# jasperlinthorst/reveal

Measured on AMD Instinct MI355X. Metric: Mbp/s indexed+MUM-anchored (reveal rem), higher is better.
Workload: dtype int32

## Files before the change

include/reveal_amd.h:

```cpp
#ifndef REVEAL_AMD_H
#define REVEAL_AMD_H
#include <stdint.h>

#ifdef __cplusplus
extern "C" {
#endif

typedef struct rv_index rv_index;

const char *rv_last_error(void);
int  rv_abi_version(void);
int  rv_sa_bits(void);
int  rv_device_count(void);

rv_index *rv_new(int device);
void rv_free(rv_index *h);

int rv_add_sample(rv_index *h);
int rv_add_sequence(rv_index *h, const char *seq, int64_t len, int64_t *begin, int64_t *end);
int rv_reset(rv_index *h);
int rv_reserve_text(rv_index *h, int64_t bytes);
int64_t rv_n(const rv_index *h);
int rv_nsamples(const rv_index *h);
int rv_nnodes(const rv_index *h);
// ... 39 lines not shown
int rv_align_end(rv_index *h);

typedef struct {
    int64_t steps;
    int64_t splits;
    int64_t anchored_bp;
    int32_t levels;
    int32_t maxdepth;
    int64_t scanned_ranks;
    double  t_scan, t_host, t_split, t_bubble;
} rv_align_stats;
int rv_align_builtin(rv_index *h, int minl, int minn, rv_align_stats *st);

int rv_align_builtin_until(rv_index *h, int minl, int minn, int stop_subs, rv_align_stats *st);
int rv_align_builtin_resume(rv_index *h, rv_align_stats *st);
int rv_align_builtin_continue(rv_index *h, int stop_subs, rv_align_stats *st);
int rv_frontier_counts(rv_index *h, int64_t *out);
int rv_frontier_export(rv_index *h, int64_t *meta, int64_t *node_first, int64_t *nodes);
int64_t rv_frontier_pack(rv_index *h, const int32_t *subs, int k, void *sa, void *lcp, void *bwt, int on_device);
int rv_frontier_import(rv_index *h, int minl, int minn, uint32_t maxlcp, int level, int nsubs, const int64_t *meta,
                       const int64_t *node_first, const int64_t *nodes, int64_t m,
                       const void *sa, const void *lcp, const void *bwt, int on_device);
int64_t rv_frontier_seeds_export(rv_index *h, const int32_t *subs, int k, int64_t *out, int64_t cap);
int rv_frontier_seeds_import(rv_index *h, int nsubs, const int64_t *words, int64_t nwords);
uint32_t rv_maxlcp(const rv_index *h);
int rv_cascade_info(const rv_index *h, int64_t *out);
int rv_capacity_events(const rv_index *h, int64_t *out);
const char *rv_cascade_why(const rv_index *h);
int64_t rv_anchor_count(rv_index *h, int64_t *members);
int rv_fetch_anchors(rv_index *h, uint32_t *l, int64_t *off, int64_t *pos);
int rv_set_result_buffers(rv_index *h, uint32_t *l, int64_t l_cap, int64_t *off, int64_t off_cap, int64_t *pos, int64_t pos_cap);
typedef struct {
    int64_t  key, n;
    int32_t  depth, nsamples, nnodes, picked;
    int64_t  nmums;
    uint32_t l; int32_t mn;
    int64_t  sp_min;
    uint64_t h_sa, h_lcp, h_mums;
} rv_trace;
int rv_set_trace(rv_index *h, int on);
int rv_set_preselect(rv_index *h, int64_t maxmums);
int rv_set_option(rv_index *h, const char *name, int64_t value);
int rv_get_option(rv_index *h, const char *name, int64_t *value);
int rv_set_launch_trace(int on);
int rv_option_count(void);
const char *rv_option_name(int k);
int64_t rv_trace_count(rv_index *h);
int rv_fetch_trace(rv_index *h, rv_trace *out, int64_t cap);

typedef struct rv_subindex rv_subindex;
rv_index *rv_clone(rv_index *h);
rv_subindex *rv_sx_main(rv_index *h);
rv_subindex *rv_sx_copy(rv_subindex *x);
void rv_sx_free(rv_subindex *x);
int rv_sx_info(const rv_subindex *x, rv_sub *out);
int rv_sx_nodes(const rv_subindex *x, int64_t *begin_end);
int64_t rv_sx_array(rv_subindex *x, int which, void *out, int64_t cap);
int64_t rv_sx_scan(rv_subindex *x, int minl, int minn, int64_t *members);
int rv_sx_fetch(rv_subindex *x, uint32_t *l, int32_t *n, int64_t *off, uint16_t *so, int64_t *pos);
int rv_sx_split(rv_subindex *x, const int64_t *lead, int nlead, const int64_t *trail, int ntrail,
                const int64_t *match, int nmatch, const int64_t *rest, int nrest, rv_subindex **out);
int rv_sx_extract(rv_subindex *x, int64_t *intervals, int niv);

int64_t rv_chain(int64_t m, int k, const uint32_t *len, const int32_t *nmem, const int64_t *crd, const int64_t *left,
                 const int64_t *right, int64_t wscore, int64_t wpen, int model, int64_t *out_idx, int64_t *out_score);

typedef struct { int64_t wscore, wpen, maxmums, seedsize; int gcmodel; int trim; double pcutoff; } rv_picker_args;
typedef struct {
    int picked; uint32_t pick_l; int32_t pick_n; int pick_members; uint16_t *pick_so; int64_t *pick_pos; int64_t member_cap;
    int64_t nleft, nright, nseed_members, seed_cap, seed_member_cap;
    uint32_t *seed_l; int32_t *seed_n; int64_t *seed_off; uint16_t *seed_so; int64_t *seed_pos; int64_t *seed_score; uint8_t *seed_right;
} rv_picker_out;
int rv_set_picker(rv_index *h, int kind, const rv_picker_args *args);
int rv_picker_info(const rv_index *h, int64_t *out);
int rv_pick_chain(const rv_picker_args *args, int nsub, int64_t m, const uint32_t *l, const int32_t *n, const int64_t *off, const uint16_t *so,
                  const int64_t *pos, int nsamples, const int64_t *seq_begin, const int64_t *iv_begin, const int64_t *iv_end, int minlength,
                  rv_picker_out *out);

typedef struct rv_graph rv_graph;
rv_graph *rv_graph_import(int64_t nnodes, const int64_t *node_b, const int64_t *node_e, const int8_t *node_aligned, const int8_t *node_sent,
                          const int64_t *off_ptr, const int32_t *off_sid, const int64_t *off_val,
                          int64_t nedges, const int32_t *edge_u, const int32_t *edge_v, const int64_t *edge_ptr, const int32_t *edge_paths,
                          const int64_t *pred_ptr, const int32_t *pred_edge, int npaths, const uint8_t *star, const int64_t *id2end,
                          int nstart, const int32_t *start_nodes, int literal_segments);
int rv_graph_pick(rv_graph *g, const rv_picker_args *args, int nsub, int64_t m, const uint32_t *l, const int32_t *n, const int64_t *off, const uint16_t *so, const int64_t *pos,
                  const int64_t *left, const int64_t *right, int minlength, rv_picker_out *out);
int rv_graph_align(rv_graph *g, const int64_t *nodes, int64_t nn, const int64_t *left, const int64_t *right, uint32_t l, const int64_t *pos, int npos,
                   int64_t *counts, int64_t *out6);
int rv_graph_align_fetch(rv_graph *g, int64_t *out);
int rv_set_graph_picker(rv_index *h, rv_graph *g, const rv_picker_args *args);
rv_graph *rv_graph_new(void);
int rv_graph_add_linear(rv_graph *g, int64_t b, int64_t e, int star);
int64_t rv_graph_read_gfa(rv_graph *g, rv_index *h, int64_t *text_n, const char *data, int64_t len, const char **names);
typedef struct GfaParsed rv_gfa_parsed;
rv_gfa_parsed *rv_gfa_parse(const char *data, int64_t len);
int64_t rv_graph_adopt(rv_graph *g, rv_index *h, int64_t *text_n, rv_gfa_parsed *parsed, const char **names);
void rv_gfa_parsed_free(rv_gfa_parsed *parsed);
int rv_graph_seal(rv_graph *g);
int rv_graph_paths(const rv_graph *g, int64_t *id2end);
int rv_graph_node_kinds(const rv_graph *g, int8_t *out);
int rv_graph_literal(const rv_graph *g);
int rv_graph_finish(rv_graph *g);
rv_graph *rv_graph_replay_begin(int nseq, const int64_t *begin, const int64_t *end);
int rv_set_replay_graph(rv_index *h, rv_graph *g);
rv_graph *rv_graph_replay(int nseq, const int64_t *begin, const int64_t *end, int64_t na, const uint32_t *an_l, const int64_t *an_off, const int64_t *an_pos);
const char *rv_graph_error(const rv_graph *g);
int rv_graph_sizes(const rv_graph *g, int64_t *out);
int rv_graph_export(const rv_graph *g, int64_t *node_b, int64_t *node_e, int8_t *node_aligned, int64_t *off_ptr, int32_t *off_sid, int64_t *off_val,
                    int64_t *succ_ptr, int32_t *succ_to, int32_t *succ_edge, int64_t *pred_ptr, int32_t *pred_from, int32_t *pred_edge, int64_t *edge_ptr, int32_t *edge_paths);
int rv_graph_prune(rv_graph *g, const char *T);
int64_t rv_graph_gfa(rv_graph *g, const char *T, int npaths, const char *const *names, const char *cmdline, const char **out);
void rv_graph_free(rv_graph *g);

enum { RV_K_SCAN_PAIR = 0, RV_K_SCAN_MULTI = 1, RV_K_SA_SORT = 2, RV_K_LCP = 3, RV_K_SPLIT = 4, RV_K_LABEL = 5,
       RV_K_BUBBLE = 6,
       RV_K_RADIX_SCATTER = 7, RV_K_RADIX_HIST = 8, RV_K_TEXT_ROUND = 9,
       RV_K_CASCADE = 10,
       RV_K_DIAG_TABLE = 11,
       RV_K_INIT_KEYS = 12,
       RV_K_PUBLISH = 13,
       RV_K_COUNT = 14 };
int rv_prof_enable(rv_index *h, int on);
int rv_prof_reset(rv_index *h);
int rv_prof_get(rv_index *h, int k, int64_t *launches, double *ms, double *bytes);
typedef struct rv_batch rv_batch;
rv_batch *rv_batch_new(void);
int rv_batch_add(rv_batch *b, rv_index *h);
int rv_batch_run(rv_batch *b, int minl, int minn, int construct, rv_align_stats *stats, int *status);
int rv_batch_info(const rv_batch *b, int64_t *out);
void rv_batch_free(rv_batch *b);
typedef struct rv_many rv_many;
rv_many *rv_many_new(int device);
void rv_many_free(rv_many *m);
int rv_many_option(rv_many *m, const char *name, int64_t value);
int rv_many_set_picker(rv_many *m, int kind, const rv_picker_args *args);
int64_t rv_many_add(rv_many *m, const char *const *seqs, const int64_t *lens, int k);
int rv_many_clear(rv_many *m);
int rv_many_run(rv_many *m, int minl, int minn, rv_align_stats *total);
int64_t rv_many_anchor_count(rv_many *m, int64_t *first, int64_t *members);
int rv_many_fetch(rv_many *m, uint32_t *l, int64_t *off, int64_t *pos);
int64_t rv_many_text(rv_many *m, int64_t job, char *out, int64_t cap);
int rv_many_info(const rv_many *m, int64_t *out);
int64_t rv_many_arrays(rv_many *m, int64_t job, int which, void *out, int64_t cap);
void *rv_dev_alloc(int device, int64_t bytes);
int rv_dev_free(int device, void *p);
int rv_ipc_export(int device, const void *p, uint8_t handle[64]);
void *rv_ipc_open(int device, const uint8_t handle[64]);
int rv_ipc_close(int device, void *p);
int rv_dev_copy(int device, void *dst, const void *src, int64_t bytes);
int rv_measure_bandwidth(int device, int64_t bytes, int iters, double *read_gbs, double *copy_gbs);
int rv_sa_stats(rv_index *h, int *sigma, int *bits, int *k0, int *rounds, int64_t *sorted_elems, int *radix_passes);
int rv_sa_diag_table(rv_index *h);
int rv_sa_tail(rv_index *h, int64_t *out);

int rv_test_exclusive_sum_u32(const uint32_t *in, uint32_t *out, int64_t n);
int rv_test_inclusive_max_u32(const uint32_t *in, uint32_t *out, int64_t n);
int rv_test_radix_sort(uint64_t *keys, uint32_t *vals, int64_t n, int bit_lo, int bit_hi);
int rv_test_radix_time(int64_t n, int bits, int dist, int flags, int iters, double *ms, int64_t *bad);

#ifdef __cplusplus
}
#endif
#endif
```

reveal_amd/_index.py:

```python
import ctypes
import mmap
import os
import sys
import numpy as np

from . import _lib
from ._lib import RV_T, RV_SA, RV_SAI, RV_LCP, RV_SO, RV_NSEP


def _page_array(count, dtype):
    nbytes = max(int(count), 1) * np.dtype(dtype).itemsize
    m = mmap.mmap(-1, (nbytes + mmap.PAGESIZE - 1) // mmap.PAGESIZE * mmap.PAGESIZE)
    return np.frombuffer(m, dtype=dtype, count=max(int(count), 1))


def _pairs(iv, sa64):
    a = np.ascontiguousarray(np.array([(int(b), int(e)) for b, e in iv], dtype=np.int64).reshape(-1, 2))
    return a, len(a)


_OPTION_DEFAULTS = {}


def make_index_type(sa64, error):

    class index(object):

        def __init__(self, sa="", lcp="", cache=0):
            self._lib = _lib.get(sa64)
            self._dll = self._lib.dll
            self._h = None
            self._safile, self._lcpfile, self._cache = sa or "", lcp or "", int(cache)
            self._samples, self._nodes, self.skipmums = [], set(), []
            self._leftnode = self._rightnode = None
            self._depth = 0
            self._constructed = False
            self._main = self
            self._slot = None
            self._sx = None
            self._n_sub = None
            self._nsamples_sub = None
            self._h = self._dll.rv_new(_lib.device())
            if not self._h:
                raise error(self._lib.err())
            self.options_from_env()

        def set_option(self, name, value=1):
            if self._dll.rv_set_option(self._main._h, name.encode(), int(value)) != 0:
                self._fail()

        def get_option(self, name):
            v = ctypes.c_int64(0)
            if self._dll.rv_get_option(self._main._h, name.encode(), ctypes.byref(v)) != 0:
                self._fail()
            return v.value

        def options_from_env(self):
            for k in range(self._dll.rv_option_count()):
                name = self._dll.rv_option_name(k).decode()
                v = os.environ.get(name)
                if v is None:
                    d = _OPTION_DEFAULTS.get((sa64, name))
                    if d is None:
                        d = _OPTION_DEFAULTS[(sa64, name)] = self.get_option(name)
                    elif self.get_option(name) != d:
                        self.set_option(name, d)
                    continue
                try:
                    iv = int(v) if v.strip() else 1
                except ValueError:
                    iv = 1
                _OPTION_DEFAULTS.setdefault((sa64, name), self.get_option(name))
                self.set_option(name, iv)

        @property
        def _main(self):
            m = self.__dict__.get("_main_ref")
            return self if m is None else m

        @_main.setter
        def _main(self, v):
            self.__dict__["_main_ref"] = None if v is self else v

        def __del__(self):
            try:
                if getattr(self, "_sx", None):
                    self._dll.rv_sx_free(self._sx)
                    self._sx = None
                if self._h and self._main is self:
                    self._dll.rv_free(self._h)
                    self._h = None
            except Exception:
                pass

        def _fail(self, exc=None):
            raise (exc or error)(self._lib.err())

        def addsample(self, *args):
            if len(args) < 1:
                raise error("Specify name of sample as argument.")
            if not isinstance(args[0], str):
                raise error("Sample name has to be a string.")
            self._samples.append(args[0])
            self._dll.rv_add_sample(self._h)
            self._constructed = False
            return None

        def addsequence(self, seq):
            if isinstance(seq, str):
                seq = seq.encode()
            elif not isinstance(seq, (bytes, bytearray)):
                raise TypeError("argument 1 must be str or bytes")
            b, e = ctypes.c_int64(0), ctypes.c_int64(0)
            if self._dll.rv_add_sequence(self._h, bytes(seq), len(seq), ctypes.byref(b), ctypes.byref(e)) != 0:
                self._fail()
            intv = (b.value, e.value)
            self._nodes.add(intv)
            self._constructed = False
            return intv

        def reset(self, reserve=0):
            if self._main is not self or self._slot is not None:
                raise error("reset() is for a main index outside align()")
            if self._sx:
                self._dll.rv_sx_free(self._sx)
                self._sx = None
            if self._dll.rv_reset(self._h) != 0:
                self._fail()
            if reserve and self._dll.rv_reserve_text(self._h, int(reserve)) != 0:
                self._fail()
            self._samples, self._nodes, self.skipmums = [], set(), []
            self._leftnode = self._rightnode = None
            self._depth = 0
            self._constructed = False
            self._pending = False
            self._n_sub = self._nsamples_sub = None

        def upload(self):
            if self._dll.rv_upload(self._h) != 0:
                self._fail()

        def upload_again(self):
            if self._dll.rv_upload_again(self._h) != 0:
                self._fail()

        def prof(self, enable=None, reset=False, only=None):
            ids = {"scan_pair": _lib.K_SCAN_PAIR, "scan_multi": _lib.K_SCAN_MULTI, "sa_build": _lib.K_SA_SORT, "lcp": _lib.K_LCP,
                   "split": _lib.K_SPLIT, "label": _lib.K_LABEL, "bubble": _lib.K_BUBBLE, "radix_scatter": _lib.K_RADIX_SCATTER,
                   "radix_hist": _lib.K_RADIX_HIST, "text_round": _lib.K_TEXT_ROUND, "cascade": _lib.K_CASCADE, "diag_table": _lib.K_DIAG_TABLE,
                   "init_keys": _lib.K_INIT_KEYS, "publish": _lib.K_PUBLISH}
            if enable is not None:
                on = 0
                if enable:
                    on = 1 if only is None else sum(2 << ids[k] for k in only)
                self._dll.rv_prof_enable(self._h, on)
            if reset:
                self._dll.rv_prof_reset(self._h)
            out = {}
            for name, k in ids.items():
                n, ms, by = ctypes.c_int64(0), ctypes.c_double(0), ctypes.c_double(0)
                self._dll.rv_prof_get(self._h, k, ctypes.byref(n), ctypes.byref(ms), ctypes.byref(by))
                out[name] = (n.value, ms.value, by.value)
            return out

        def sa_stats(self):
            v = [ctypes.c_int(0) for _ in range(4)]
            se, rp = ctypes.c_int64(0), ctypes.c_int(0)
            self._dll.rv_sa_stats(self._h, *[ctypes.byref(x) for x in v], ctypes.byref(se), ctypes.byref(rp))
            tail = (ctypes.c_int64 * 2)()
            self._dll.rv_sa_tail(self._h, tail)
            return dict(sigma=v[0].value, bits=v[1].value, k0=v[2].value, rounds=v[3].value, sorted_elems=se.value, radix_passes=rp.value,
                        diag_table=int(self._dll.rv_sa_diag_table(self._h)), far_pairs=int(tail[0]), lcp_list=int(tail[1]))

        def construct(self, rc=0):
            if self._sx:
                self._dll.rv_sx_free(self._sx)
                self._sx = None
            r = self._dll.rv_construct(self._h, int(rc), self._safile.encode(), self._lcpfile.encode(), self._cache)
            if r != 0:
                self._fail()
            self._constructed = True
            self._rc = 1 if int(rc) == 1 else 0
            self._depth = 0
            self._main = self
            return None

        def _sx_info(self):
            info = _lib.RvSub()
            self._dll.rv_sx_info(self._sx, ctypes.byref(info))
            return info

        @property
        def n(self):
            if self._sx:
                return self._sx_info().n
            return self._n_sub if self._n_sub is not None else self._dll.rv_n(self._h)

        @property
        def depth(self):
            return self._depth

        @property
        def nsamples(self):
            if self._sx and self._depth > 0:
                return self._sx_info().nsamples
            return self._nsamples_sub if self._nsamples_sub is not None else self._dll.rv_nsamples(self._h)

        @property
        def samples(self):
            return self._main._samples

        @property
        def nodes(self):
            if self.__dict__.get("_nodes_stale"):
                self._sync_nodes()
            return self._nodes

        @property
        def leftnode(self):
            return self._leftnode

        @property
        def rightnode(self):
            return self._rightnode

        @property
        def nsep(self):
            ns = self._dll.rv_nsamples(self._h)
            out = np.zeros(max(ns - 1, 1), dtype=np.int64)
            k = self._dll.rv_get_array(self._h, RV_NSEP, out.ctypes.data, len(out))
            return [int(x) for x in out[:max(k, 0)]]

        def _array(self, which, dtype, count, exc=TypeError):
            out = np.zeros(max(count, 1), dtype=dtype)
            if self._sx and which in (RV_SA, RV_LCP):
                k = self._dll.rv_sx_array(self._sx, which, out.ctypes.data, len(out))
            elif self._slot is not None and which in (RV_SA, RV_LCP):
                k = self._dll.rv_sub_array(self._h, self._slot, which, out.ctypes.data, len(out))
            else:
                k = self._dll.rv_get_array(self._h, which, out.ctypes.data, len(out))
            if k < 0:
                raise exc(self._lib.err())
            return out[:k]

        def _main_n(self):
            return self._dll.rv_n(self._h)

        @property
        def SA(self):
            return self._array(RV_SA, self._lib.sa_t, self.n).tolist()

        @property
        def LCP(self):
            return self._array(RV_LCP, self._lib.lcp_t, self.n).tolist()

        @property
        def SAi(self):
            return self._array(RV_SAI, self._lib.sa_t, self._main_n()).tolist()

        @property
        def SO(self):
            return self._array(RV_SO, np.uint16, self._main_n()).tolist()

        @property
        def T(self):
            return self._array(RV_T, np.uint8, self._main_n(), exc=error).tobytes().decode("latin-1")

        def array(self, name):
            which = {"SA": RV_SA, "LCP": RV_LCP, "SAi": RV_SAI, "SO": RV_SO, "T": RV_T}[name]
            dt = {RV_SA: self._lib.sa_t, RV_LCP: self._lib.lcp_t, RV_SAI: self._lib.sa_t, RV_SO: np.uint16, RV_T: np.uint8}[which]
            return self._array(which, dt, self.n if which in (RV_SA, RV_LCP) else self._main_n())

        def _sx_mums(self, minl, minn):
            mem = ctypes.c_int64(0)
            cnt = self._dll.rv_sx_scan(self._sx, int(minl), int(minn), ctypes.byref(mem))
            if cnt < 0:
                self._fail()
            l = np.zeros(max(cnt, 1), dtype=np.uint32); n = np.zeros(max(cnt, 1), dtype=np.int32)
            off = np.zeros(cnt + 1, dtype=np.int64)
            so = np.zeros(max(mem.value, 1), dtype=np.uint16); pos = np.zeros(max(mem.value, 1), dtype=np.int64)
            if self._dll.rv_sx_fetch(self._sx, l.ctypes.data, n.ctypes.data, off.ctypes.data, so.ctypes.data, pos.ctypes.data) != 0:
                self._fail()
            return _csr_to_tuples(cnt, l, n, off, so, pos)

        def getmums(self, minl=0):
            if self._sx:
                if self._dll.rv_nsamples(self._h) != 2:
                    raise error("getmums on a sub-index needs a two-sample main index")
                rc = 1 if getattr(self._main, "_rc", 0) else 0
                out = [(l, (spd[0][1], spd[1][1]), rc) for l, _, spd in self._sx_mums(minl, 0)]
                if rc:
                    nsep0, nT = self.nsep[0], self._main_n()
                    out = [(l, (a, nsep0 + (nT - b - l)), rc) for l, (a, b), _ in out]
                return out
            cnt = self._dll.rv_getmums(self._h, int(minl))
            if cnt < 0:
                self._fail(TypeError if cnt == -2 else error)
            l = np.zeros(max(cnt, 1), dtype=np.uint32)
            a = np.zeros(max(cnt, 1), dtype=np.int64)
            b = np.zeros(max(cnt, 1), dtype=np.int64)
            if self._dll.rv_fetch_mums(self._h, l.ctypes.data, a.ctypes.data, b.ctypes.data, len(l)) != 0:
                self._fail()
            rc = 1 if getattr(self, "_rc", 0) else 0
            return [(int(l[k]), (int(a[k]), int(b[k])), rc) for k in range(cnt)]

        def _multi(self, minlength, minn, mems):
            if self._sx:
                if mems or self._dll.rv_nsamples(self._h) <= 2:
                    raise error("only getmultimums of an index with more than two samples is available on a sub-index")
                return self._sx_mums(minlength, minn)
            members = ctypes.c_int64(0)
            cnt = self._dll.rv_getmultimums(self._h, int(minlength), int(minn), mems, ctypes.byref(members))
            if cnt < 0:
                self._fail(TypeError if cnt == -2 else error)
            l = np.zeros(max(cnt, 1), dtype=np.uint32); n = np.zeros(max(cnt, 1), dtype=np.int32)
            off = np.zeros(cnt + 1, dtype=np.int64)
            so = np.zeros(max(members.value, 1), dtype=np.uint16); pos = np.zeros(max(members.value, 1), dtype=np.int64)
            if self._dll.rv_fetch_multi(self._h, l.ctypes.data, n.ctypes.data, off.ctypes.data, so.ctypes.data, pos.ctypes.data) != 0:
                self._fail()
            return _csr_to_tuples(cnt, l, n, off, so, pos)

        def getmultimums(self, minlength=0, minn=2):
            return self._multi(minlength, minn, 0)

        def getmultimems(self, minlength=0, minn=2):
# ... 404 lines not shown
```

reveal_amd/_lib.py:

```python
import ctypes
import importlib.util
import os
import sys
import numpy as np

_HERE = os.path.dirname(os.path.abspath(__file__))

RV_T, RV_SA, RV_SAI, RV_LCP, RV_SO, RV_NSEP, RV_NODES = range(7)
K_SCAN_PAIR, K_SCAN_MULTI, K_SA_SORT, K_LCP, K_SPLIT, K_LABEL, K_BUBBLE, K_RADIX_SCATTER, K_RADIX_HIST, K_TEXT_ROUND, K_CASCADE, K_DIAG_TABLE, K_INIT_KEYS, K_PUBLISH = range(14)

CAPACITY_EVENTS = ("pair_ovf", "pair_out", "pair_pick_ovf", "pair_second_copy", "multi_rec", "multi_mem", "multi_cand",
                   "mems_rec", "mems_mem", "mems_long")
CAP_SITES = {"multi_cand": 1, "cas_wit": 2, "cas_tables": 4, "casm_matches": 8, "casm_wit": 16, "casm_tables": 32,
             "mems_rec": 64, "mems_mem": 128, "mems_long": 256}

c_i64p = ctypes.POINTER(ctypes.c_int64)
V = ctypes.c_void_p


class RvSub(ctypes.Structure):
    _fields_ = [("n", ctypes.c_int64), ("depth", ctypes.c_int32), ("nsamples", ctypes.c_int32),
                ("nnodes", ctypes.c_int32), ("parent", ctypes.c_int32), ("kind", ctypes.c_int32),
                ("reserved", ctypes.c_int32), ("nmums", ctypes.c_int64), ("nmembers", ctypes.c_int64)]


class RvAlignStats(ctypes.Structure):
    _fields_ = [("steps", ctypes.c_int64), ("splits", ctypes.c_int64), ("anchored_bp", ctypes.c_int64),
                ("levels", ctypes.c_int32), ("maxdepth", ctypes.c_int32), ("scanned_ranks", ctypes.c_int64),
                ("t_scan", ctypes.c_double), ("t_host", ctypes.c_double), ("t_split", ctypes.c_double),
                ("t_bubble", ctypes.c_double)]


TRACE_DTYPE = np.dtype([("key", np.int64), ("n", np.int64), ("depth", np.int32), ("nsamples", np.int32),
                        ("nnodes", np.int32), ("picked", np.int32), ("nmums", np.int64), ("l", np.uint32),
                        ("mn", np.int32), ("sp_min", np.int64), ("h_sa", np.uint64), ("h_lcp", np.uint64),
                        ("h_mums", np.uint64)], align=True)

_I, _L, _D = ctypes.c_int, ctypes.c_int64, ctypes.c_double
SYMBOLS = {
    "rv_last_error": (ctypes.c_char_p, []),
    "rv_abi_version": (_I, []),
    "rv_sa_bits": (_I, []),
    "rv_device_count": (_I, []),
    "rv_new": (V, [_I]),
    "rv_free": (None, [V]),
    "rv_add_sample": (_I, [V]),
    "rv_add_sequence": (_I, [V, ctypes.c_char_p, _L, c_i64p, c_i64p]),
    "rv_reset": (_I, [V]),
    "rv_reserve_text": (_I, [V, _L]),
    "rv_n": (_L, [V]),
    "rv_nsamples": (_I, [V]),
    "rv_nnodes": (_I, [V]),
    "rv_node_list": (_I, [V, V]),
    "rv_construct": (_I, [V, _I, ctypes.c_char_p, ctypes.c_char_p, _I]),
    "rv_upload": (_I, [V]),
    "rv_upload_again": (_I, [V]),
    "rv_get_array": (_L, [V, _I, V, _L]),
    "rv_getmums": (_L, [V, _I]),
    "rv_fetch_mums": (_I, [V, V, V, V, _L]),
    "rv_getmultimums": (_L, [V, _I, _I, _I, c_i64p]),
    "rv_fetch_multi": (_I, [V, V, V, V, V, V]),
    "rv_align_begin": (_I, [V, _I, _I]),
    "rv_frontier_size": (_I, [V]),
    "rv_frontier_scan": (_I, [V]),
    "rv_sub_skip_scan": (_I, [V, _I]),
    "rv_sub_info": (_I, [V, _I, ctypes.POINTER(RvSub)]),
    "rv_sub_nodes": (_I, [V, _I, V]),
    "rv_sub_mums": (_I, [V, _I, V, V, V, V, V]),
    "rv_sub_array": (_L, [V, _I, _I, V, _L]),
    "rv_sub_split": (_I, [V, _I, ctypes.c_uint32, _I, V, V, _I, V, _I, V, _I, V, _I]),
    "rv_frontier_commit": (_I, [V, V]),
    "rv_align_end": (_I, [V]),
    "rv_align_builtin": (_I, [V, _I, _I, ctypes.POINTER(RvAlignStats)]),
    "rv_align_builtin_until": (_I, [V, _I, _I, _I, ctypes.POINTER(RvAlignStats)]),
    "rv_align_builtin_resume": (_I, [V, ctypes.POINTER(RvAlignStats)]),
    "rv_align_builtin_continue": (_I, [V, _I, ctypes.POINTER(RvAlignStats)]),
    "rv_frontier_counts": (_I, [V, V]),
    "rv_frontier_export": (_I, [V, V, V, V]),
    "rv_frontier_pack": (_L, [V, V, _I, V, V, V, _I]),
    "rv_frontier_import": (_I, [V, _I, _I, ctypes.c_uint32, _I, _I, V, V, V, _L, V, V, V, _I]),
    "rv_frontier_seeds_export": (_L, [V, V, _I, V, _L]),
    "rv_frontier_seeds_import": (_I, [V, _I, V, _L]),
    "rv_maxlcp": (ctypes.c_uint32, [V]),
    "rv_cascade_info": (ctypes.c_int, [V, V]),
    "rv_cascade_why": (ctypes.c_char_p, [V]),
    "rv_capacity_events": (_I, [V, V]),
    "rv_anchor_count": (_L, [V, c_i64p]),
    "rv_fetch_anchors": (_I, [V, V, V, V]),
    "rv_set_result_buffers": (_I, [V, V, _L, V, _L, V, _L]),
    "rv_set_trace": (_I, [V, _I]),
    "rv_set_preselect": (_I, [V, _L]),
    "rv_set_option": (_I, [V, ctypes.c_char_p, _L]),
    "rv_set_launch_trace": (_I, [_I]),
    "rv_batch_new": (V, []),
    "rv_batch_add": (_I, [V, V]),
    "rv_batch_run": (_I, [V, _I, _I, _I, V, V]),
    "rv_batch_info": (_I, [V, V]),
    "rv_batch_free": (None, [V]),
    "rv_dev_alloc": (V, [_I, _L]),
    "rv_dev_free": (_I, [_I, V]),
    "rv_ipc_export": (_I, [_I, V, V]),
    "rv_ipc_open": (V, [_I, V]),
    "rv_ipc_close": (_I, [_I, V]),
    "rv_dev_copy": (_I, [_I, V, V, _L]),
    "rv_get_option": (_I, [V, ctypes.c_char_p, c_i64p]),
    "rv_option_count": (_I, []),
    "rv_option_name": (ctypes.c_char_p, [_I]),
    "rv_trace_count": (_L, [V]),
    "rv_fetch_trace": (_I, [V, V, _L]),
    "rv_clone": (V, [V]),
    "rv_sx_main": (V, [V]),
    "rv_sx_copy": (V, [V]),
    "rv_sx_free": (None, [V]),
    "rv_sx_info": (_I, [V, ctypes.POINTER(RvSub)]),
    "rv_sx_nodes": (_I, [V, V]),
    "rv_sx_array": (_L, [V, _I, V, _L]),
    "rv_sx_scan": (_L, [V, _I, _I, c_i64p]),
    "rv_sx_fetch": (_I, [V, V, V, V, V, V]),
    "rv_sx_split": (_I, [V, V, _I, V, _I, V, _I, V, _I, V]),
    "rv_sx_extract": (_I, [V, V, _I]),
    "rv_chain": (_L, [_L, _I, V, V, V, V, V, _L, _L, _I, V, V]),
    "rv_prof_enable": (_I, [V, _I]),
    "rv_prof_reset": (_I, [V]),
    "rv_prof_get": (_I, [V, _I, c_i64p, ctypes.POINTER(_D), ctypes.POINTER(_D)]),
    "rv_measure_bandwidth": (_I, [_I, _L, _I, ctypes.POINTER(_D), ctypes.POINTER(_D)]),
    "rv_sa_stats": (_I, [V] + [ctypes.POINTER(_I)] * 4 + [c_i64p, ctypes.POINTER(_I)]),
    "rv_sa_diag_table": (_I, [V]),
    "rv_sa_tail": (_I, [V, c_i64p]),
    "rv_set_picker": (_I, [V, _I, V]),
    "rv_picker_info": (_I, [V, c_i64p]),
    "rv_pick_chain": (_I, [V, _I, _L, V, V, V, V, V, _I, V, V, V, _I, V]),
    "rv_graph_import": (V, [_L, V, V, V, V, V, V, V, _L, V, V, V, V, V, V, _I, V, V, _I, V, _I]),
    "rv_graph_pick": (_I, [V, V, _I, _L, V, V, V, V, V, V, V, _I, V]),
    "rv_graph_align": (_I, [V, V, _L, V, V, ctypes.c_uint32, V, _I, V, V]),
    "rv_graph_align_fetch": (_I, [V, V]),
    "rv_graph_finish": (_I, [V]),
    "rv_set_graph_picker": (_I, [V, V, V]),
    "rv_graph_new": (V, []),
    "rv_graph_replay_begin": (V, [_I, V, V]),
    "rv_set_replay_graph": (_I, [V, V]),
    "rv_graph_add_linear": (_I, [V, _L, _L, _I]),
    "rv_graph_read_gfa": (_L, [V, V, V, V, _L, V]),
    "rv_graph_paths": (_I, [V, V]),
    "rv_graph_seal": (_I, [V]),
    "rv_gfa_parse": (V, [V, _L]),
    "rv_graph_adopt": (_L, [V, V, V, V, V]),
    "rv_gfa_parsed_free": (None, [V]),
    "rv_add_sequences": (_I, [V, V, _L, V, _L]),
    "rv_graph_node_kinds": (_I, [V, V]),
    "rv_graph_literal": (_I, [V]),
    "rv_graph_replay": (V, [_I, V, V, _L, V, V, V]),
    "rv_graph_error": (ctypes.c_char_p, [V]),
    "rv_graph_sizes": (_I, [V, c_i64p]),
    "rv_graph_export": (_I, [V] * 15),
    "rv_graph_prune": (_I, [V, V]),
    "rv_graph_gfa": (_L, [V, V, _I, V, V, V]),
    "rv_graph_free": (None, [V]),
    "rv_many_new": (V, [_I]),
    "rv_many_free": (None, [V]),
    "rv_many_option": (_I, [V, ctypes.c_char_p, _L]),
    "rv_many_set_picker": (_I, [V, _I, V]),
    "rv_many_add": (_L, [V, V, V, _I]),
    "rv_many_clear": (_I, [V]),
    "rv_many_run": (_I, [V, _I, _I, ctypes.POINTER(RvAlignStats)]),
    "rv_many_anchor_count": (_L, [V, V, c_i64p]),
    "rv_many_fetch": (_I, [V, V, V, V]),
    "rv_many_text": (_L, [V, _L, V, _L]),
    "rv_many_info": (_I, [V, V]),
    "rv_many_arrays": (_L, [V, _L, _I, V, _L]),
    "rv_test_exclusive_sum_u32": (_I, [V, V, _L]),
    "rv_test_inclusive_max_u32": (_I, [V, V, _L]),
    "rv_test_radix_sort": (_I, [V, V, _L, _I, _I]),
    "rv_test_radix_time": (_I, [_L, _I, _I, _I, _I, ctypes.POINTER(_D), c_i64p]),
}


def _share_torch_runtime():
    if os.environ.get("RV_SYSTEM_HIP") or "torch" in sys.modules:
        return
    try:
        spec = importlib.util.find_spec("torch")
    except (ImportError, ValueError):
        spec = None
    if spec is None or not spec.origin:
        return
    path = os.path.join(os.path.dirname(spec.origin), "lib", "libamdhip64.so")
    if os.path.exists(path):
        ctypes.CDLL(path, mode=ctypes.RTLD_GLOBAL)


class Lib:
    def __init__(self, sa64=False):
        self.sa64 = sa64
        _share_torch_runtime()
        name = "libreveal_amd64.so" if sa64 else "libreveal_amd.so"
        self.path = os.path.join(os.environ.get("RV_LIB_DIR") or _HERE, name)
        if not os.path.exists(self.path):
            raise ImportError("%s is missing: build it with `python -c 'import __graft_entry__ as g; g.build()'` "
                              "(hipcc --offload-arch=gfx950); reveal_amd has no CPU fallback" % self.path)
        self.dll = ctypes.CDLL(self.path)
        for sym, (res, args) in SYMBOLS.items():
            fn = getattr(self.dll, sym)
            fn.restype, fn.argtypes = res, args
        self.sa_t = np.int64 if sa64 else np.int32
        self.lcp_t = np.uint32 if sa64 else np.int32
        assert self.dll.rv_sa_bits() == (64 if sa64 else 32)
        v = os.environ.get("RV_LAUNCH_TRACE")
        if v is not None and v.strip() not in ("", "0"):
            self.dll.rv_set_launch_trace(1)

    def err(self):
        return (self.dll.rv_last_error() or b"").decode(errors="replace")


_libs = {}
_device = 0


def set_device(i):
    global _device
    _device = int(i)


def device():
    return _device


def measure_bandwidth(nbytes=1 << 30, iters=10):
    lib = get(False)
    r, c = _D(0), _D(0)
    if lib.dll.rv_measure_bandwidth(device(), int(nbytes), int(iters), ctypes.byref(r), ctypes.byref(c)) != 0:
        raise RuntimeError(lib.err())
    return r.value, c.value


def set_launch_trace(on=True):
    return [bool(get(w).dll.rv_set_launch_trace(1 if on else 0)) for w in (False, True)]


def get(sa64=False):
    if sa64 not in _libs:
        _libs[sa64] = Lib(sa64)
    return _libs[sa64]
```

reveal_amd/csrc/rv_api.hip:

```cpp
#include "rv_index.h"
#include "rv_cascade.h"
#include <limits>
#include <stdarg.h>
#include <stdio.h>
#include <string.h>
#include <limits.h>
#include <algorithm>
#include <thread>

static thread_local char g_err[1024] = "";

void rv_set_error(const char *fmt, ...) {
    va_list ap;
    va_start(ap, fmt);
    vsnprintf(g_err, sizeof g_err, fmt, ap);
    va_end(ap);
}

static std::vector<rv_index *> &live_handles() { static std::vector<rv_index *> v; return v; }
std::mutex &rv_trim_mutex() { static std::mutex *m = new std::mutex(); return *m; }
bool rv_oom_trim() {
    size_t got = 0;
    bool log = false;
    int caller_dev = 0;
// ... 788 lines not shown
        int id = h->prof.begin(q, RV_K_SCAN_MULTI, (double)m * (sizeof(sa_t) + sizeof(lcp_t)));
        RV_TRY(rv_scan_multi_launch(h->ws, SA, LCP, m, BWT, h->dNsep.as<sa_t>(), h->nsamples, minl, minn,
                                    brec.as<RvMultiRec>(), bso.as<uint16_t>(), bpos.as<sa_t>(), (u32)std::min<size_t>(rcap, 0xffffffffu),
                                    (u32)std::min<size_t>(mcap, 0xffffffffu), bcnt.as<u32>(), btab.as<uint4>(), d_sub_start, d_sub_want, nsubs));
        h->prof.end(q, id);
        u32 tot[2] = {0, 0};
        RV_HIP(hipMemcpyAsync(tot, bcnt.p, 8, hipMemcpyDeviceToHost, q));
        RV_HIP(hipMemcpyAsync(tab.data(), btab.p, (size_t)ntile * sizeof(uint4), hipMemcpyDeviceToHost, q));
        RV_HIP(hipStreamSynchronize(q));
        if (tot[0] <= rcap && tot[1] <= mcap) {
            std::vector<RvMultiRec> rr(tot[0]);
            std::vector<uint16_t> rso(tot[1]);
            std::vector<sa_t> rpos(tot[1]);
            if (tot[0]) RV_HIP(hipMemcpy(rr.data(), brec.p, (size_t)tot[0] * sizeof(RvMultiRec), hipMemcpyDeviceToHost));
            if (tot[1]) {
                RV_HIP(hipMemcpy(rso.data(), bso.p, (size_t)tot[1] * 2, hipMemcpyDeviceToHost));
                RV_HIP(hipMemcpy(rpos.data(), bpos.p, (size_t)tot[1] * sizeof(sa_t), hipMemcpyDeviceToHost));
            }
            l.reserve(tot[0]); n.reserve(tot[0]); off.reserve(tot[0] + 1); so.reserve(tot[1]); pos.reserve(tot[1]);
            for (int64_t t = 0; t < ntile; t++) {
                const uint4 e = tab[(size_t)t];
                for (u32 k = 0; k < e.y; k++) {
                    const RvMultiRec &r = rr[e.x + k];
                    l.push_back(r.l); n.push_back((int32_t)r.n);
                    if (ub_out) ub_out->push_back((int64_t)r.ub);
                }
                for (u32 k = 0; k < e.w; k++) { so.push_back(rso[e.z + k]); pos.push_back((int64_t)rpos[e.z + k]); }
            }
            int64_t acc = 0;
            for (size_t k = 0; k < n.size(); k++) { acc += n[k]; off.push_back(acc); }
            return 0;
        }
        if (tot[0] > rcap) { h->ws.cap_events[RV_CE_MULTI_REC]++; RV_TRY(brec.reserve((size_t)tot[0] * sizeof(RvMultiRec))); }
        if (tot[1] > mcap) { h->ws.cap_events[RV_CE_MULTI_MEM]++; RV_TRY(bso.reserve((size_t)tot[1] * 2)); RV_TRY(bpos.reserve((size_t)tot[1] * sizeof(sa_t))); }
    }
    rv_set_error("multi scan: output buffer sizing failed");
    return -1;
}

int rv_run_multi_pick(rv_index *h, const sa_t *SA, const lcp_t *LCP, const uint8_t *BWT, int64_t m, int minl, int minn,
                      const int64_t *d_sub_start, const int *d_sub_want, int nsubs, const int *d_tile_sub, std::vector<u32> &pick_l, std::vector<sa_t> &pick_pos,
                      int (*after_pick)(rv_index *), bool *redo) {
    pick_l.assign((size_t)nsubs, 0); pick_pos.clear();
    if (m <= 1 || nsubs <= 0) return 0;
    hipStream_t q = h->ws.stream;
    const int W = h->nsamples;
    DBuf &bbest = h->ws.misc[12], &bl = h->ws.misc[13], &bpos = h->ws.misc[7], &bcand = h->ws.misc[8], &bcnt = h->ws.misc[1];
    RV_TRY(bbest.reserve((size_t)nsubs * 8)); RV_TRY(bl.reserve((size_t)nsubs * 4)); RV_TRY(bpos.reserve((size_t)nsubs * W * sizeof(sa_t)));
    RV_TRY(bcnt.reserve((RV_MULTI_REGIONS * 64 + 16) * 4));
    if (bcand.cap < 65536 * RV_MULTI_CAND_BYTES) RV_TRY(bcand.reserve((size_t)std::max<int64_t>(65536, m / 64) * RV_MULTI_CAND_BYTES));
    for (int attempt = 0; attempt < 2; attempt++) {
        size_t ccap = std::min<size_t>(bcand.cap / RV_MULTI_CAND_BYTES, 0xffffffffu);
        if (attempt == 0) ccap = h->ws.cap_first<size_t>(RV_CS_MULTI_CAND, ccap, RV_MULTI_REGIONS);
        h->ws.multi_cand_cap = (u32)(ccap / RV_MULTI_REGIONS);
        hipEvent_t ev_a, ev_b;
        (void)h->prof.attach(RV_K_SCAN_MULTI, (double)m * 8.0, &ev_a, &ev_b);
        RV_TRY(rv_multi_pick_launch(h->ws, SA, LCP, m, BWT, h->dNsep.as<sa_t>(), W, minl, minn, d_sub_start, d_sub_want, nsubs, d_tile_sub,
                                    bbest.as<unsigned long long>(), bl.as<u32>(), bpos.as<sa_t>(), (RvMultiCand *)bcand.p,
                                    (u32)ccap, bcnt.as<u32>(), ev_a, ev_b));
        u32 ncand = 0;
        pick_pos.resize((size_t)nsubs * W);
        {
            const size_t b1 = (size_t)nsubs * 4, b2 = (size_t)nsubs * W * sizeof(sa_t), o1 = 64, o2 = (o1 + b1 + 63) & ~(size_t)63;
            RV_TRY(h->ws.hpin.reserve(o2 + b2 + 64));
            uint8_t *hp = h->ws.hpin.as<uint8_t>();
            if (!h->ws.ev_rb) RV_HIP(hipEventCreateWithFlags(&h->ws.ev_rb, hipEventDisableTiming));
            RV_HIP(hipMemcpyAsync(hp, bcnt.as<u32>() + RV_MULTI_REGIONS * 64, 4, hipMemcpyDeviceToHost, q));
            RV_HIP(hipMemcpyAsync(hp + o1, bl.p, b1, hipMemcpyDeviceToHost, q));
            RV_HIP(hipMemcpyAsync(hp + o2, bpos.p, b2, hipMemcpyDeviceToHost, q));
            RV_HIP(hipEventRecord(h->ws.ev_rb, q));
            if (attempt == 0 && after_pick) RV_TRY(after_pick(h));
            const hipError_t qe = rv_event_wait(h->ws.ev_rb);
            if (qe != hipSuccess) { rv_set_error("stream: %s", hipGetErrorString(qe)); return -1; }
            memcpy(&ncand, hp, 4); memcpy(pick_l.data(), hp + o1, b1); memcpy(pick_pos.data(), hp + o2, b2);
        }
        if ((size_t)ncand <= ccap / RV_MULTI_REGIONS) return 0;
        if (redo) *redo = true;
        h->ws.cap_events[RV_CE_MULTI_CAND]++;
        RV_TRY(bcand.reserve(((size_t)ncand + ncand / 2 + 64) * RV_MULTI_REGIONS * RV_MULTI_CAND_BYTES));
    }
    rv_set_error("multi picker: candidate buffer sizing failed");
    return -1;
}

extern "C" {

int64_t rv_getmultimums(rv_index *h, int minlength, int minn, int mems, int64_t *members) {
    if (!h->constructed || h->main_arrays_freed) { rv_set_error("Index not yet constructed."); return -2; }
    if (h->nsamples <= 2) {
        if (mems && h->nsamples == 2 && minn >= 2) { h->mm_l.clear(); h->mm_n.clear(); h->mm_off.assign(1, 0); h->mm_so.clear(); h->mm_pos.clear(); if (members) *members = 0; return 0; }
        rv_set_error("getmultimums needs more than two samples (SO not available)"); return -1;
    }
    (void)hipSetDevice(h->device);
    if (rv_run_multi_scan(h, h->dSA.as<sa_t>(), h->dLCP.as<lcp_t>(), h->dBWT.as<uint8_t>(), h->n, minlength, minn, mems, h->mm_l, h->mm_n, h->mm_off, h->mm_so, h->mm_pos, nullptr, nullptr, nullptr, 0)) return -1;
    if (members) *members = (int64_t)h->mm_pos.size();
    return (int64_t)h->mm_l.size();
}

int rv_fetch_multi(rv_index *h, uint32_t *l, int32_t *n, int64_t *off, uint16_t *so, int64_t *pos) {
    memcpy(l, h->mm_l.data(), h->mm_l.size() * 4);
    memcpy(n, h->mm_n.data(), h->mm_n.size() * 4);
    memcpy(off, h->mm_off.data(), h->mm_off.size() * 8);
    memcpy(so, h->mm_so.data(), h->mm_so.size() * 2);
    memcpy(pos, h->mm_pos.data(), h->mm_pos.size() * 8);
    return 0;
}

int64_t rv_getmums(rv_index *h, int minl) {
    if (!h->constructed || h->main_arrays_freed) { rv_set_error("Index not yet constructed."); return -2; }
    (void)hipSetDevice(h->device);
    std::vector<RvPairRec> recs;
    if (rv_run_pair_scan(h, h->dSA.as<sa_t>(), h->dLCP.as<lcp_t>(), h->dBWT.as<uint8_t>(), h->n, minl, recs, nullptr, nullptr, nullptr, 0, nullptr, false) != 0) return -1;
    h->m_l.resize(recs.size()); h->m_a.resize(recs.size()); h->m_b.resize(recs.size());
    for (size_t k = 0; k < recs.size(); k++) {
        int64_t b = recs[k].b;
        if (h->rc == 1) b = h->nsep[0] + (h->nT - b - (int64_t)recs[k].l);
        h->m_l[k] = recs[k].l; h->m_a[k] = recs[k].a; h->m_b[k] = b;
    }
    return (int64_t)recs.size();
}

int rv_fetch_mums(rv_index *h, uint32_t *l, int64_t *a, int64_t *b, int64_t cap) {
    if (cap < (int64_t)h->m_l.size()) { rv_set_error("buffer too small"); return -1; }
    for (size_t k = 0; k < h->m_l.size(); k++) { l[k] = h->m_l[k]; a[k] = h->m_a[k]; b[k] = h->m_b[k]; }
    return 0;
}

int rv_prof_enable(rv_index *h, int on) {
    h->prof.on = on != 0;
    h->prof.mask = (on & 1) ? 0xFFFFFFFFu : ((u32)on >> 1);
    return 0;
}
int rv_prof_reset(rv_index *h) { (void)hipStreamSynchronize(h->ws.stream); h->prof.reset(); return 0; }
int rv_prof_get(rv_index *h, int k, int64_t *launches, double *ms, double *bytes) {
    if (k < 0 || k >= RV_K_COUNT) { rv_set_error("bad kernel id"); return -1; }
    (void)hipStreamSynchronize(h->ws.stream);
    h->prof.resolve();
    if (launches) *launches = h->prof.launches[k];
    if (ms) *ms = h->prof.ms[k];
    if (bytes) *bytes = h->prof.bytes[k];
    return 0;
}
int rv_sa_stats(rv_index *h, int *sigma, int *bits, int *k0, int *rounds, int64_t *sorted_elems, int *radix_passes) {
    if (sigma) *sigma = h->sa_stats.sigma;
    if (bits) *bits = h->sa_stats.bits;
    if (k0) *k0 = h->sa_stats.k0;
    if (rounds) *rounds = h->sa_stats.rounds;
    if (sorted_elems) *sorted_elems = h->sa_stats.sorted_elems;
    if (radix_passes) *radix_passes = h->sa_stats.radix_passes;
    return 0;
}
int rv_sa_diag_table(rv_index *h) { return h->sa_stats.diag_table; }
int rv_sa_tail(rv_index *h, int64_t *out) { if (!h || !out) return -1; out[0] = h->sa_stats.far_pairs; out[1] = h->sa_stats.lcp_list; return 0; }

}
namespace {
typedef int bw_v4 __attribute__((ext_vector_type(4)));
__global__ __launch_bounds__(256) void k_bw_read(const bw_v4 *__restrict__ a, int64_t n16, unsigned *sink) {
    bw_v4 acc = {0, 0, 0, 0};
    for (int64_t i = (int64_t)blockIdx.x * 256 + threadIdx.x; i < n16; i += (int64_t)gridDim.x * 256) acc ^= __builtin_nontemporal_load(a + i);
    if ((acc.x ^ acc.y ^ acc.z ^ acc.w) == 0x12345678) sink[0] = 1;
}
__global__ __launch_bounds__(256) void k_bw_copy(const bw_v4 *__restrict__ a, bw_v4 *__restrict__ b, int64_t n16) {
    for (int64_t i = (int64_t)blockIdx.x * 256 + threadIdx.x; i < n16; i += (int64_t)gridDim.x * 256) __builtin_nontemporal_store(__builtin_nontemporal_load(a + i), b + i);
}
}
extern "C" {
struct rv_batch {
    std::vector<rv_index *> hs;
    RvBatchGroup *g = nullptr;
    std::vector<std::string> errs;
};
rv_batch *rv_batch_new(void) {
    try { return new rv_batch(); } catch (...) { rv_set_error("rv_batch_new: out of host memory"); return nullptr; }
}
int rv_batch_add(rv_batch *b, rv_index *h) {
    if (!b || !h) { rv_set_error("rv_batch_add: null argument"); return -1; }
    if (!b->hs.empty() && b->hs[0]->device != h->device) { rv_set_error("rv_batch_add: the handles of a batch live on one device"); return -1; }
    try { b->hs.push_back(h); } catch (...) { rv_set_error("rv_batch_add: out of host memory"); return -1; }
    return 0;
}
void rv_batch_free(rv_batch *b) {
    if (!b) return;
    rv_batch_group_free(b->g);
    delete b;
}
int rv_batch_info(const rv_batch *b, int64_t *out) {
    out[0] = out[1] = 0;
    if (b && b->g) rv_batch_group_info(b->g, out);
    return 0;
}
int rv_batch_run(rv_batch *b, int minl, int minn, int construct, rv_align_stats *stats, int *status) {
    if (!b || b->hs.empty()) { rv_set_error("rv_batch_run: empty batch"); return -1; }
    const int n = (int)b->hs.size();
    try {
        b->errs.assign((size_t)n, std::string());
        if (!b->g) b->g = rv_batch_group_new(b->hs[0]->device);
        int members = 0;
        for (rv_index *h : b->hs) {
            const bool in = h->nsamples > 2 && !h->ws.opt.no_cascade;
            h->batch = in ? b->g : nullptr; h->batch_settled = false;
            members += in ? 1 : 0;
        }
        rv_batch_group_begin(b->g, members);
        std::vector<int> rc((size_t)n, 0);
        auto work = [&](int i) {
            rv_index *h = b->hs[(size_t)i];
            int r = 0;
            if (hipSetDevice(h->device) != hipSuccess) { rv_set_error("hipSetDevice failed"); r = -1; }
            if (r == 0 && construct) r = rv_construct(h, 0, "", "", 0);
            if (r == 0) r = rv_align_builtin(h, minl, minn, stats ? &stats[i] : nullptr);
            if (h->batch && !h->batch_settled) { h->batch_settled = true; rv_batch_group_leave(h->batch); }
            if (r != 0) b->errs[(size_t)i] = rv_last_error();
            rc[(size_t)i] = r;
        };
        std::vector<std::thread> th;
        int started = n;
        for (int i = 1; i < n; i++) {
            try { th.emplace_back(work, i); }
            catch (...) { started = i; break; }
        }
        if (started < n) for (int i = started; i < n; i++) { rv_index *h = b->hs[(size_t)i]; if (h->batch) { h->batch_settled = true; rv_batch_group_leave(h->batch); h->batch = nullptr; } }
        work(0);
        for (auto &t : th) t.join();
        for (int i = started; i < n; i++) work(i);
        int bad = -1;
        for (int i = 0; i < n; i++) { b->hs[(size_t)i]->batch = nullptr; if (status) status[i] = rc[(size_t)i]; if (rc[(size_t)i] != 0 && bad < 0) bad = i; }
        if (bad >= 0) { rv_set_error("rv_batch_run: job %d: %s", bad, b->errs[(size_t)bad].c_str()); return -1; }
        return 0;
    } catch (const std::exception &e) {
        for (rv_index *h : b->hs) h->batch = nullptr;
        rv_set_error("rv_batch_run: %s", e.what());
        return -1;
    }
}

void *rv_dev_alloc(int device, int64_t bytes) {
    void *p = nullptr;
    if (bytes < 0 || hipSetDevice(device) != hipSuccess) { rv_set_error("rv_dev_alloc: bad device or size"); return nullptr; }
    const hipError_t e = hipMalloc(&p, (size_t)std::max<int64_t>(bytes, 256));
    if (e != hipSuccess) { (void)hipGetLastError(); rv_set_error("rv_dev_alloc(%lld bytes): %s", (long long)bytes, hipGetErrorString(e)); return nullptr; }
    return p;
}
int rv_dev_free(int device, void *p) {
    if (!p) return 0;
    RV_HIP(hipSetDevice(device));
    RV_HIP(hipFree(p));
    return 0;
}
int rv_ipc_export(int device, const void *p, uint8_t handle[64]) {
    static_assert(sizeof(hipIpcMemHandle_t) == 64, "hipIpcMemHandle_t is 64 bytes");
    RV_HIP(hipSetDevice(device));
    hipIpcMemHandle_t hd;
    RV_HIP(hipIpcGetMemHandle(&hd, const_cast<void *>(p)));
    memcpy(handle, &hd, 64);
    return 0;
}
void *rv_ipc_open(int device, const uint8_t handle[64]) {
    if (hipSetDevice(device) != hipSuccess) { rv_set_error("rv_ipc_open: bad device"); return nullptr; }
    hipIpcMemHandle_t hd;
    memcpy(&hd, handle, 64);
    void *p = nullptr;
    const hipError_t e = hipIpcOpenMemHandle(&p, hd, hipIpcMemLazyEnablePeerAccess);
    if (e != hipSuccess) { (void)hipGetLastError(); rv_set_error("rv_ipc_open: %s", hipGetErrorString(e)); return nullptr; }
    return p;
}
int rv_ipc_close(int device, void *p) {
    if (!p) return 0;
    RV_HIP(hipSetDevice(device));
    RV_HIP(hipIpcCloseMemHandle(p));
    return 0;
}
int rv_dev_copy(int device, void *dst, const void *src, int64_t bytes) {
    if (bytes <= 0) return 0;
    RV_HIP(hipSetDevice(device));
    RV_HIP(hipMemcpy(dst, src, (size_t)bytes, hipMemcpyDefault));
    RV_HIP(hipStreamSynchronize(nullptr));
    return 0;
}

int rv_measure_bandwidth(int device, int64_t bytes, int iters, double *read_gbs, double *copy_gbs) {
    if (bytes < (1 << 20) || iters < 1) { rv_set_error("rv_measure_bandwidth: bytes >= 1 MiB and iters >= 1 needed"); return -1; }
    RV_HIP(hipSetDevice(device));
    const int64_t n16 = bytes / 16;
    void *a = nullptr, *b = nullptr; unsigned *sink = nullptr;
    hipStream_t q = nullptr; hipEvent_t e0 = nullptr, e1 = nullptr;
    RV_HIP(hipMalloc(&a, (size_t)n16 * 16)); RV_HIP(hipMalloc(&b, (size_t)n16 * 16)); RV_HIP(hipMalloc((void **)&sink, 64));
    RV_HIP(hipStreamCreateWithFlags(&q, hipStreamNonBlocking));
    RV_HIP(hipEventCreate(&e0)); RV_HIP(hipEventCreate(&e1));
    RV_HIP(hipMemsetAsync(a, 1, (size_t)n16 * 16, q)); RV_HIP(hipMemsetAsync(b, 2, (size_t)n16 * 16, q));
    const unsigned grid = 256 * 16;
    double out[2] = {0, 0};
    for (int pass = 0; pass < 2; pass++) {
        for (int r = -1; r < iters; r++) {
            if (r == 0) RV_HIP(hipEventRecord(e0, q));
            if (pass == 0) hipLaunchKernelGGL(k_bw_read, dim3(grid), dim3(256), 0, q, (const bw_v4 *)a, n16, sink);
            else hipLaunchKernelGGL(k_bw_copy, dim3(grid), dim3(256), 0, q, (const bw_v4 *)a, (bw_v4 *)b, n16);
        }
        RV_HIP(hipEventRecord(e1, q));
        RV_HIP(hipEventSynchronize(e1));
        float ms = 0.f;
        RV_HIP(hipEventElapsedTime(&ms, e0, e1));
        out[pass] = (double)n16 * 16 * (pass ? 2 : 1) * iters / ((double)ms * 1e6);
    }
    if (read_gbs) *read_gbs = out[0];
    if (copy_gbs) *copy_gbs = out[1];
    (void)hipEventDestroy(e0); (void)hipEventDestroy(e1); (void)hipStreamDestroy(q);
    (void)hipFree(a); (void)hipFree(b); (void)hipFree(sink);
    return 0;
}

static int test_ws(Workspace &ws) {
    if (rv_device_count() <= 0) { rv_set_error("no HIP device"); return -1; }
    RV_HIP(hipSetDevice(0));
    RV_HIP(hipStreamCreateWithFlags(&ws.stream, hipStreamNonBlocking));
    return 0;
}
static void test_ws_done(Workspace &ws) { ws.release(); (void)hipStreamDestroy(ws.stream); }

static int test_scan(const uint32_t *in, uint32_t *out, int64_t n, bool maxscan) {
    Workspace ws;
    RV_TRY(test_ws(ws));
    DBuf a, b;
    int r = 0;
    if (a.reserve((size_t)n * 4 + 64) || b.reserve((size_t)n * 4 + 64)) r = -1;
    if (!r && hipMemcpy(a.p, in, (size_t)n * 4, hipMemcpyHostToDevice) != hipSuccess) r = -1;
    if (!r) r = maxscan ? rv_inclusive_max_u32(ws, a.as<u32>(), b.as<u32>(), n) : rv_exclusive_sum_u32(ws, a.as<u32>(), b.as<u32>(), n);
    if (!r && hipStreamSynchronize(ws.stream) != hipSuccess) { rv_set_error("sync failed: %s", hipGetErrorString(hipGetLastError())); r = -1; }
    if (!r && hipMemcpy(out, b.p, (size_t)n * 4, hipMemcpyDeviceToHost) != hipSuccess) r = -1;
    a.release(); b.release();
    test_ws_done(ws);
    return r;
}
int rv_test_exclusive_sum_u32(const uint32_t *in, uint32_t *out, int64_t n) { return test_scan(in, out, n, false); }
int rv_test_inclusive_max_u32(const uint32_t *in, uint32_t *out, int64_t n) { return test_scan(in, out, n, true); }

int rv_test_radix_sort(uint64_t *keys, uint32_t *vals, int64_t n, int bit_lo, int bit_hi) {
    Workspace ws;
    RV_TRY(test_ws(ws));
    DBuf k0, k1, v0, v1;
    int r = 0, in1 = 0;
    if (k0.reserve((size_t)n * 8 + 64) || k1.reserve((size_t)n * 8 + 64) || v0.reserve((size_t)n * 4 + 64) || v1.reserve((size_t)n * 4 + 64)) r = -1;
    if (!r && hipMemcpy(k0.p, keys, (size_t)n * 8, hipMemcpyHostToDevice) != hipSuccess) r = -1;
    if (!r && hipMemcpy(v0.p, vals, (size_t)n * 4, hipMemcpyHostToDevice) != hipSuccess) r = -1;
    if (!r) r = rv_radix_sort_pairs<u32>(ws, k0.as<u64>(), v0.as<u32>(), k1.as<u64>(), v1.as<u32>(), n, bit_lo, bit_hi, &in1);
    if (!r && hipStreamSynchronize(ws.stream) != hipSuccess) { rv_set_error("sync failed: %s", hipGetErrorString(hipGetLastError())); r = -1; }
    if (!r && hipMemcpy(keys, in1 ? k1.p : k0.p, (size_t)n * 8, hipMemcpyDeviceToHost) != hipSuccess) r = -1;
    if (!r && hipMemcpy(vals, in1 ? v1.p : v0.p, (size_t)n * 4, hipMemcpyDeviceToHost) != hipSuccess) r = -1;
    k0.release(); k1.release(); v0.release(); v1.release();
    test_ws_done(ws);
    return r;
}

}
namespace {
__device__ inline u64 rt_mix(u64 x) { x ^= x >> 33; x *= 0xff51afd7ed558ccdull; x ^= x >> 33; x *= 0xc4ceb9fe1a85ec53ull; x ^= x >> 33; return x; }
__global__ __launch_bounds__(256) void k_rt_fill(u64 *keys, u32 *vals, int64_t n, int bits, int dist) {
    const int64_t i = (int64_t)blockIdx.x * 256 + threadIdx.x;
    if (i >= n) return;
    u64 r = rt_mix((u64)i * 0x9E3779B97F4A7C15ull + 12345);
    u64 k = 0;
    if (dist == 0) k = r;
    else if (dist == 1) { u64 r2 = rt_mix(r); for (int j = 0; j < 17; j++) { k = k * 5 + 1 + (r2 & 3); r2 >>= 2; } }
    const u64 mask = bits >= 64 ? ~0ull : (1ull << bits) - 1;
    keys[i] = (k & mask) | (r & ~mask & 0x00ffffffffffffffull);
    vals[i] = (u32)i;
}
__global__ __launch_bounds__(256) void k_rt_check(const u64 *keys, const u32 *vals, int64_t n, int bits, unsigned long long *bad) {
    const int64_t i = (int64_t)blockIdx.x * 256 + threadIdx.x;
    if (i + 1 >= n) return;
    const u64 mask = bits >= 64 ? ~0ull : (1ull << bits) - 1;
    const u64 a = keys[i] & mask, b = keys[i + 1] & mask;
    if (a > b || (a == b && vals[i] > vals[i + 1])) atomicAdd(bad, 1ull);
}
}
extern "C" {
int rv_test_radix_time(int64_t n, int bits, int dist, int flags, int iters, double *ms, int64_t *bad) {
    Workspace ws;
    RV_TRY(test_ws(ws));
    ws.opt.rs_bits = (flags & 1) ? 10 : 8; ws.opt.rs_xcd = (flags & 2) ? 1 : 0; ws.opt.rs_cnt16 = (flags & 4) ? 1 : 0; ws.opt.rs_no_digit_bytes = (flags & 8) ? 1 : 0;
    DBuf k0, k1, v0, v1, db;
    int r = 0, in1 = 0;
    hipEvent_t e0 = nullptr, e1 = nullptr;
    if (k0.reserve((size_t)n * 8 + 64) || k1.reserve((size_t)n * 8 + 64) || v0.reserve((size_t)n * 4 + 64) || v1.reserve((size_t)n * 4 + 64) || db.reserve(64)) r = -1;
    if (!r && (hipEventCreate(&e0) != hipSuccess || hipEventCreate(&e1) != hipSuccess)) r = -1;
    for (int it = 0; !r && it < iters; it++) {
        hipLaunchKernelGGL(k_rt_fill, dim3((unsigned)ceil_div(n, 256)), dim3(256), 0, ws.stream, k0.as<u64>(), v0.as<u32>(), n, bits, dist);
        (void)hipEventRecord(e0, ws.stream);
        r = rv_radix_sort_pairs<u32>(ws, k0.as<u64>(), v0.as<u32>(), k1.as<u64>(), v1.as<u32>(), n, 0, bits, &in1);
        (void)hipEventRecord(e1, ws.stream);
        if (!r && hipEventSynchronize(e1) != hipSuccess) { rv_set_error("sync failed: %s", hipGetErrorString(hipGetLastError())); r = -1; }
        float t = 0;
        if (!r) { (void)hipEventElapsedTime(&t, e0, e1); ms[it] = t; }
    }
    if (!r) {
        (void)hipMemsetAsync(db.p, 0, 8, ws.stream);
        hipLaunchKernelGGL(k_rt_check, dim3((unsigned)ceil_div(n, 256)), dim3(256), 0, ws.stream, (const u64 *)(in1 ? k1.p : k0.p), (const u32 *)(in1 ? v1.p : v0.p), n, bits,
                           db.as<unsigned long long>());
        unsigned long long b = 0;
        if (hipMemcpyAsync(&b, db.p, 8, hipMemcpyDeviceToHost, ws.stream) != hipSuccess || hipStreamSynchronize(ws.stream) != hipSuccess) r = -1;
        *bad = (int64_t)b;
    }
    if (e0) (void)hipEventDestroy(e0);
    if (e1) (void)hipEventDestroy(e1);
    k0.release(); k1.release(); v0.release(); v1.release(); db.release();
    test_ws_done(ws);
    return r;
}

}
```

reveal_amd/csrc/rv_common.h:

```cpp
#pragma once
#include <algorithm>
#include <mutex>
#include <thread>
#include <vector>
#include <utility>
#include <hip/hip_runtime.h>
#include <stdint.h>
#include <string.h>
#include <stddef.h>
#include <vector>
#include <string>

#ifdef RV_SA64
typedef int64_t  sa_t;
typedef uint32_t lcp_t;
#else
typedef int32_t  sa_t;
typedef int32_t  lcp_t;
#endif

typedef unsigned long long u64;
typedef unsigned int       u32;

void rv_set_error(const char *fmt, ...);

#define RV_HIP(x)                                                                              \
    do {                                                                                       \
        hipError_t e_ = (x);                                                                   \
        if (e_ != hipSuccess) {                                                                \
            rv_set_error("%s:%d %s: %s", __FILE__, __LINE__, #x, hipGetErrorString(e_));       \
            return -1;                                                                         \
        }                                                                                      \
    } while (0)
#define RV_TRY(x)                                                                              \
    do {                                                                                       \
        int r_ = (x);                                                                          \
        if (r_ != 0) return r_;                                                                \
    } while (0)
#define RV_OPTION_LIST(X) \
    X(bubble_par_min, "RV_BUBBLE_PAR_MIN", -1) \
    X(presel_log, "RV_PRESEL_LOG", 0) \
    X(presel_host, "RV_PRESEL_HOST", 0) \
    X(leaf_acap, "RV_LEAF_ACAP", 256) \
    X(bubble_lds_always, "RV_BUBBLE_LDS_ALWAYS", 0) \
    X(no_early_bubble, "RV_NO_EARLY_BUBBLE", 0) \
    X(early_bubble_many, "RV_EARLY_BUBBLE_MANY", 0) \
    X(no_early_split, "RV_NO_EARLY_SPLIT", 0) \
    X(keep_dead, "RV_KEEP_DEAD", 0) \
    X(bubble_no_lds, "RV_BUBBLE_NO_LDS", 0) \
    X(bubble_no_join, "RV_BUBBLE_NO_JOIN", 0) \
    X(bubble_no_merge, "RV_BUBBLE_NO_MERGE", 0) \
    X(tables_memcpy, "RV_TABLES_MEMCPY", 0) \
    X(bubble_parent_scratch, "RV_BUBBLE_PARENT_SCRATCH", 0) \
    X(level_log, "RV_LEVEL_LOG", 0) \
    X(pb_two_pass, "RV_PB_TWO_PASS", 0) \
    X(no_leaf, "RV_NO_LEAF", 0) \
    X(leaf_prof, "RV_LEAF_PROF", 0) \
    X(no_cascade, "RV_NO_CASCADE", 0) \
    X(cascade_second, "RV_CASCADE_SECOND", 0) \
    X(cascade_danger, "RV_CASCADE_DANGER", 1) \
    X(cascade_second_off, "RV_CASCADE_SECOND_OFF", 0) \
    X(sync_block, "RV_SYNC_BLOCK", 0) \
    X(pb_refresh_tmin, "RV_PB_REFRESH_TMIN", 0) \
    X(cascade_log, "RV_CASCADE_LOG", 0) \
    X(cascade_danger_min, "RV_CASCADE_DANGER_MIN", 0) \
    X(cascade_batch, "RV_CASCADE_BATCH", 8) \
    X(lcp_by_rank, "RV_LCP_BY_RANK", 0) \
    X(no_tiny_sa, "RV_NO_TINY_SA", 0) \
    X(no_short_alphabet, "RV_NO_SHORT_ALPHABET", 0) \
    X(no_fused_lcp, "RV_NO_FUSED_LCP", 0) \
    X(no_diag, "RV_NO_DIAG", 0) \
    X(no_packed_text, "RV_NO_PACKED_TEXT", 0) \
    X(no_heads_fusion, "RV_NO_HEADS_FUSION", 0) \
    X(no_twin_collapse, "RV_NO_TWIN_COLLAPSE", 0) \
    X(no_far_twins, "RV_NO_FAR_TWINS", 0) \
    X(no_lcp_list, "RV_NO_LCP_LIST", 0) \
    X(no_text_jump, "RV_NO_TEXT_JUMP", 0) \
    X(far_table, "RV_FAR_TABLE", 0) \
    X(no_slow_class, "RV_NO_SLOW_CLASS", 0) \
    X(no_dwalk_blocks, "RV_NO_DWALK_BLOCKS", 0) \
    X(no_pub_twins, "RV_NO_PUB_TWINS", 0) \
    X(sa_no_text, "RV_SA_NO_TEXT", 0) \
    X(text_mode, "RV_TEXT_MODE", -1) \
    X(carry_ch, "RV_CARRY_CH", -1) \
    X(rs_bits, "RV_RS_BITS", 8) \
    X(rs_xcd, "RV_RS_XCD", 1) \
    X(rs_cnt16, "RV_RS_CNT16", 1) \
    X(rs_no_digit_bytes, "RV_RS_NO_DIGIT_BYTES", 0) \
    X(diag_table, "RV_DIAG_TABLE", -1) \
    X(no_cascade_chain, "RV_NO_CASCADE_CHAIN", 0) \
    X(casm_rank_count, "RV_CASM_RANK_COUNT", 0) \
    X(casm_big_min, "RV_CASM_BIG_MIN", -1) \
    X(casm_no_big, "RV_CASM_NO_BIG", 0) \
    X(casm_big_root, "RV_CASM_BIG_ROOT", 1 << 22) \
    X(casm_big_total, "RV_CASM_BIG_TOTAL", 1 << 26) \
    X(lock_any, "RV_LOCK_ANY", 0) \
    X(presel_dev_min, "RV_PRESEL_DEV_MIN", 65536) \
    X(scan_v1, "RV_SCAN_V1", 0) \
    X(pick_threads, "RV_PICK_THREADS", 0) \
    X(cascade_prio, "RV_CASCADE_PRIO", 0) \
    X(cas_witness_pass, "RV_CAS_WITNESS_PASS", 0) \
    X(cap_limit, "RV_CAP_LIMIT", 0) \
    X(cap_sites, "RV_CAP_SITES", -1) \
    X(many_chain_multi, "RV_MANY_CHAIN_MULTI", 0)
struct RvOptions {
#define RV_X_(f, name, def) int64_t f = def;
    RV_OPTION_LIST(RV_X_)
#undef RV_X_
    int64_t *find(const char *name) {
#define RV_X_(f, nm, def) if (strcmp(name, nm) == 0) return &f;
        RV_OPTION_LIST(RV_X_)
#undef RV_X_
        return nullptr;
    }
};
extern int g_rv_launch_trace;
static inline bool rv_launch_trace_on() { return g_rv_launch_trace != 0; }
#define RV_LAUNCH_CHECK()                                                                      \
    do {                                                                                       \
        RV_HIP(hipGetLastError());                                                             \
        if (rv_launch_trace_on()) {                                                            \
            fprintf(stderr, "launch %s:%d\n", __FILE__, __LINE__);                             \
            fflush(stderr);                                                                    \
            RV_HIP(hipDeviceSynchronize());                                                    \
        }                                                                                      \
    } while (0)

static inline int64_t ceil_div(int64_t a, int64_t b) { return (a + b - 1) / b; }

#define RV_BWT_SIDE 0x80u
#define RV_BWT_CHAR 0x7fu

#ifdef __HIPCC__
__device__ inline u32 rv_wave_min_u32(u32 v) {
    const int inf = -1;
    int x = (int)v, y;
#define RV_DPP_MIN(ctrl, rmask)                                                        \
    y = __builtin_amdgcn_update_dpp(inf, x, ctrl, rmask, 0xf, false);                  \
    x = (int)(((u32)y < (u32)x) ? (u32)y : (u32)x);
    RV_DPP_MIN(0xB1, 0xf)
    RV_DPP_MIN(0x4E, 0xf)
    RV_DPP_MIN(0x141, 0xf)
    RV_DPP_MIN(0x140, 0xf)
    RV_DPP_MIN(0x142, 0xa)
    RV_DPP_MIN(0x143, 0xc)
#undef RV_DPP_MIN
    return (u32)__builtin_amdgcn_readlane(x, 63);
}
#endif

#ifdef __HIPCC__
template <int CTRL, int ROWMASK> __device__ inline u32 rv_dpp_u32(u32 x) { return (u32)__builtin_amdgcn_update_dpp(0, (int)x, CTRL, ROWMASK, 0xf, false); }
#define RV_WAVE_SCAN_STEPS(STEP)                                                     \
    STEP(0x111, 0xf, (lane & 15) >= 1)                                               \
    STEP(0x112, 0xf, (lane & 15) >= 2)                                               \
    STEP(0x114, 0xf, (lane & 15) >= 4)                                               \
    STEP(0x118, 0xf, (lane & 15) >= 8)                                               \
    STEP(0x142, 0xa, (lane & 31) >= 16)                                              \
    STEP(0x143, 0xc, lane >= 32)
__device__ inline u64 rv_wave_max_u64(u64 v) {
#define RV_STEP_(CTRL, RM, TAKE) { const u64 t = ((u64)rv_dpp_u32<CTRL, RM>((u32)(v >> 32)) << 32) | rv_dpp_u32<CTRL, RM>((u32)v); v = t > v ? t : v; }
    RV_WAVE_SCAN_STEPS(RV_STEP_)
#undef RV_STEP_
    return ((u64)(u32)__builtin_amdgcn_readlane((int)(u32)(v >> 32), 63) << 32) | (u32)__builtin_amdgcn_readlane((int)(u32)v, 63);
}
__device__ inline u64 rv_wave_seg_max_u64(u32 seg, u64 v) {
    const int lane = threadIdx.x & 63;
    u32 lo = (u32)v, hi = (u32)(v >> 32);
#define RV_STEP_(CTRL, RM, TAKE) { const u32 os = rv_dpp_u32<CTRL, RM>(seg), ol = rv_dpp_u32<CTRL, RM>(lo), oh = rv_dpp_u32<CTRL, RM>(hi); \
                                   const bool up = (TAKE) && os == seg && (oh > hi || (oh == hi && ol > lo)); lo = up ? ol : lo; hi = up ? oh : hi; }
    RV_WAVE_SCAN_STEPS(RV_STEP_)
#undef RV_STEP_
    return ((u64)hi << 32) | lo;
}
__device__ inline u32 rv_wave_seg_max_u32(u32 seg, u32 v) {
    const int lane = threadIdx.x & 63;
#define RV_STEP_(CTRL, RM, TAKE) { const u32 os = rv_dpp_u32<CTRL, RM>(seg), ov = rv_dpp_u32<CTRL, RM>(v); v = ((TAKE) && os == seg && ov > v) ? ov : v; }
    RV_WAVE_SCAN_STEPS(RV_STEP_)
#undef RV_STEP_
    return v;
}
__device__ inline u32 rv_wave_incl_sum_u32(u32 v) {
    const int lane = threadIdx.x & 63;
#define RV_STEP_(CTRL, RM, TAKE) { const u32 t = rv_dpp_u32<CTRL, RM>(v); v += (TAKE) ? t : 0u; }
    RV_WAVE_SCAN_STEPS(RV_STEP_)
#undef RV_STEP_
    return v;
}
#endif

bool rv_oom_trim();

inline hipError_t rv_event_wait(hipEvent_t ev) {
    hipError_t e;
    for (int spins = 0; (e = hipEventQuery(ev)) == hipErrorNotReady; spins++) {
        if (spins < 64) { __builtin_ia32_pause(); continue; }
        if (spins < 640) { std::this_thread::yield(); continue; }
        return hipEventSynchronize(ev);
    }
    return e;
}

struct DBuf {
    void  *p = nullptr;
    size_t cap = 0;
    int reserve(size_t bytes) {
        if (bytes <= cap) return 0;
        if (p) { (void)hipFree(p); p = nullptr; cap = 0; }
        size_t want = bytes + (bytes >= ((size_t)256 << 20) ? bytes / 64 : bytes / 8) + 256;
        hipError_t e = hipMalloc(&p, want);
        if (e == hipErrorOutOfMemory) {
            (void)hipGetLastError();
            if (rv_oom_trim()) e = hipMalloc(&p, want);
            if (e == hipErrorOutOfMemory) { (void)hipGetLastError(); want = bytes + 256; e = hipMalloc(&p, want); }
        }
        if (e != hipSuccess) { p = nullptr; rv_set_error("%s:%d hipMalloc(%zu bytes): %s", __FILE__, __LINE__, want, hipGetErrorString(e)); return -1; }
        cap = want;
        return 0;
    }
    void release() { if (p) (void)hipFree(p); p = nullptr; cap = 0; }
    template <class T> T *as() const { return (T *)p; }
};

struct RvPools {
    std::mutex mu;
    std::vector<std::pair<int, hipStream_t>> streams;
    struct Pin { int dev; void *p; size_t cap; };
    std::vector<Pin> pinned;
    size_t pinned_bytes = 0;
};
inline RvPools &rv_pools() { static RvPools *p = new RvPools(); return *p; }
inline hipError_t rv_stream_get(hipStream_t *s) {
    int dev = 0; (void)hipGetDevice(&dev);
    {
        RvPools &P = rv_pools();
        std::lock_guard<std::mutex> g(P.mu);
        for (size_t k = P.streams.size(); k-- > 0;)
            if (P.streams[k].first == dev) { *s = P.streams[k].second; P.streams.erase(P.streams.begin() + (ptrdiff_t)k); return hipSuccess; }
    }
    return hipStreamCreateWithFlags(s, hipStreamNonBlocking);
}
inline void rv_stream_put(hipStream_t s) {
    if (!s) return;
    (void)hipStreamSynchronize(s);
    int dev = 0; (void)hipGetDevice(&dev);
    RvPools &P = rv_pools();
    {
        std::lock_guard<std::mutex> g(P.mu);
        if (P.streams.size() < 64) { P.streams.push_back({dev, s}); return; }
    }
    (void)hipStreamDestroy(s);
}
inline hipError_t rv_pinned_get(size_t bytes, void **p, size_t *cap) {
    int dev = 0; (void)hipGetDevice(&dev);
    {
        RvPools &P = rv_pools();
        std::lock_guard<std::mutex> g(P.mu);
        size_t best = (size_t)-1;
        for (size_t k = 0; k < P.pinned.size(); k++)
            if (P.pinned[k].dev == dev && P.pinned[k].cap >= bytes && P.pinned[k].cap <= 4 * bytes + (1u << 20) && (best == (size_t)-1 || P.pinned[k].cap < P.pinned[best].cap)) best = k;
        if (best != (size_t)-1) { *p = P.pinned[best].p; *cap = P.pinned[best].cap; P.pinned_bytes -= *cap; P.pinned.erase(P.pinned.begin() + (ptrdiff_t)best); return hipSuccess; }
    }
    const hipError_t e = hipHostMalloc(p, bytes, hipHostMallocDefault);
    if (e == hipSuccess) *cap = bytes;
    return e;
}
inline void rv_pinned_put(void *p, size_t cap) {
    if (!p) return;
    int dev = 0; (void)hipGetDevice(&dev);
    RvPools &P = rv_pools();
    {
        std::lock_guard<std::mutex> g(P.mu);
        if (cap <= ((size_t)64 << 20) && P.pinned_bytes + cap <= ((size_t)512 << 20) && P.pinned.size() < 256) { P.pinned.push_back({dev, p, cap}); P.pinned_bytes += cap; return; }
    }
    (void)hipHostFree(p);
}

struct HBuf {
    void  *p = nullptr;
    size_t cap = 0;
    int reserve(size_t bytes) {
        if (bytes <= cap) return 0;
        if (p) { (void)hipDeviceSynchronize(); rv_pinned_put(p, cap); p = nullptr; cap = 0; }
        size_t want = bytes + bytes / 2 + 4096;
        RV_HIP(rv_pinned_get(want, &p, &cap));
        return 0;
    }
    void release() { if (p) rv_pinned_put(p, cap); p = nullptr; cap = 0; }
    template <class T> T *as() const { return (T *)p; }
};

enum RvCapEvent { RV_CE_PAIR_OVF = 0, RV_CE_PAIR_OUT, RV_CE_PAIR_PICK_OVF, RV_CE_PAIR_SECOND_COPY, RV_CE_MULTI_REC, RV_CE_MULTI_MEM, RV_CE_MULTI_CAND,
                  RV_CE_MEMS_REC, RV_CE_MEMS_MEM, RV_CE_MEMS_LONG, RV_CE_COUNT };
enum RvCapSite { RV_CS_MULTI_CAND = 1, RV_CS_CAS_WIT = 2, RV_CS_CAS_TABLES = 4, RV_CS_CASM_MATCHES = 8, RV_CS_CASM_WIT = 16, RV_CS_CASM_TABLES = 32,
                 RV_CS_MEMS_REC = 64, RV_CS_MEMS_MEM = 128, RV_CS_MEMS_LONG = 256 };
struct Workspace {
    hipStream_t stream = nullptr;
    RvOptions opt;
    int64_t cap_events[RV_CE_COUNT] = {0};
    u32 pair_ovf_cap = 0, multi_cand_cap = 0;
    template <class T> T cap_first(int site, T cap, T least = 1) const {
        if (opt.cap_limit <= 0 || !(opt.cap_sites & (int64_t)site)) return cap;
        const T lim = (T)std::max<int64_t>(opt.cap_limit, (int64_t)least);
        return cap < lim ? cap : lim;
    }
    DBuf scan_tmp[4];
    DBuf rs_hist;
    DBuf rs_digits;
    DBuf misc[20];
    DBuf sa[32];
    HBuf hpin;
    hipEvent_t ev_rb = nullptr;
    void *prof_ctx = nullptr;
    int (*prof_begin_fn)(void *, hipStream_t, int, double) = nullptr;
    void (*prof_end_fn)(void *, hipStream_t, int) = nullptr;
    int prof_begin(int k, double bytes) { return prof_begin_fn ? prof_begin_fn(prof_ctx, stream, k, bytes) : -1; }
    void prof_end(int id) { if (prof_end_fn && id >= 0) prof_end_fn(prof_ctx, stream, id); }
    bool sa_in_use = false;
    size_t trim_sa() {
        size_t got = 0;
        for (auto &b : sa) { got += b.cap; b.release(); }
        return got;
    }
    void release() {
        hpin.release();
        if (ev_rb) { (void)hipEventDestroy(ev_rb); ev_rb = nullptr; }
        for (auto &b : scan_tmp) b.release();
        rs_hist.release(); rs_digits.release();
        for (auto &b : misc) b.release();
        for (auto &b : sa) b.release();
    }
};

std::mutex &rv_trim_mutex();
struct SaScratchInUse {
    Workspace &w; bool was;
    SaScratchInUse(Workspace &x) : w(x) { std::lock_guard<std::mutex> g(rv_trim_mutex()); was = w.sa_in_use; w.sa_in_use = true; }
    ~SaScratchInUse() { std::lock_guard<std::mutex> g(rv_trim_mutex()); w.sa_in_use = was; }
};

int rv_exclusive_sum_u32(Workspace &ws, const u32 *in, u32 *out, int64_t n);
int rv_exclusive_sum_u64(Workspace &ws, const u64 *in, u64 *out, int64_t n);
int rv_inclusive_max_u32(Workspace &ws, const u32 *in, u32 *out, int64_t n);
int rv_inclusive_max_u64(Workspace &ws, const u64 *in, u64 *out, int64_t n);

int rv_radix_passes(const Workspace &ws, int nbits);
template <class V>
int rv_radix_sort_pairs(Workspace &ws, u64 *k0, V *v0, u64 *k1, V *v1, int64_t n,
                        int bit_lo, int bit_hi, int *result_in_1, bool first_digits = false);
uint8_t *rv_radix_first_digits(Workspace &ws, int64_t n, int bit_lo, int bit_hi);

int rv_read_back(Workspace &ws, void *dst, const void *dsrc, size_t bytes);
int rv_read_back2(Workspace &ws, void *dst_a, const void *dsrc_a, size_t bytes_a, void *dst_b, const void *dsrc_b, size_t bytes_b);

int rv_h2d_copy(Workspace &ws, const void *pinned_src, void *dst, size_t bytes);

struct RvSaStats {
    int    sigma, bits, k0;
    int    rounds;
    int64_t sorted_elems;
    int    radix_passes;
    int    diag_table;
    int64_t far_pairs;
    int64_t lcp_list;
};
int rv_build_sa(Workspace &ws, const uint8_t *T, int64_t n, sa_t *SA, RvSaStats *st,
                lcp_t *LCP = nullptr, uint8_t *BWT = nullptr, sa_t side_sep = 0, u32 *d_maxlcp = nullptr, bool *fused_done = nullptr,
                const int64_t *seps = nullptr, int nseps = 0);
int rv_build_inverse(Workspace &ws, const sa_t *SA, sa_t *SAi, int64_t n);
int rv_build_inverse_checked(Workspace &ws, const sa_t *SA, sa_t *SAi, int64_t n);
int rv_build_lcp(Workspace &ws, const uint8_t *T, const sa_t *SA, bool by_rank, lcp_t *LCP, int64_t n, u32 *d_maxlcp, uint8_t *BWT, sa_t side_sep);
int rv_build_bwt(Workspace &ws, const uint8_t *T, const sa_t *SA, int64_t n, uint8_t *BWT, sa_t side_sep);
```

reveal_amd/csrc/rv_construct.hip:

```cpp
#include "rv_common.h"
#include <string.h>
#include <stdlib.h>
#include <algorithm>
#include <limits>

#ifdef RV_SA64
typedef u64 sav_t;
#else
typedef u32 sav_t;
#endif

namespace {

constexpr int TB = 256;

__device__ inline u64 swar_eq(u64 v, uint8_t c) {
    const u64 t = v ^ (0x0101010101010101ull * c);
    return ~(((t & 0x7f7f7f7f7f7f7f7full) + 0x7f7f7f7f7f7f7f7full) | t) & 0x8080808080808080ull;
}
__device__ inline u64 swar_acgt(u64 v) { return swar_eq(v, 'A') | swar_eq(v, 'C') | swar_eq(v, 'G') | swar_eq(v, 'T'); }
__device__ inline u32 swar_code2(u64 v) {
    u64 y = ((v >> 1) ^ (v >> 2)) & 0x0303030303030303ull;
    y = (y | (y >> 6)) & 0x000f000f000f000full;
    y = (y | (y >> 12)) & 0x000000ff000000ffull;
    y = (y | (y >> 24)) & 0xffffull;
    return (u32)y;
}

__global__ __launch_bounds__(TB) void k_hist256(const uint8_t *__restrict__ T, int64_t n, u32 *__restrict__ hist) {
    __shared__ u32 hh[256];
    hh[threadIdx.x] = 0;
    __syncthreads();
    u32 cA = 0, cC = 0, cG = 0, cT = 0, cS = 0;
    const int64_t stride = (int64_t)gridDim.x * TB * 16;
    for (int64_t base = ((int64_t)blockIdx.x * TB + threadIdx.x) * 16; base < n; base += stride) {
        if (base + 16 <= n) {
            const uint4 v = *reinterpret_cast<const uint4 *>(T + base);
            const u64 w[2] = {(u64)v.x | ((u64)v.y << 32), (u64)v.z | ((u64)v.w << 32)};
            u64 sep[2];
#pragma unroll
            for (int k = 0; k < 2; k++) {
                const u64 eA = swar_eq(w[k], 'A'), eC = swar_eq(w[k], 'C'), eG = swar_eq(w[k], 'G'), eT = swar_eq(w[k], 'T'), eS = swar_eq(w[k], '$');
                cA += (u32)__popcll(eA); cC += (u32)__popcll(eC); cG += (u32)__popcll(eG); cT += (u32)__popcll(eT); cS += (u32)__popcll(eS);
                sep[k] = eS;
                u64 other = ~(eA | eC | eG | eT | eS) & 0x8080808080808080ull;
                while (other) {
                    const int b = __builtin_ctzll(other) >> 3;
                    atomicAdd(&hh[(w[k] >> (8 * b)) & 255u], 1u);
                    other &= other - 1;
                }
            }
            if (sep[0] | sep[1]) for (int64_t i = base; i < base + 16; i++) if (T[i] == '$' && i + 1 < n && T[i + 1] == '$') atomicAdd(&hist[256], 1u);
        } else {
            for (int64_t i = base; i < n; i++) { atomicAdd(&hh[T[i]], 1u); if (T[i] == '$' && i + 1 < n && T[i + 1] == '$') atomicAdd(&hist[256], 1u); }
        }
    }
    if (cA) atomicAdd(&hh[(uint8_t)'A'], cA);
    if (cC) atomicAdd(&hh[(uint8_t)'C'], cC);
    if (cG) atomicAdd(&hh[(uint8_t)'G'], cG);
    if (cT) atomicAdd(&hh[(uint8_t)'T'], cT);
    if (cS) atomicAdd(&hh[(uint8_t)'$'], cS);
    __syncthreads();
    const u32 tot = hh[threadIdx.x];
    if (tot) atomicAdd(&hist[threadIdx.x], tot);
    if (blockIdx.x == 0 && threadIdx.x == 0) hist[257] = T[n - 1];
}

constexpr int KEY_TILE = 1024;

struct DiagBits { const u64 *stop, *exc, *lt; int64_t D; int tab; };
struct DiagSamples { int ns; int64_t sep[15], Ds[16]; };
__device__ inline int64_t diag_partner(const DiagSamples &ds, int64_t y) {
    int s = 0;
    for (int q = 0; q < ds.ns - 1; q++) s += ds.sep[q] < y ? 1 : 0;
    return s == 0 ? y + ds.Ds[1] : (s < 16 ? y - ds.Ds[s] : -1);
}
__global__ __launch_bounds__(TB) void k_diag_bits(const uint8_t *__restrict__ T, int64_t n, DiagSamples ds, u64 *__restrict__ stop, u64 *__restrict__ exc,
                                                  u64 *__restrict__ lt, int64_t nwords) {
    const int64_t w = (int64_t)blockIdx.x * TB + threadIdx.x;
    if (w >= nwords) return;
    const int64_t y0 = w * 64;
    u64 ws = 0, we = 0, wl = 0;
    const int64_t p0 = diag_partner(ds, y0), p63 = y0 + 63 < n ? diag_partner(ds, y0 + 63) : -1;
    if (y0 + 64 <= n && p0 >= 0 && p63 == p0 + 63 && p0 + 64 <= n) {
        u64 a[8], b[8];
        __builtin_memcpy(a, T + y0, 64);
        __builtin_memcpy(b, T + p0, 64);
#pragma unroll
        for (int k = 0; k < 8; k++)
#pragma unroll
            for (int j = 0; j < 8; j++) {
                const u32 ca = (u32)(a[k] >> (8 * j)) & 0xffu, cb = (u32)(b[k] >> (8 * j)) & 0xffu;
                const bool ea = !((ca == 'A') | (ca == 'C') | (ca == 'G') | (ca == 'T')), eb = !((cb == 'A') | (cb == 'C') | (cb == 'G') | (cb == 'T'));
                const int bit = 8 * k + j;
                we |= (u64)(ea | eb) << bit; ws |= (u64)((ca != cb) | ea | eb) << bit; wl |= (u64)(ca < cb) << bit;
            }
    } else {
        for (int bit = 0; bit < 64; bit++) {
            const int64_t y = y0 + bit;
            const int64_t p = y < n ? diag_partner(ds, y) : -1;
            if (p < 0 || p >= n) { we |= 1ull << bit; ws |= 1ull << bit; continue; }
            const u32 ca = T[y], cb = T[p];
            const bool ea = !((ca == 'A') | (ca == 'C') | (ca == 'G') | (ca == 'T')), eb = !((cb == 'A') | (cb == 'C') | (cb == 'G') | (cb == 'T'));
            we |= (u64)(ea | eb) << bit; ws |= (u64)((ca != cb) | ea | eb) << bit; wl |= (u64)(ca < cb) << bit;
        }
    }
    stop[w] = ws; exc[w] = we; lt[w] = wl;
}
constexpr int32_t DT_NONE = 0x7fffffff;
constexpr int DT_SHIFT = 4, DT_TILE = 1 << DT_SHIFT;
constexpr int SEED_K = 32, SEED_SLOTS = 4;
constexpr u64 SEED_EMPTY = (1ull << 40) - 1;
struct DiagTab { const int32_t *dtab; int64_t S2, D; };
__device__ inline u64 seed_mix(u64 x) { x ^= x >> 31; x *= 0x9E3779B97F4A7C15ull; x ^= x >> 29; x *= 0xBF58476D1CE4E5B9ull; x ^= x >> 32; return x; }
__global__ __launch_bounds__(TB) void k_seed_sample(const uint8_t *__restrict__ T, int64_t n, u64 *__restrict__ keys, sav_t *__restrict__ vals, int64_t nwords) {
    const int64_t w = (int64_t)blockIdx.x * TB + threadIdx.x;
    if (w >= nwords) return;
    const int64_t y0 = w * 64;
    u64 code = 0; int run = 0, cnt = 0;
    u64 ok[SEED_SLOTS]; sav_t ov[SEED_SLOTS];
#pragma unroll
    for (int k = 0; k < SEED_SLOTS; k++) { ok[k] = SEED_EMPTY; ov[k] = 0; }
    for (int64_t i = y0 - (SEED_K - 1); i < y0 + 64 && i < n; i++) {
        const u32 c = i >= 0 ? T[i] : 0u;
        const u32 c2 = c == 'A' ? 0u : c == 'C' ? 1u : c == 'G' ? 2u : c == 'T' ? 3u : 4u;
        run = c2 < 4u ? run + 1 : 0;
        code = (code << 2) | (c2 & 3u);
        if (i >= y0 && run >= SEED_K) {
            const u64 h = seed_mix(code);
            if ((h & 15u) == 0u && cnt < SEED_SLOTS) {
                const u64 k40 = h >> 24;
                if (k40 != SEED_EMPTY) {
#pragma unroll
                    for (int k = 0; k < SEED_SLOTS; k++) if (k == cnt) { ok[k] = k40; ov[k] = (sav_t)(i - (SEED_K - 1)); }
                    cnt++;
                }
            }
        }
    }
#pragma unroll
    for (int k = 0; k < SEED_SLOTS; k++) { keys[w * SEED_SLOTS + k] = ok[k]; vals[w * SEED_SLOTS + k] = ov[k]; }
}
__global__ __launch_bounds__(TB) void k_seed_pairs(const u64 *__restrict__ keys, const sav_t *__restrict__ vals, int64_t m, int64_t S2, int64_t D, int32_t *__restrict__ raw) {
    const int64_t j = (int64_t)blockIdx.x * TB + threadIdx.x;
    if (j + 1 >= m) return;
    const u64 mk = (1ull << 40) - 1;
    const u64 k0 = keys[j] & mk, k1 = keys[j + 1] & mk;
    if (k0 == SEED_EMPTY || k0 != k1) return;
    if (j > 0 && (keys[j - 1] & mk) == k0) return;
    if (j + 2 < m && (keys[j + 2] & mk) == k0) return;
    int64_t a = (int64_t)vals[j], b = (int64_t)vals[j + 1];
    if (a > b) { const int64_t t = a; a = b; b = t; }
    if (!(a + SEED_K < S2 && b >= S2)) return;
    const int64_t dd = b - a - D;
    if (dd <= -(int64_t)0x3fffffff || dd >= (int64_t)0x3fffffff) return;
    for (int64_t t = a >> DT_SHIFT; t <= (a + SEED_K - 1) >> DT_SHIFT; t++) atomicMin(&raw[t], (int32_t)dd);
    for (int64_t t = b >> DT_SHIFT; t <= (b + SEED_K - 1) >> DT_SHIFT; t++) atomicMin(&raw[t], (int32_t)dd);
}
__device__ inline int dtab_agree(const uint8_t *__restrict__ T, int64_t n, int64_t S2, int64_t D, int64_t t, int32_t dd) {
    int c = 0;
    for (int k = 0; k < DT_TILE; k++) {
        const int64_t y = (t << DT_SHIFT) + k;
        if (y >= n) break;
        const int64_t z = y < S2 ? y + D + (int64_t)dd : y - D - (int64_t)dd;
        c += (z >= 0 && z < n && T[y] == T[z]) ? 1 : 0;
    }
    return c;
}
__global__ __launch_bounds__(TB) void k_dtab_fill(const uint8_t *__restrict__ T, int64_t n, int64_t S2, int64_t D, const int32_t *__restrict__ raw, int32_t *__restrict__ dtab, int64_t ntiles) {
    const int64_t t = (int64_t)blockIdx.x * TB + threadIdx.x;
    if (t >= ntiles) return;
    int32_t v = raw[t];
    if (v >= 0x7f000000) {
        int32_t L = DT_NONE, R = DT_NONE;
        for (int d = 1; d <= 64 && L == DT_NONE; d++) if (t - d >= 0) { const int32_t x = raw[t - d]; if (x < 0x7f000000) L = x; }
        for (int d = 1; d <= 64 && R == DT_NONE; d++) if (t + d < ntiles) { const int32_t x = raw[t + d]; if (x < 0x7f000000) R = x; }
        if (L == DT_NONE) v = R;
        else if (R == DT_NONE || R == L) v = L;
        else v = dtab_agree(T, n, S2, D, t, R) > dtab_agree(T, n, S2, D, t, L) ? R : L;
    }
    dtab[t] = v;
}
__device__ inline int32_t dtab_link(const DiagTab &dt, int64_t y, int64_t n, int64_t *partner) {
    if (y < 0 || y >= n || y == dt.S2 - 1) return DT_NONE;
    const int32_t dd = dt.dtab[y >> DT_SHIFT];
    if (dd == DT_NONE) return DT_NONE;
    const bool s1 = y < dt.S2;
    const int64_t z = s1 ? y + dt.D + (int64_t)dd : y - dt.D - (int64_t)dd;
    if (z < 0 || z >= n || (s1 ? z < dt.S2 : z >= dt.S2 - 1)) return DT_NONE;
    if (dt.dtab[z >> DT_SHIFT] != dd) return DT_NONE;
    *partner = z;
    return dd;
}
__global__ __launch_bounds__(TB) void k_diag_bits_tab(const uint8_t *__restrict__ T, int64_t n, DiagTab dt, u64 *__restrict__ stop, u64 *__restrict__ exc,
                                                      u64 *__restrict__ lt, int64_t nwords) {
    const int64_t w = (int64_t)blockIdx.x * TB + threadIdx.x;
    if (w >= nwords) return;
    const int64_t y0 = w * 64;
    u64 ws = 0, we = 0, wl = 0;
    int64_t zp = 0;
    int32_t prev = dtab_link(dt, y0 - 1, n, &zp);
    for (int sub = 0; sub < 64 / DT_TILE; sub++) {
        const int64_t ys = y0 + sub * DT_TILE;
        u32 ms = 0, me = 0, ml = 0;
        const int32_t dd = ys < n ? dt.dtab[ys >> DT_SHIFT] : DT_NONE;
        const bool one_side = ys >= dt.S2 || ys + DT_TILE - 1 < dt.S2 - 1;
        const int64_t z0 = ys < dt.S2 ? ys + dt.D + (int64_t)dd : ys - dt.D - (int64_t)dd;
        const bool other_side = ys < dt.S2 ? z0 >= dt.S2 : z0 + DT_TILE - 1 < dt.S2 - 1;
        if (dd == DT_NONE) { ms = me = 0xffffu; prev = DT_NONE; }
        else if (one_side && ys + DT_TILE <= n && z0 >= 0 && z0 + DT_TILE <= n && other_side) {
            const int off = (int)(z0 & (DT_TILE - 1));
            const bool v0 = dt.dtab[z0 >> DT_SHIFT] == dd, v1 = off ? dt.dtab[(z0 >> DT_SHIFT) + 1] == dd : v0;
            const u32 lowm = off ? ((1u << (DT_TILE - off)) - 1u) : 0xffffu;
            const u32 valid = (v0 ? lowm : 0u) | (v1 ? (~lowm & 0xffffu) : 0u);
            u64 a[2], b[2];
            __builtin_memcpy(a, T + ys, 16);
            __builtin_memcpy(b, T + z0, 16);
#pragma unroll
            for (int k = 0; k < 2; k++)
#pragma unroll
                for (int j = 0; j < 8; j++) {
                    const u32 ca = (u32)(a[k] >> (8 * j)) & 0xffu, cb = (u32)(b[k] >> (8 * j)) & 0xffu;
                    const bool ea = !((ca == 'A') | (ca == 'C') | (ca == 'G') | (ca == 'T')), eb = !((cb == 'A') | (cb == 'C') | (cb == 'G') | (cb == 'T'));
                    const int bit = 8 * k + j;
                    me |= (u32)(ea | eb) << bit; ms |= (u32)((ca != cb) | ea | eb) << bit; ml |= (u32)(ca < cb) << bit;
                }
            u32 forced = 0;
            if ((valid & 1u) && prev != dd) forced |= 1u;
            if (off && !v0 && v1) forced |= 1u << (DT_TILE - off);
            ms |= (~valid & 0xffffu) | forced; me |= (~valid & 0xffffu) | forced; ml &= valid & ~forced;
            prev = (valid >> (DT_TILE - 1)) & 1u ? dd : DT_NONE;
        } else {
            for (int bit = 0; bit < DT_TILE; bit++) {
                const int64_t y = ys + bit;
                int64_t z = 0;
                const int32_t l = dtab_link(dt, y, n, &z);
                if (l == DT_NONE || l != prev) { me |= 1u << bit; ms |= 1u << bit; prev = l; continue; }
                const u32 ca = T[y], cb = T[z];
                const bool ea = !((ca == 'A') | (ca == 'C') | (ca == 'G') | (ca == 'T')), eb = !((cb == 'A') | (cb == 'C') | (cb == 'G') | (cb == 'T'));
                me |= (u32)(ea | eb) << bit; ms |= (u32)((ca != cb) | ea | eb) << bit; ml |= (u32)((ca < cb) & !(ea | eb)) << bit;
            }
        }
        ws |= (u64)ms << (sub * DT_TILE); we |= (u64)me << (sub * DT_TILE); wl |= (u64)ml << (sub * DT_TILE);
    }
    stop[w] = ws; exc[w] = we; lt[w] = wl;
}
constexpr sav_t TW_FLAG = (sav_t)1 << (sizeof(sav_t) * 8 - 1);
__device__ inline u64 tw_window_clear(u64 prev, u64 lo, u64 hi, int K) {
    u64 a = lo, b = hi;
    int m = 1;
    while (2 * m <= K) { a |= (a >> m) | (b << (64 - m)); b |= b >> m; m *= 2; }
    if (m < K) { const int d = K - m; a |= (a >> d) | (b << (64 - d)); }
    return ~(a | (lo << 1) | (prev >> 63));
}
__device__ inline u64 tw_range(int64_t w, int64_t a, int64_t b) {
    const int64_t lo = a - 64 * w, hi = b - 64 * w;
    if (hi <= 0 || lo >= 64) return 0ull;
    const u64 from = lo <= 0 ? ~0ull : (~0ull << lo), to = hi >= 64 ? ~0ull : ((1ull << hi) - 1ull);
    return from & to;
}
// ... 737 lines not shown
            const u32 q = run + before + (u32)__popcll(bal & lt);
            P[q] = pos_in ? pos_in[j] : (u32)j;
            S[q] = suf_in[j];
            G[q] = grp_in[j];
            if (cls_out) cls_out[q] = cls_in ? (cls_is ? (cls_in[j] == (uint8_t)cls_is) : cls_in[j]) : (uint8_t)0;
        }
        run += tot;
        __syncthreads();
    }
}

__global__ __launch_bounds__(TB) void k_cp_count_g(const uint8_t *__restrict__ head, int64_t n, u32 *__restrict__ tilecnt, u32 *__restrict__ tilelast) {
    __shared__ u32 wsum[TB / 64], wlast[TB / 64];
    static_assert(CP_ITEMS == 8, "eight head bytes per load");
    const int64_t j0 = (int64_t)blockIdx.x * CP_TILE + (int64_t)threadIdx.x * CP_ITEMS;
    u32 c = 0, last = 0;
    if (j0 + CP_ITEMS < n) {
        const u64 hb = *reinterpret_cast<const u64 *>(head + j0);
        const u64 nx = (hb >> 8) | ((u64)head[j0 + CP_ITEMS] << 56);
#pragma unroll
        for (int k = 0; k < CP_ITEMS; k++) c += !(((hb >> (8 * k)) & 0xFFu) && ((nx >> (8 * k)) & 0xFFu));
        if (hb) last = (u32)(j0 + ((63 - __builtin_clzll(hb)) >> 3) + 1);
    } else {
        for (int64_t j = j0; j < j0 + CP_ITEMS && j < n; j++) { c += unsorted_at(head, j, n); last = head[j] ? (u32)(j + 1) : last; }
    }
    for (int d = 32; d >= 1; d >>= 1) { c += __shfl_down(c, d, 64); const u32 o = __shfl_down(last, d, 64); last = o > last ? o : last; }
    if ((threadIdx.x & 63) == 0) { wsum[threadIdx.x >> 6] = c; wlast[threadIdx.x >> 6] = last; }
    __syncthreads();
    if (threadIdx.x == 0) {
        tilecnt[blockIdx.x] = wsum[0] + wsum[1] + wsum[2] + wsum[3];
        if (blockIdx.x + 1 == gridDim.x) tilecnt[gridDim.x] = 0;
        u32 l = wlast[0];
        for (int k = 1; k < TB / 64; k++) l = wlast[k] > l ? wlast[k] : l;
        tilelast[blockIdx.x] = l;
    }
}
__global__ __launch_bounds__(TB) void k_cp_emit_g(const uint8_t *__restrict__ head, int64_t n, const u32 *__restrict__ tileoff, const u32 *__restrict__ tilelast,
                                                  const sav_t *__restrict__ suf_in, u32 *__restrict__ P, sav_t *__restrict__ S, u32 *__restrict__ G) {
    __shared__ u32 wcnt[TB / 64], wlast[TB / 64];
    static_assert(CP_ITEMS == 8, "eight head bytes per load");
    const int lane = threadIdx.x & 63, w = threadIdx.x >> 6;
    const int64_t j0 = (int64_t)blockIdx.x * CP_TILE + (int64_t)threadIdx.x * CP_ITEMS;
    u32 hm = 0, um = 0;
    if (j0 + CP_ITEMS < n) {
        const u64 hb = *reinterpret_cast<const u64 *>(head + j0);
        const u64 nx = (hb >> 8) | ((u64)head[j0 + CP_ITEMS] << 56);
#pragma unroll
        for (int k = 0; k < CP_ITEMS; k++) {
            const bool h = (hb >> (8 * k)) & 0xFFu, hn = (nx >> (8 * k)) & 0xFFu;
            hm |= (u32)h << k; um |= (u32)!(h && hn) << k;
        }
    } else {
        for (int k = 0; k < CP_ITEMS; k++) { const int64_t j = j0 + k; if (j < n) { hm |= (u32)(head[j] != 0) << k; um |= (u32)unsorted_at(head, j, n) << k; } }
    }
    const u32 c = (u32)__popc(um);
    const u32 mylast = hm ? (u32)(j0 + (31 - __clz(hm)) + 1) : 0u;
    u32 inc = c, lastinc = mylast;
#pragma unroll
    for (int d = 1; d < 64; d <<= 1) {
        const u32 t = __shfl_up(inc, d, 64), l = __shfl_up(lastinc, d, 64);
        if (lane >= d) { inc += t; lastinc = l > lastinc ? l : lastinc; }
    }
    if (lane == 63) { wcnt[w] = inc; wlast[w] = lastinc; }
    __syncthreads();
    u32 before = inc - c;
    u32 prevlast = __shfl_up(lastinc, 1, 64);
    if (lane == 0) prevlast = 0;
    u32 seen = blockIdx.x ? tilelast[blockIdx.x - 1] : 0u;
    for (int k = 0; k < w; k++) { before += wcnt[k]; seen = wlast[k] > seen ? wlast[k] : seen; }
    prevlast = prevlast > seen ? prevlast : seen;
    u32 q = tileoff[blockIdx.x] + before;
    u32 cur = prevlast;
#pragma unroll
    for (int k = 0; k < CP_ITEMS; k++) {
        const int64_t j = j0 + k;
        if ((hm >> k) & 1u) cur = (u32)(j + 1);
        if ((um >> k) & 1u) {
            P[q] = (u32)j;
            S[q] = suf_in[j];
            G[q] = cur - 1u;
            q++;
        }
    }
}

__global__ __launch_bounds__(TB) void k_round_isa(const sav_t *__restrict__ S, const u32 *__restrict__ newG, int64_t m, u32 *__restrict__ ISA, const u32 *__restrict__ oldG = nullptr) {
    const int64_t q = (int64_t)blockIdx.x * TB + threadIdx.x;
    if (q >= m) return;
    const u32 g = newG[q];
    if (oldG && oldG[q] == g) return;
    ISA[S[q]] = g;
}

constexpr int SMALL_GROUP = 8;

__device__ inline u32 key2_of(sav_t s, int64_t h, int64_t n, const u32 *__restrict__ ISA) {
    const int64_t s2 = (int64_t)s + h;
    return (s2 < n) ? ISA[s2] + 1u : 0u;
}

__global__ __launch_bounds__(TB) void k_round_small(sav_t *__restrict__ S, const u32 *__restrict__ G, const u32 *__restrict__ P, int64_t m, int64_t n, int64_t h,
                                                    const u32 *__restrict__ ISA, uint8_t *__restrict__ headq, uint8_t *__restrict__ bigflag,
                                                    sa_t *__restrict__ SA, const uint8_t *__restrict__ slow = nullptr) {
    const int64_t q = (int64_t)blockIdx.x * TB + threadIdx.x;
    if (q >= m) return;
    const u32 g = G[q];
    const u32 off = P[q] - g;
    if (slow && !slow[q]) { bigflag[q] = 0; headq[q] = off == 0; return; }
    const int64_t look = q + (SMALL_GROUP - (int64_t)off);
    const bool big = off >= (u32)SMALL_GROUP || (look < m && G[look] == g);
    bigflag[q] = big;
    if (big || off != 0) return;
    sav_t s[SMALL_GROUP]; u32 k[SMALL_GROUP];
    int size = 1;
    s[0] = S[q]; k[0] = key2_of(s[0], h, n, ISA);
#pragma unroll
    for (int j = 1; j < SMALL_GROUP; j++) {
        if (size == j && q + j < m && G[q + j] == g) { s[j] = S[q + j]; k[j] = key2_of(s[j], h, n, ISA); size = j + 1; }
    }
#pragma unroll
    for (int a = 1; a < SMALL_GROUP; a++) {
        if (a < size) {
            const sav_t cs = s[a]; const u32 ck = k[a];
            int b = a;
#pragma unroll
            for (int t = SMALL_GROUP - 1; t >= 1; t--) {
                if (t <= a && t == b && k[t - 1] > ck) { s[t] = s[t - 1]; k[t] = k[t - 1]; b = t - 1; }
            }
#pragma unroll
            for (int t = 0; t < SMALL_GROUP; t++) if (t == b) { s[t] = cs; k[t] = ck; }
        }
    }
#pragma unroll
    for (int j = 0; j < SMALL_GROUP; j++) {
        if (j < size) {
            S[q + j] = s[j];
            SA[(size_t)g + j] = (sa_t)s[j];
            headq[q + j] = (j == 0) || (k[j] != k[j - (j > 0)]);
        }
    }
}

__device__ inline u64 zero_bytes(u64 y) {
    return (y - 0x0101010101010101ull) & ~y & 0x8080808080808080ull;
}
__device__ inline u64 load8(const uint8_t *p) {
    u64 v;
    __builtin_memcpy(&v, p, 8);
    return v;
}

constexpr int TEXT_LIM = 4096;
constexpr int PK_BLOCK = 128;
__global__ __launch_bounds__(TB) void k_pack2(const uint8_t *__restrict__ T, int64_t n, u64 *__restrict__ Tp, uint8_t *__restrict__ blk, int64_t nwords) {
    const int64_t w = (int64_t)blockIdx.x * TB + threadIdx.x;
    if (w >= nwords) return;
    const int64_t p0 = w * 32;
    u64 word = 0; bool exc = false;
    if (p0 + 32 <= n) {
        const uint4 *q4 = reinterpret_cast<const uint4 *>(T + p0);
        const uint4 lo = q4[0], hi = q4[1];
        const u64 v[4] = {(u64)lo.x | ((u64)lo.y << 32), (u64)lo.z | ((u64)lo.w << 32), (u64)hi.x | ((u64)hi.y << 32), (u64)hi.z | ((u64)hi.w << 32)};
        u64 ok = 0x8080808080808080ull;
#pragma unroll
        for (int k = 0; k < 4; k++) {
            const u64 m = swar_acgt(v[k]);
            ok &= m;
            word |= (u64)swar_code2(v[k] & (m | (m >> 1) | (m >> 2) | (m >> 3) | (m >> 4) | (m >> 5) | (m >> 6) | (m >> 7))) << (16 * k);
        }
        exc = ok != 0x8080808080808080ull;
    } else {
        exc = true;
        for (int j = 0; j < 32 && p0 + j < n; j++) {
            const u32 c = T[p0 + j];
            const u32 code = c == 'A' ? 0u : c == 'C' ? 1u : c == 'G' ? 2u : c == 'T' ? 3u : 0u;
            word |= (u64)code << (2 * j);
        }
    }
    Tp[w] = word;
    if (exc) blk[p0 / PK_BLOCK] = 1;
}
struct Packed { const u64 *Tp; const uint8_t *blk; };

template <int W>
__device__ inline int cmp_text(const uint8_t *__restrict__ T, sav_t a, sav_t b, u32 *lcp, int h0 = 0, u32 stop0 = 0xFFFFFFFFu) {
    const uint8_t *pa = T + (int64_t)a, *pb = T + (int64_t)b;
    u32 stop_at = stop0;
    for (int off = h0; off < TEXT_LIM; off += 8 * W) {
        u64 wa[W], wb[W];
        __builtin_memcpy(wa, pa + off, 8 * W);
        __builtin_memcpy(wb, pb + off, 8 * W);
        if (stop_at == 0xFFFFFFFFu) {
            u64 any = 0;
#pragma unroll
            for (int k = 0; k < W; k++) any |= zero_bytes(wb[k] ^ 0x2424242424242424ull) | zero_bytes(wb[k] ^ 0x4E4E4E4E4E4E4E4Eull) | zero_bytes(wb[k]);
            if (any) {
#pragma unroll
                for (int k = W - 1; k >= 0; k--) {
                    const u64 st = zero_bytes(wb[k] ^ 0x2424242424242424ull) | zero_bytes(wb[k] ^ 0x4E4E4E4E4E4E4E4Eull) | zero_bytes(wb[k]);
                    stop_at = st ? (u32)off + 8u * (u32)k + (u32)(__builtin_ctzll(st) >> 3) : stop_at;
                }
            }
        }
        u64 x = 0, y = 0; u32 at = 0; bool diff = false;
#pragma unroll
        for (int k = W - 1; k >= 0; k--) {
            const bool d = wa[k] != wb[k];
            x = d ? wa[k] : x; y = d ? wb[k] : y; at = d ? 8u * (u32)k : at; diff |= d;
        }
        if (diff) {
            const u32 dpos = (u32)off + at + (u32)(__builtin_ctzll(x ^ y) >> 3);
            *lcp = dpos < stop_at ? dpos : stop_at;
            return __builtin_bswap64(x) < __builtin_bswap64(y) ? -1 : 1;
        }
    }
    *lcp = 0;
    return 0;
}

template <int W>
__device__ inline int cmp_suffix(const uint8_t *__restrict__ T, const Packed &pk, sav_t a, sav_t b, u32 *lcp, int h0, u32 stop0) {
#ifdef RV_RT_NOCMP
    *lcp = 20; return a < b ? -1 : 1;
#endif
    if (pk.Tp == nullptr) return cmp_text<W>(T, a, b, lcp, h0, stop0);
    for (int off = h0; off < TEXT_LIM; off += PK_BLOCK) {
        const int64_t pa = (int64_t)a + off, pb = (int64_t)b + off;
        const int64_t ba = pa / PK_BLOCK, bb = pb / PK_BLOCK;
        if (pk.blk[ba] | pk.blk[ba + 1] | pk.blk[bb] | pk.blk[bb + 1]) return cmp_text<W>(T, a, b, lcp, off, stop0);
        u64 ra[5], rb[5];
        __builtin_memcpy(ra, pk.Tp + (pa >> 5), 40);
        __builtin_memcpy(rb, pk.Tp + (pb >> 5), 40);
        const int sa = (int)(pa & 31) * 2, sb = (int)(pb & 31) * 2;
        u64 x = 0, y = 0; u32 at = 0; bool diff = false;
#pragma unroll
        for (int k = 3; k >= 0; k--) {
            const u64 xa = sa ? (ra[k] >> sa) | (ra[k + 1] << (64 - sa)) : ra[k];
            const u64 xb = sb ? (rb[k] >> sb) | (rb[k + 1] << (64 - sb)) : rb[k];
            const bool d = xa != xb;
            x = d ? xa : x; y = d ? xb : y; at = d ? 32u * (u32)k : at; diff |= d;
        }
        if (diff) {
            const int bit = __builtin_ctzll(x ^ y) & ~1;
            const u32 dpos = (u32)off + at + (u32)(bit >> 1);
            *lcp = dpos < stop0 ? dpos : stop0;
            return ((x >> bit) & 3u) < ((y >> bit) & 3u) ? -1 : 1;
        }
    }
    *lcp = 0;
    return 0;
}

struct FusedOut { lcp_t *LCP; uint8_t *BWT; const u64 *keys; u32 *maxlcp; sa_t side_sep; KeyDigits kd; int h; Packed pk; int far_defer; };
__device__ inline bool twins_linked(const KeyDigits &kd, int64_t n, int64_t a, int64_t b) {
    if (a < 0 || a >= kd.D - 1 || b >= n || b < kd.D) return false;
    if (!kd.dtab) return b - a == kd.D;
    const int32_t dd = kd.dtab[a >> DT_SHIFT];
    return dd != DT_NONE && kd.D + (int64_t)dd == b - a && kd.dtab[b >> DT_SHIFT] == dd;
}
__device__ inline void fused_put(const FusedOut &f, size_t rank, sav_t suf, u32 pay, bool first, u32 lcp, u32 &lmax) {
    f.BWT[rank] = (uint8_t)(pay | ((sa_t)suf > f.side_sep ? RV_BWT_SIDE : 0u));
    if (!first) {
        f.LCP[rank] = (lcp_t)lcp;
        lmax = lcp > lmax ? lcp : lmax;
    }
}
__device__ inline void fused_max_flush(const FusedOut &f, u32 lmax) {
    const u32 wm = (u32)rv_wave_max_u64((u64)lmax);
    if ((threadIdx.x & 63) == 0 && f.maxlcp && wm > __atomic_load_n(f.maxlcp, __ATOMIC_RELAXED)) atomicMax(f.maxlcp, wm);
}

constexpr int MEDIUM_GROUP = 64;
__global__ __launch_bounds__(TB) void k_medium_back(const uint8_t *__restrict__ flag, const sav_t *__restrict__ Sout, sav_t *__restrict__ S, int64_t m) {
    const int64_t q0 = ((int64_t)blockIdx.x * TB + threadIdx.x) * 8;
    if (q0 >= m) return;
    if (q0 + 8 <= m) {
        const u64 f = *reinterpret_cast<const u64 *>(flag + q0);
        if (((f ^ 0x0202020202020202ull) - 0x0101010101010101ull) & ~(f ^ 0x0202020202020202ull) & 0x8080808080808080ull) {
#pragma unroll
            for (int k = 0; k < 8; k++) if (((f >> (8 * k)) & 0xFFu) == 2u) S[q0 + k] = Sout[q0 + k];
        }
    } else {
        for (int64_t q = q0; q < m; q++) if (flag[q] == 2) S[q] = Sout[q];
    }
}
template <int W, int MODE>
__device__ __forceinline__ void round_text_body(const uint8_t *__restrict__ T, sav_t *__restrict__ S, const u32 *__restrict__ G, const u32 *__restrict__ P,
                                                int64_t m, uint8_t *__restrict__ headq, uint8_t *__restrict__ bigflag, sa_t *__restrict__ SA,
                                                sav_t *__restrict__ Sout, const FusedOut &fo, int64_t q, u32 &lmax) {
    const u32 g = G[q];
    const u32 off = P[q] - g;
    const int64_t look = q + (MEDIUM_GROUP - (int64_t)off);
    const bool big = off >= (u32)MEDIUM_GROUP || (look < m && G[look] == g);
    const int64_t qs = q - (int64_t)off;
    const bool fused = fo.LCP != nullptr;
    const int h0 = fo.h;
    const u32 stop0 = (fused && !big) ? key_first_stop(fo.keys[g], fo.kd) : 0xFFFFFFFFu;
    constexpr int DIRECT = MODE == 0 ? SMALL_GROUP : MODE == 1 ? 2 : 1;
    const bool self = !big && qs + DIRECT < m && G[qs + DIRECT] == g;
    bigflag[q] = big ? 1 : self ? 2 : 0;
    if (big) return;
    if (self) {
        int size = (int)off + 1;
        while (qs + size < m && G[qs + size] == g) size++;
        const sav_t mine = S[q];
        int rank = 0; bool tie_before = false; u32 best = 0;
        for (int j = 0; j < size; j++) {
            if (j == (int)off) continue;
            u32 l;
            const int c = cmp_suffix<W>(T, fo.pk, S[qs + j], mine, &l, h0, stop0);
            rank += (c < 0) | ((c == 0) & (j < (int)off));
            tie_before |= (c == 0) & (j < (int)off);
            best = (c < 0 && l > best) ? l : best;
        }
        Sout[qs + rank] = mine;
        SA[(size_t)g + rank] = (sa_t)mine;
        headq[qs + rank] = !tie_before;
        if (fused) fused_put(fo, (size_t)g + rank, mine, (u32)(fo.keys[(size_t)g + off] >> 56), rank == 0, best, lmax);
        return;
    }
    if (off != 0) return;
    if (MODE >= 1) {
        const sav_t s0 = S[q], s1 = S[q + 1];
        u32 l;
        const int c = cmp_suffix<W>(T, fo.pk, s0, s1, &l, h0, stop0);
        const sav_t lo = c <= 0 ? s0 : s1, hi = c <= 0 ? s1 : s0;
        S[q] = lo; S[q + 1] = hi;
        SA[(size_t)g] = (sa_t)lo; SA[(size_t)g + 1] = (sa_t)hi;
        headq[q] = 1; headq[q + 1] = c != 0;
        if (fused) {
            const u32 p0 = (u32)(fo.keys[(size_t)g] >> 56), p1 = (u32)(fo.keys[(size_t)g + 1] >> 56);
            fused_put(fo, (size_t)g, lo, c <= 0 ? p0 : p1, true, 0, lmax);
            fused_put(fo, (size_t)g + 1, hi, c <= 0 ? p1 : p0, false, l, lmax);
// ... 693 lines not shown
    const int64_t k = (int64_t)blockIdx.x * TB + threadIdx.x;
    if (k < n) { const sa_t p = SA[k]; BWT[k] = (uint8_t)((p > 0 ? T[p - 1] : (uint8_t)'$') | (p > side_sep ? RV_BWT_SIDE : 0)); }
}

constexpr int TINY_N = 2048;
__global__ __launch_bounds__(TB) void k_sa_tiny_rank(const uint8_t *__restrict__ T, int n, uint16_t *__restrict__ ord) {
    __shared__ __attribute__((aligned(8))) uint8_t txt[TINY_N + 32];
    for (int k = threadIdx.x; k < n + 32; k += TB) txt[k] = k < n ? T[k] : (uint8_t)0;
    __syncthreads();
    const int i = (int)blockIdx.x * TB + threadIdx.x;
    if (i >= n) return;
    u64 ki = 0, wj = 0;
#pragma unroll
    for (int b = 0; b < 8; b++) { ki |= (u64)txt[i + b] << (8 * b); wj |= (u64)txt[b] << (8 * b); }
    int cnt = 0;
    for (int j0 = 0; j0 < n; j0 += 8) {
        u64 nxt = *reinterpret_cast<const u64 *>(txt + j0 + 8);
#pragma unroll
        for (int e = 0; e < 8; e++) {
            const int j = j0 + e;
            if (j < n && j != i) {
                const int lim = n - (i > j ? i : j);
                const u64 d = ki ^ wj;
                int x = d ? (__builtin_ctzll(d) >> 3) : 8;
                bool j_less;
                if (x < 8 && x < lim) j_less = (u32)((wj >> (8 * x)) & 0xffu) < (u32)((ki >> (8 * x)) & 0xffu);
                else {
                    if (x >= 8 && lim > 8) {
                        x = 8;
                        while (x + 8 <= lim) {
                            u64 a, b;
                            __builtin_memcpy(&a, txt + i + x, 8);
                            __builtin_memcpy(&b, txt + j + x, 8);
                            if (a != b) { x += __builtin_ctzll(a ^ b) >> 3; break; }
                            x += 8;
                        }
                        while (x < lim && txt[i + x] == txt[j + x]) x++;
                    }
                    j_less = (x < lim) ? (txt[j + x] < txt[i + x]) : (j > i);
                }
                cnt += j_less ? 1 : 0;
            }
            wj = (wj >> 8) | (nxt << 56);
            nxt >>= 8;
        }
    }
    ord[cnt] = (uint16_t)i;
}
__global__ __launch_bounds__(TB) void k_sa_tiny_emit(const uint8_t *__restrict__ T, int n, const uint16_t *__restrict__ ord, sa_t *__restrict__ SA, lcp_t *__restrict__ LCP,
                                                     uint8_t *__restrict__ BWT, sa_t side_sep, u32 *__restrict__ d_maxlcp) {
    __shared__ uint8_t txt[TINY_N + 16];
    for (int k = threadIdx.x; k < n + 16; k += TB) txt[k] = k < n ? T[k] : (uint8_t)0;
    __syncthreads();
    const int r = (int)blockIdx.x * TB + threadIdx.x;
    u32 l = 0;
    if (r < n) {
        const int i = ord[r];
        if (r > 0) {
            const int j = ord[r - 1];
            const int lim = n - (i > j ? i : j);
            int x = 0;
            while (x < lim) { const uint8_t c = txt[i + x]; if (c != txt[j + x] || c == '$' || c == 'N') break; x++; }
            l = (u32)x;
        }
        SA[r] = (sa_t)i; LCP[r] = (lcp_t)l;
        BWT[r] = (uint8_t)((i > 0 ? txt[i - 1] : (uint8_t)'$') | ((sa_t)i > side_sep ? RV_BWT_SIDE : 0u));
    }
    const u32 wm = (u32)rv_wave_max_u64((u64)l);
    if ((threadIdx.x & 63) == 0 && wm) atomicMax(d_maxlcp, wm);
}

inline int bitlen(u64 v) { int b = 0; while (v) { b++; v >>= 1; } return b; }

}

int rv_build_inverse(Workspace &ws, const sa_t *SA, sa_t *SAi, int64_t n) {
    if (n <= 0) return 0;
    hipLaunchKernelGGL(k_inverse, dim3((unsigned)ceil_div(n, TB)), dim3(TB), 0, ws.stream, SA, SAi, n);
    RV_LAUNCH_CHECK();
    return 0;
}

int rv_build_inverse_checked(Workspace &ws, const sa_t *SA, sa_t *SAi, int64_t n) {
    if (n <= 0) return 0;
    RV_TRY(ws.misc[1].reserve(64));
    u32 *d_err = ws.misc[1].as<u32>();
    RV_HIP(hipMemsetAsync(d_err, 0, 4, ws.stream));
    RV_HIP(hipMemsetAsync(SAi, 0xFF, (size_t)n * sizeof(sa_t), ws.stream));
    hipLaunchKernelGGL(k_inverse_checked, dim3((unsigned)ceil_div(n, TB)), dim3(TB), 0, ws.stream, SA, SAi, n, d_err);
    RV_LAUNCH_CHECK();
    hipLaunchKernelGGL(k_inverse_verify, dim3((unsigned)ceil_div(n, TB)), dim3(TB), 0, ws.stream, SA, (const sa_t *)SAi, n, d_err);
    RV_LAUNCH_CHECK();
    u32 err = 0;
    RV_TRY(rv_read_back(ws, &err, d_err, 4));
    if (err) { rv_set_error("the suffix array file does not hold a permutation of 0..n-1 (%s): stale or foreign cache file?", (err & 1u) ? "entry out of range" : "duplicate entries"); return -1; }
    return 0;
}

int rv_build_bwt(Workspace &ws, const uint8_t *T, const sa_t *SA, int64_t n, uint8_t *BWT, sa_t side_sep) {
    if (n <= 0) return 0;
    hipLaunchKernelGGL(k_bwt, dim3((unsigned)ceil_div(n, TB)), dim3(TB), 0, ws.stream, T, SA, n, BWT, side_sep);
    RV_LAUNCH_CHECK();
    return 0;
}

int rv_build_lcp(Workspace &ws, const uint8_t *T, const sa_t *SA, bool by_rank, lcp_t *LCP, int64_t n, u32 *d_maxlcp, uint8_t *BWT, sa_t side_sep) {
    SaScratchInUse in_use(ws);
    if (n <= 0) return 0;
    RV_HIP(hipMemsetAsync(d_maxlcp, 0, sizeof(u32), ws.stream));
    if (by_rank || ws.opt.lcp_by_rank) {
        hipLaunchKernelGGL(k_lcp, dim3((unsigned)ceil_div(n, TB)), dim3(TB), 0, ws.stream, T, SA, LCP, n, d_maxlcp, BWT, side_sep);
        RV_LAUNCH_CHECK();
        return 0;
    }
    DBuf &bphi = ws.sa[1], &bpl = ws.sa[0];
    RV_TRY(bphi.reserve((size_t)n * sizeof(sa_t)));
    RV_TRY(bpl.reserve((size_t)n * 8));
    hipLaunchKernelGGL(k_phi, dim3((unsigned)ceil_div(n, TB)), dim3(TB), 0, ws.stream, SA, n, bphi.as<sa_t>());
    RV_LAUNCH_CHECK();
    hipLaunchKernelGGL(k_plcp, dim3((unsigned)ceil_div(ceil_div(n, PHI_K), TB)), dim3(TB), 0, ws.stream, T, (const sa_t *)bphi.as<sa_t>(), bpl.as<u64>(), n, side_sep);
    RV_LAUNCH_CHECK();
    hipLaunchKernelGGL(k_lcp_gather, dim3((unsigned)ceil_div(n, TB)), dim3(TB), 0, ws.stream, SA, (const u64 *)bpl.as<u64>(), LCP, n, d_maxlcp, BWT);
    RV_LAUNCH_CHECK();
    return 0;
}

int rv_build_sa(Workspace &ws, const uint8_t *T, int64_t n, sa_t *SA, RvSaStats *st,
                lcp_t *LCP, uint8_t *BWT, sa_t side_sep, u32 *d_maxlcp, bool *fused_done, const int64_t *seps, int nseps) {
    SaScratchInUse in_use(ws);
    RvSaStats s;
    memset(&s, 0, sizeof s);
    if (fused_done) *fused_done = false;
    if (n <= 0) { if (st) *st = s; return 0; }
    if (n >= ((int64_t)1 << 32) - 2) { rv_set_error("SA build: n >= 2^32-2 not supported yet"); return -1; }
    hipStream_t q = ws.stream;
    if (n <= TINY_N / 2 && LCP && BWT && d_maxlcp && !ws.opt.no_tiny_sa) {
        RV_TRY(ws.sa[0].reserve((size_t)TINY_N * 2 + 64));
        RV_HIP(hipMemsetAsync(d_maxlcp, 0, sizeof(u32), q));
        const unsigned nb = (unsigned)ceil_div(n, TB);
        hipLaunchKernelGGL(k_sa_tiny_rank, dim3(nb), dim3(TB), 0, q, T, (int)n, ws.sa[0].as<uint16_t>());
        RV_LAUNCH_CHECK();
        hipLaunchKernelGGL(k_sa_tiny_emit, dim3(nb), dim3(TB), 0, q, T, (int)n, (const uint16_t *)ws.sa[0].as<uint16_t>(), SA, LCP, BWT, side_sep, d_maxlcp);
        RV_LAUNCH_CHECK();
        s.rounds = 0; s.sorted_elems = 0;
        if (st) *st = s;
        if (fused_done) *fused_done = true;
        return 0;
    }

    DBuf &d_hist = ws.sa[16], &d_lut = ws.sa[17];
    RV_TRY(d_hist.reserve(264 * sizeof(u32)));
    RV_TRY(d_lut.reserve(256));
    RV_HIP(hipMemsetAsync(d_hist.p, 0, 264 * sizeof(u32), q));
    {
        int64_t blocks = ceil_div(n, (int64_t)TB * 16);
        if (blocks > 2048) blocks = 2048;
        hipLaunchKernelGGL(k_hist256, dim3((unsigned)blocks), dim3(TB), 0, q, T, n, d_hist.as<u32>());
        RV_LAUNCH_CHECK();
    }
    u32 hist[258];
    RV_TRY(rv_read_back(ws, hist, d_hist.p, sizeof hist));
    uint8_t lut[256];
    int sigma = 0;
    for (int c = 0; c < 256; c++) lut[c] = hist[c] ? (uint8_t)(++sigma) : (uint8_t)0;
    u32 radix = (u32)sigma + 1;
    if (sigma >= 255) radix = 256;
    if (sigma >= 255) for (int c = 0; c < 256; c++) lut[c] = (uint8_t)c;
    const bool short_alphabet = sigma >= 2 && sigma < 255 && T != nullptr && hist[(uint8_t)'$'] > 0 && lut[(uint8_t)'$'] == 1 && hist[256] == 0 && !ws.opt.no_short_alphabet;
    bool ends_with_sep = false;
    if (short_alphabet) ends_with_sep = hist[257] == (u32)(uint8_t)'$';
    if (short_alphabet && ends_with_sep) {
        for (int c = 0; c < 256; c++) lut[c] = hist[c] ? (uint8_t)(lut[c] - 1) : (uint8_t)0;
        radix = (u32)sigma;
    }
    int K = 1;
    int bits = 0;
    KeyPack kp;
    {
        const double base = sigma > 2 ? (double)(sigma - 1) : 2.0;
        const double want = (double)n * ((seps && nseps > 1) ? 16.0 : 1.0);
        int best_g = 0, best_K = 0, best_bits = 0;
        u64 rg = 1;
        for (int g = 1; g <= KP_MAXG; g++) {
            rg *= radix;
            if (rg > KP_MAXFIELD && g > 1) break;
            const int fb = bitlen(rg - 1);
            auto bits_of = [&](int k) { u64 rl = 1; for (int e = 0; e < k % g; e++) rl *= radix; return (k / g) * fb + (k % g ? bitlen(rl - 1) : 0); };
            bool exact = true;
            for (int i = 1; i < g && exact; i++) {
                u64 d = 1; for (int e = 0; e < g - i; e++) d *= radix;
                const u32 m = (u32)(((1ull << 20) + d - 1) / d);
                for (u64 f = 0; f < rg && exact; f++) exact = ((f * m) >> 20) == f / d && f * m < (1ull << 32);
            }
            if (!exact) continue;
            int k = 1; double cap = base;
            while (cap < want && bits_of(k + 1) <= 62) { cap *= base; k++; }
            const int passes = rv_radix_passes(ws, bits_of(k));
            while (bits_of(k + 1) <= 62 && rv_radix_passes(ws, bits_of(k + 1)) == passes) k++;
            const int b = bits_of(k);
            if (k > best_K || (k == best_K && b < best_bits)) { best_g = g; best_K = k; best_bits = b; }
        }
        K = best_K; bits = best_bits;
        u64 rgb = 1; for (int e = 0; e < best_g; e++) rgb *= radix;
        kp.g = best_g; kp.fb = bitlen(rgb - 1); kp.nf = (K + best_g - 1) / best_g; kp.gl = K - (kp.nf - 1) * best_g;
        u64 rl = 1; for (int e = 0; e < kp.gl; e++) rl *= radix;
        kp.fbl = bitlen(rl - 1); kp.bits = bits; kp.rad = radix; kp.fmask = (1u << kp.fb) - 1u; kp.lmask = (1u << kp.fbl) - 1u;
        kp.lscale = (u32)(rgb / rl); kp.fdiv = (1u << 16) / (u32)kp.fb + 1u;
        kp.lastmul = kp.gl == best_g ? (1u << 20) : (u32)(((1ull << 20) + kp.lscale - 1) / kp.lscale);
        for (int i = 1; i < KP_MAXG; i++) {
            u64 d = 1; for (int e = 0; e < best_g - i; e++) d *= radix;
            kp.dmul[i - 1] = i < best_g ? (u32)(((1ull << 20) + d - 1) / d) : 0u;
        }
    }
    s.sigma = sigma; s.bits = bits; s.k0 = K;
    RV_HIP(hipMemcpyAsync(d_lut.p, lut, 256, hipMemcpyHostToDevice, q));
    bool fused = LCP && BWT && d_maxlcp && bits <= 48 && !ws.opt.no_fused_lcp;
    KeyDigits kd;
    kd.ly.sortmask = bits >= 64 ? ~0ull : (1ull << bits) - 1;
    kd.ly.at_bits = K <= 30 ? 5 : 8; kd.ly.at_shift = 56 - kd.ly.at_bits;
    kd.ly.nd_shift = (bits + 7) / 8 * 8; kd.ly.nd_bits = 0;
    kd.D = (side_sep > 0 && (int64_t)side_sep < n - 1) ? (int64_t)side_sep + 1 : 0;
    kd.ns = 0;
    for (int q2 = 0; q2 < HINT_K - 1; q2++) kd.sep[q2] = std::numeric_limits<int64_t>::max();
    for (int q2 = 0; q2 < HINT_K; q2++) kd.Ds[q2] = 0;
    if (seps && nseps > 0 && kd.D > 0) {
        kd.ns = (nseps + 1 < HINT_K + 1) ? nseps + 1 : HINT_K + 1;
        if (kd.ns > HINT_K) kd.ns = HINT_K;
        for (int q2 = 0; q2 < kd.ns - 1; q2++) kd.sep[q2] = seps[q2];
        for (int q2 = 1; q2 < kd.ns; q2++) kd.Ds[q2] = seps[q2 - 1] + 1;
        if (nseps + 1 > HINT_K) kd.ns = 0;
    }
    const bool want_hint = fused && kd.D > 0 && kd.ns >= 2 && kd.ly.at_shift - kd.ly.nd_shift >= 8 && !ws.opt.no_diag && !ws.opt.no_packed_text;
    if (want_hint) kd.ly.nd_bits = std::min(kd.ly.at_shift - kd.ly.nd_shift - 1, 11);
    kd.K = K; kd.kp = kp; kd.stop0 = lut[(uint8_t)'$']; kd.stop1 = lut[(uint8_t)'N'];
    if (fused) RV_HIP(hipMemsetAsync(d_maxlcp, 0, sizeof(u32), q));

    DBuf &bk0 = ws.sa[0], &bk1 = ws.sa[1], &bv0 = ws.sa[2], &bv1 = ws.sa[3], &bhead = ws.sa[4], &bseed = ws.sa[5], &bgrp = ws.sa[6], &bisa = ws.sa[7],
         &bP0 = ws.sa[8], &bP1 = ws.sa[9], &bG0 = ws.sa[10], &bG1 = ws.sa[11], &btile = ws.sa[12], &bbig = ws.sa[13], &bQb = ws.sa[14], &bPb = ws.sa[15];
    auto freeall = [&]() {};
#define SA_TRY(x) do { int r__ = (x); if (r__) { freeall(); return r__; } } while (0)
#define SA_HIP(x) do { hipError_t e__ = (x); if (e__ != hipSuccess) { rv_set_error("%s:%d %s", __FILE__, __LINE__, hipGetErrorString(e__)); freeall(); return -1; } } while (0)
    SA_TRY(bk0.reserve((size_t)n * 8)); SA_TRY(bk1.reserve((size_t)n * 8));
    SA_TRY(bv0.reserve((size_t)n * sizeof(sav_t))); SA_TRY(bv1.reserve((size_t)n * sizeof(sav_t)));
    SA_TRY(bhead.reserve((size_t)n + 16));
    auto need_seed_grp = [&](int64_t cnt) -> int {
        RV_TRY(bseed.reserve((size_t)std::max<int64_t>(cnt, 1) * (sizeof(sav_t) > 4 ? sizeof(sav_t) : 4)));
        return bgrp.reserve((size_t)std::max<int64_t>(cnt, 1) * 4);
    };
    SA_TRY(bisa.reserve((size_t)n * 4));
    const unsigned nblk = (unsigned)ceil_div(n, TB);

    DiagBits dg; dg.stop = dg.exc = dg.lt = nullptr; dg.D = kd.D; dg.tab = 0;
    kd.dtab = nullptr;
    const int64_t nw = (n + 63) / 64;
    DiagSamples dsm; dsm.ns = kd.ns;
    for (int q2 = 0; q2 < HINT_K - 1; q2++) dsm.sep[q2] = kd.sep[q2];
    for (int q2 = 0; q2 < HINT_K; q2++) dsm.Ds[q2] = kd.Ds[q2];
    if (kd.ly.nd_bits > 0) {
        DBuf &bds = ws.sa[20], &bde = ws.sa[21], &bdl = ws.sa[22];
        SA_TRY(bds.reserve((size_t)nw * 8)); SA_TRY(bde.reserve((size_t)nw * 8)); SA_TRY(bdl.reserve((size_t)nw * 8));
        hipLaunchKernelGGL(k_diag_bits, dim3((unsigned)ceil_div(nw, TB)), dim3(TB), 0, q, T, n, dsm, bds.as<u64>(), bde.as<u64>(), bdl.as<u64>(), nw);
        SA_HIP(hipGetLastError());
        dg.stop = bds.as<u64>(); dg.exc = bde.as<u64>(); dg.lt = bdl.as<u64>();
    }
    const bool collapse = fused && kd.ly.nd_bits > 0 && kd.ns == 2 && K < 64 && kd.D > 1 && n > kd.D + 1 && !ws.opt.no_heads_fusion && !ws.opt.no_twin_collapse
                          && (sizeof(sav_t) > 4 || n < ((int64_t)1 << 31));
    int64_t nsort = n;
    const u32 *tw_off = nullptr;
    if (collapse) {
        const int64_t ntiles = ceil_div(n, KEY_TILE);
        DBuf &btw = ws.sa[23];
        SA_TRY(btw.reserve((size_t)(std::max<int64_t>(ntiles, ceil_div(n, TB)) + 1) * 4 + 64));
        u32 *tc = btw.as<u32>();
        auto count_kept = [&](int tab, u32 *kept_out) -> int {
            hipLaunchKernelGGL(k_tw_count, dim3((unsigned)ceil_div(nw, TB)), dim3(TB), 0, q, (const u64 *)dg.stop, nw, K, kd.D, n, tc, ntiles, tab);
            RV_LAUNCH_CHECK();
            RV_TRY(rv_exclusive_sum_u32(ws, tc, tc, ntiles + 1));
            return rv_read_back(ws, kept_out, tc + ntiles, 4);
        };
        u32 kept = 0;
        SA_TRY(count_kept(0, &kept));
        const int dt_mode = (int)ws.opt.diag_table;
        const int64_t n2 = n - kd.D;
        if (dt_mode != 0 && n >= 4096 && (dt_mode == 1 || (int64_t)kept * 10 > n2 * 3)) {
            const int64_t mseeds = nw * SEED_SLOTS;
            DBuf &bdt = ws.sa[25];
            const int64_t ndt = (n >> DT_SHIFT) + 1;
            SA_TRY(bdt.reserve((size_t)ndt * 8 + 64));
            int32_t *raw = bdt.as<int32_t>(), *tab = raw + ndt;
            const int did = ws.prof_begin(11 , (double)n + (double)mseeds * 12.0);
            hipLaunchKernelGGL(k_seed_sample, dim3((unsigned)ceil_div(nw, TB)), dim3(TB), 0, q, T, n, bk0.as<u64>(), bv0.as<sav_t>(), nw);
            SA_HIP(hipGetLastError());
            int sin1 = 0;
            SA_TRY(rv_radix_sort_pairs<sav_t>(ws, bk0.as<u64>(), bv0.as<sav_t>(), bk1.as<u64>(), bv1.as<sav_t>(), mseeds, 0, 40, &sin1));
            SA_HIP(hipMemsetAsync(raw, 0x7f, (size_t)ndt * 4, q));
            hipLaunchKernelGGL(k_seed_pairs, dim3((unsigned)ceil_div(mseeds, TB)), dim3(TB), 0, q, (const u64 *)(sin1 ? bk1.as<u64>() : bk0.as<u64>()),
                               (const sav_t *)(sin1 ? bv1.as<sav_t>() : bv0.as<sav_t>()), mseeds, kd.D, kd.D, raw);
            SA_HIP(hipGetLastError());
            hipLaunchKernelGGL(k_dtab_fill, dim3((unsigned)ceil_div(ndt, TB)), dim3(TB), 0, q, T, n, kd.D, kd.D, (const int32_t *)raw, tab, ndt);
            SA_HIP(hipGetLastError());
            DiagTab dt; dt.dtab = tab; dt.S2 = kd.D; dt.D = kd.D;
            hipLaunchKernelGGL(k_diag_bits_tab, dim3((unsigned)ceil_div(nw, TB)), dim3(TB), 0, q, T, n, dt, ws.sa[20].as<u64>(), ws.sa[21].as<u64>(), ws.sa[22].as<u64>(), nw);
            SA_HIP(hipGetLastError());
            ws.prof_end(did);
            u32 kept_tab = 0;
            SA_TRY(count_kept(1, &kept_tab));
            if (dt_mode == 1 || (int64_t)kept_tab * 5 < (int64_t)kept * 4) { kept = kept_tab; kd.dtab = tab; dg.tab = 1; }
            else {
                hipLaunchKernelGGL(k_diag_bits, dim3((unsigned)ceil_div(nw, TB)), dim3(TB), 0, q, T, n, dsm, ws.sa[20].as<u64>(), ws.sa[21].as<u64>(), ws.sa[22].as<u64>(), nw);
                SA_HIP(hipGetLastError());
                SA_TRY(count_kept(0, &kept));
            }
        }
        nsort = kd.D + (int64_t)kept;
        tw_off = tc;
        s.diag_table = dg.tab;
    }
    uint8_t *dig0 = nullptr;
    {
        const int64_t iktiles = ceil_div(n, KEY_TILE);
        const dim3 ig((unsigned)std::min<int64_t>(iktiles, 256 * 8));
        dig0 = rv_radix_first_digits(ws, nsort, 0, bits);
#define RV_IK_(G) hipLaunchKernelGGL(k_init_keys<G>, ig, dim3(TB), 0, q, T, n, d_lut.as<uint8_t>(), K, kp, bk0.as<u64>(), bv0.as<sav_t>(), fused ? 1 : 0, \
                                     kd.stop0, kd.stop1, kd.ly, dg, tw_off, iktiles, dig0)
        const int ikid = ws.prof_begin(12 , (double)n + (double)nsort * (8.0 + sizeof(sav_t) + 1.0));
        switch (kp.g) { case 1: RV_IK_(1); break; case 2: RV_IK_(2); break; case 3: RV_IK_(3); break; case 4: RV_IK_(4); break; default: RV_IK_(5); break; }
        ws.prof_end(ikid);
#undef RV_IK_
    }
    SA_HIP(hipGetLastError());
    int in1 = 0;
    SA_TRY(rv_radix_sort_pairs<sav_t>(ws, bk0.as<u64>(), bv0.as<sav_t>(), bk1.as<u64>(), bv1.as<sav_t>(), nsort, 0, bits, &in1, dig0 != nullptr));
    s.radix_passes += rv_radix_passes(ws, bits); s.sorted_elems += nsort;
    u64 *ks = in1 ? bk1.as<u64>() : bk0.as<u64>();
    sav_t *vs = in1 ? bv1.as<sav_t>() : bv0.as<sav_t>();
    u64 *kt = in1 ? bk0.as<u64>() : bk1.as<u64>();
    sav_t *vt = in1 ? bv0.as<sav_t>() : bv1.as<sav_t>();

    uint8_t *head = bhead.as<uint8_t>();
    if (!collapse) SA_TRY(need_seed_grp(n));
    u32 *seed = bseed.as<u32>(), *grp = bgrp.as<u32>(), *ISA = bisa.as<u32>();
    const u64 *keys_by_rank = ks;
    const sav_t *vals_by_rank = vs;
    if (collapse) {
        const int64_t nb = ceil_div(nsort, TC_TILE);
        u32 *bc = ws.sa[23].as<u32>();
        hipLaunchKernelGGL(k_tw_flags, dim3((unsigned)nb), dim3(TB), 0, q, (const sav_t *)vs, nsort, bc);
        SA_HIP(hipGetLastError());
        SA_TRY(rv_exclusive_sum_u32(ws, bc, bc, nb));
        sav_t *vexp = reinterpret_cast<sav_t *>(bisa.p);
        if (sizeof(sav_t) > 4) { SA_TRY(ws.sa[24].reserve((size_t)n * sizeof(sav_t))); vexp = ws.sa[24].as<sav_t>(); }
        const int pbid = ws.prof_begin(13 , (double)nsort * 2.0 * (8.0 + sizeof(sav_t)) + (double)n * (1.0 + sizeof(sa_t) + sizeof(lcp_t) + 1.0));
        hipLaunchKernelGGL(k_heads_publish_tc, dim3((unsigned)nb), dim3(TB), 0, q, (const u64 *)ks, (const sav_t *)vs, nsort, (const u32 *)bc, head, LCP, SA, BWT,
                           side_sep, kd, d_maxlcp, ws.opt.no_pub_twins ? 0 : 1, kt, vexp);
        ws.prof_end(pbid);
        SA_HIP(hipGetLastError());
        keys_by_rank = kt; vals_by_rank = vexp;
    } else if (fused && kd.ly.nd_bits > 0 && !ws.opt.no_heads_fusion) {
        hipLaunchKernelGGL(k_heads_publish, dim3((unsigned)ceil_div(n, (int64_t)HP_ITEMS * TB)), dim3(TB), 0, q, (const u64 *)ks, (const sav_t *)vs, n, head, seed, LCP, SA, BWT, side_sep, kd, d_maxlcp,
                           ws.opt.no_pub_twins ? 0 : 1);
        SA_HIP(hipGetLastError());
        SA_TRY(rv_inclusive_max_u32(ws, seed, grp, n));
    } else {
        hipLaunchKernelGGL(k_heads, dim3(nblk), dim3(TB), 0, q, (const u64 *)ks, n, head, seed, fused ? LCP : (lcp_t *)nullptr, kd, fused ? d_maxlcp : (u32 *)nullptr);
        SA_HIP(hipGetLastError());
        SA_TRY(rv_inclusive_max_u32(ws, seed, grp, n));
        {
            KeyDigits kp = kd;
            if (ws.opt.no_pub_twins) kp.ly.nd_bits = 0;
            hipLaunchKernelGGL(k_publish0, dim3(nblk), dim3(TB), 0, q, (const sav_t *)vs, n, SA, (const u64 *)ks, fused ? BWT : (uint8_t *)nullptr, side_sep,
                               kp, fused ? LCP : (lcp_t *)nullptr, head, d_maxlcp, grp);
        }
        SA_HIP(hipGetLastError());
    }
    bool isa_built = false;
    const sav_t *cur_S = nullptr; const u32 *cur_G = nullptr; int64_t cur_m = 0;
    auto need_isa = [&]() -> int {
        if (isa_built) return 0;
        hipLaunchKernelGGL(k_isa_identity, dim3(nblk), dim3(TB), 0, q, (const sa_t *)SA, n, ISA);
        RV_LAUNCH_CHECK();
        if (cur_m > 0) {
            hipLaunchKernelGGL(k_round_isa, dim3((unsigned)ceil_div(cur_m, TB)), dim3(TB), 0, q, cur_S, cur_G, cur_m, ISA);
            RV_LAUNCH_CHECK();
        }
        isa_built = true;
        return 0;
    };

    int64_t ntile = ceil_div(n, CP_TILE);
    SA_TRY(btile.reserve(std::max((size_t)(ntile + 1) * 8 + 64, (size_t)RT_REGIONS * 4)));
    u32 *tile = btile.as<u32>();
    auto count_unsorted = [&](const uint8_t *hd, int64_t len, int64_t *m_out) -> int {
        const int64_t nt = ceil_div(len, CP_TILE);
        hipLaunchKernelGGL(k_cp_count, dim3((unsigned)nt), dim3(TB), 0, q, hd, len, tile);
        RV_LAUNCH_CHECK();
        RV_TRY(rv_exclusive_sum_u32(ws, tile, tile, nt + 1));
        u32 tot = 0;
        RV_TRY(rv_read_back(ws, &tot, tile + nt, 4));
        *m_out = tot;
        return 0;
    };
    auto emit_unsorted = [&](const uint8_t *hd, int64_t len, const u32 *pos_in, const sav_t *suf_in, const u32 *grp_in, u32 *P, sav_t *S, u32 *G,
                             const uint8_t *cls_in = nullptr, uint8_t *cls_out = nullptr, int cls_is = 0) -> int {
        const int64_t nt = ceil_div(len, CP_TILE);
        hipLaunchKernelGGL(k_cp_emit, dim3((unsigned)nt), dim3(TB), 0, q, hd, len, (const u32 *)tile, pos_in, suf_in, grp_in, P, S, G, cls_in, cls_out, cls_is);
        RV_LAUNCH_CHECK();
        return 0;
    };
    int64_t m = 0;
    if (collapse) {
        u32 *tlast = tile + (ntile + 1);
        hipLaunchKernelGGL(k_cp_count_g, dim3((unsigned)ntile), dim3(TB), 0, q, (const uint8_t *)head, n, tile, tlast);
        SA_HIP(hipGetLastError());
        SA_TRY(rv_exclusive_sum_u32(ws, tile, tile, ntile + 1));
        SA_TRY(rv_inclusive_max_u32(ws, tlast, tlast, ntile));
        u32 tot = 0;
        SA_TRY(rv_read_back(ws, &tot, tile + ntile, 4));
        m = tot;
        SA_TRY(bP0.reserve((size_t)std::max<int64_t>(m, 1) * 4)); SA_TRY(bG0.reserve((size_t)std::max<int64_t>(m, 1) * 4));
        SA_TRY(need_seed_grp(m));
        seed = bseed.as<u32>(); grp = bgrp.as<u32>();
        if (m > 0) {
            hipLaunchKernelGGL(k_cp_emit_g, dim3((unsigned)ntile), dim3(TB), 0, q, (const uint8_t *)head, n, (const u32 *)tile, (const u32 *)tlast, vals_by_rank,
                               bP0.as<u32>(), vt, bG0.as<u32>());
            SA_HIP(hipGetLastError());
        }
    } else {
        SA_TRY(count_unsorted(head, n, &m));
        SA_TRY(bP0.reserve((size_t)std::max<int64_t>(m, 1) * 4)); SA_TRY(bG0.reserve((size_t)std::max<int64_t>(m, 1) * 4));
        if (m > 0) SA_TRY(emit_unsorted(head, n, nullptr, vals_by_rank, grp, bP0.as<u32>(), vt, bG0.as<u32>()));
    }
    const int64_t m_list0 = m;
    u32 *P = bP0.as<u32>(), *G = bG0.as<u32>(), *Pn = nullptr, *Gn = nullptr;
    sav_t *S = vt;
    sav_t *Sfree = vs;
    u64 *kA = ks, *kB = kt;
    if (m > 0) { SA_TRY(bbig.reserve((size_t)m + 16)); SA_TRY(bQb.reserve((size_t)m * 4)); SA_TRY(bPb.reserve((size_t)m * 4)); }

    const int lowbits = bitlen((u64)n), highbits = bitlen((u64)(n > 1 ? n - 1 : 1));
    int64_t h = K;
    const bool can_far = fused && kd.ly.nd_bits > 0 && kd.ns == 2 && dg.stop != nullptr && !ws.opt.no_far_twins;
    const bool can_list = fused && !ws.opt.no_lcp_list;
    bool text_round_ran = false, far_ran = false, partial = false;
    DBuf &btodo = ws.sa[26];
    int64_t ntodo = 0;
    auto todo_add = [&](const u32 *ranks, int64_t cnt) -> int {
        if (cnt <= 0) return 0;
        if ((size_t)(ntodo + cnt) * 4 > btodo.cap) {
            DBuf nb;
            RV_TRY(nb.reserve((size_t)(ntodo + cnt) * 4 * 2 + 1024));
            if (ntodo) RV_HIP(hipMemcpyAsync(nb.p, btodo.p, (size_t)ntodo * 4, hipMemcpyDeviceToDevice, q));
            RV_HIP(hipStreamSynchronize(q));
            btodo.release();
            btodo = nb;
        }
        RV_HIP(hipMemcpyAsync(btodo.as<u32>() + ntodo, ranks, (size_t)cnt * 4, hipMemcpyDeviceToDevice, q));
        ntodo += cnt;
        return 0;
    };
    auto leave_fused = [&](const u32 *ranks, int64_t cnt) -> int {
        if (!fused) return 0;
        if (!can_list) { fused = false; return 0; }
        partial = true;
        return todo_add(ranks, cnt);
    };
    bool list_in_todo = false;
    DBuf &bcls0 = ws.sa[30], &bcls1 = ws.sa[31];
    uint8_t *cls = nullptr, *cls_next = nullptr;
    while (m > 0) {
        if (h >= 2 * n + 2 + 2 * TEXT_LIM) { rv_set_error("SA build: did not converge"); freeall(); return -1; }
        s.rounds++;
        const unsigned mb = (unsigned)ceil_div(m, TB);
        uint8_t *bigflag = bbig.as<uint8_t>();
        cur_S = S; cur_G = G; cur_m = m;
        const bool far_round = text_round_ran && !far_ran && can_far;
        const bool text_round = !far_round && s.rounds == 1 && h <= 64 && !ws.opt.sa_no_text;
        bool text_big = false;
        if (far_round) {
            far_ran = true;
            DBuf &bR = ws.sa[27], &bM = ws.sa[28];
            const int64_t nw1 = ceil_div(kd.D - 1, (int64_t)64);
            SA_TRY(bR.reserve(std::max((size_t)nw * 4 + 64, (size_t)(nw1 * 64 + 64) * 4))); SA_TRY(bM.reserve((size_t)nw * 4 + 64));
            hipLaunchKernelGGL(k_far_rev, dim3((unsigned)ceil_div(nw, TB)), dim3(TB), 0, q, (const u64 *)dg.stop, nw, bR.as<u32>());
            SA_HIP(hipGetLastError());
            SA_TRY(rv_inclusive_max_u32(ws, bR.as<u32>(), bM.as<u32>(), nw));
            FarTwins ft; ft.stop = dg.stop; ft.exc = dg.exc; ft.lt = dg.lt; ft.M = bM.as<u32>(); ft.nw = nw; ft.n = n; ft.S2 = kd.D; ft.D = kd.D; ft.dtab = kd.dtab;
            const bool nd_table = m >= ((int64_t)1 << 21) || ws.opt.far_table == 1;
            if (nd_table) {
                hipLaunchKernelGGL(k_far_nd, dim3((unsigned)ceil_div(nw1, TB)), dim3(TB), 0, q, ft, bR.as<u32>(), nw1);
                SA_HIP(hipGetLastError());
            }
            hipLaunchKernelGGL(k_far_twins, dim3(mb), dim3(TB), 0, q, T, S, (const u32 *)G, (const u32 *)P, m, ft, nd_table ? (const u32 *)bR.as<u32>() : (const u32 *)nullptr, head, bigflag, SA, LCP, BWT, side_sep, d_maxlcp);
            SA_HIP(hipGetLastError());
        }
        else if (text_round)
        {
            text_round_ran = true;
            FusedOut fo;
            fo.pk.Tp = nullptr; fo.pk.blk = nullptr;
            if (!ws.opt.no_packed_text) {
                DBuf &bTp = ws.sa[18], &bBlk = ws.sa[19];
                const int64_t nwords = n / 32 + 4, nblk = n / PK_BLOCK + 8;
                SA_TRY(bTp.reserve((size_t)(nwords + 8) * 8)); SA_TRY(bBlk.reserve((size_t)nblk + 16));
                SA_HIP(hipMemsetAsync(bBlk.p, 0, (size_t)nblk + 16, q));
                SA_HIP(hipMemsetAsync(bTp.as<u64>() + nwords, 0, 64, q));
                hipLaunchKernelGGL(k_pack2, dim3((unsigned)ceil_div(nwords, TB)), dim3(TB), 0, q, T, n, bTp.as<u64>(), bBlk.as<uint8_t>(), nwords);
                SA_HIP(hipGetLastError());
                fo.pk.Tp = bTp.as<u64>(); fo.pk.blk = bBlk.as<uint8_t>();
            }
            fo.LCP = fused ? LCP : (lcp_t *)nullptr; fo.BWT = BWT; fo.keys = keys_by_rank; fo.maxlcp = d_maxlcp; fo.side_sep = side_sep; fo.kd = kd;
            fo.h = (int)h;
            fo.far_defer = (can_far && kd.dtab == nullptr) ? 1 : 0;
            const int tmode = ws.opt.text_mode >= 0 ? (int)ws.opt.text_mode : (kd.ly.nd_bits > 0 ? 3 : 1);
#define RT_LAUNCH(M_) hipLaunchKernelGGL((k_round_text<4, M_>), dim3(mb), dim3(TB), 0, q, T, S, (const u32 *)G, (const u32 *)P, m, head, bigflag, SA, Sfree, fo)
            const int tid = ws.prof_begin(9 , (double)m * (4 + 4 + sizeof(sav_t) + 8) + (double)m * (sizeof(sav_t) + sizeof(sa_t) + sizeof(lcp_t) + 2));
            if (tmode == 3 && fused) {
                u32 *work = bQb.as<u32>(), *work_count = tile;
                const u32 reg_cap = (u32)(ceil_div((int64_t)mb, RT_REGIONS) * (TB / 2));
                SA_HIP(hipMemsetAsync(work_count, 0, RT_REGIONS * 4, q));
                hipLaunchKernelGGL((k_round_text3<4>), dim3(mb), dim3(TB), 0, q, T, S, (const u32 *)G, (const u32 *)P, m, n, head, bigflag, SA, Sfree, fo, work, work_count, reg_cap);
                SA_HIP(hipGetLastError());
                u32 cnt[RT_REGIONS];
                SA_TRY(rv_read_back(ws, cnt, work_count, sizeof cnt));
                u32 mx = 0;
                for (int r = 0; r < RT_REGIONS; r++) mx = std::max(mx, cnt[r]);
                if (mx) {
                    const u32 bpr = (u32)ceil_div((int64_t)mx, TB);
                    hipLaunchKernelGGL((k_round_text3b<4>), dim3(bpr * RT_REGIONS), dim3(TB), 0, q, T, S, (const u32 *)G, m, n, head, SA, fo, (const u32 *)work,
                                       (const u32 *)work_count, reg_cap, bpr);
                }
            }
            else if (tmode == 0) RT_LAUNCH(0); else if (tmode == 2) RT_LAUNCH(2); else RT_LAUNCH(1);
#undef RT_LAUNCH
            SA_HIP(hipGetLastError());
            ws.prof_end(tid);
            hipLaunchKernelGGL(k_medium_back, dim3((unsigned)ceil_div(m, (int64_t)TB * 8)), dim3(TB), 0, q, (const uint8_t *)bigflag, (const sav_t *)Sfree, S, m);
        }
        else {
            if (!list_in_todo) { SA_TRY(leave_fused(P, m)); list_in_todo = true; }
            SA_TRY(need_isa());
            const uint8_t *slow = (cls && 2 * h <= TEXT_LIM) ? cls : nullptr;
            hipLaunchKernelGGL(k_round_small, dim3(mb), dim3(TB), 0, q, S, (const u32 *)G, (const u32 *)P, m, n, h, (const u32 *)ISA, head, bigflag, SA, slow);
        }
        SA_HIP(hipGetLastError());
        if (!far_round) {
            const int64_t nt = ceil_div(m, CP_TILE);
            hipLaunchKernelGGL(k_flag_count, dim3((unsigned)nt), dim3(TB), 0, q, (const uint8_t *)bigflag, m, tile);
            SA_HIP(hipGetLastError());
            SA_TRY(rv_exclusive_sum_u32(ws, tile, tile, nt + 1));
            u32 mbig = 0;
            SA_TRY(rv_read_back(ws, &mbig, tile + nt, 4));
            if (mbig > 0) {
                text_big = text_round;
                SA_TRY(need_isa());
                u32 *Pb = bPb.as<u32>(), *Qb = bQb.as<u32>();
                hipLaunchKernelGGL(k_flag_emit, dim3((unsigned)nt), dim3(TB), 0, q, (const uint8_t *)bigflag, m, (const u32 *)tile, (const u32 *)P, (const sav_t *)S,
                                   (const u32 *)G, n, h, (const u32 *)ISA, Pb, Sfree, Qb, kA);
                SA_HIP(hipGetLastError());
                if (!list_in_todo) SA_TRY(leave_fused(Pb, (int64_t)mbig));
                sav_t *sb0 = Sfree, *sb1 = reinterpret_cast<sav_t *>(bseed.p);
                int f1 = 0, f2 = 0;
                SA_TRY(rv_radix_sort_pairs<sav_t>(ws, kA, sb0, kB, sb1, mbig, 0, lowbits, &f1));
                u64 *k_in = f1 ? kB : kA, *k_out = f1 ? kA : kB;
                sav_t *s_in = f1 ? sb1 : sb0, *s_out = f1 ? sb0 : sb1;
                SA_TRY(rv_radix_sort_pairs<sav_t>(ws, k_in, s_in, k_out, s_out, mbig, 32, 32 + highbits, &f2));
                const u64 *kS = f2 ? k_out : k_in;
                const sav_t *sS = f2 ? s_out : s_in;
                s.radix_passes += rv_radix_passes(ws, lowbits) + rv_radix_passes(ws, highbits); s.sorted_elems += mbig;
                hipLaunchKernelGGL(k_big_writeback, dim3((unsigned)ceil_div(mbig, TB)), dim3(TB), 0, q, kS, (const u32 *)Pb, (const u32 *)Qb, sS, (int64_t)mbig, S, head, SA);
                SA_HIP(hipGetLastError());
            }
        }
        int64_t m2 = 0;
        SA_TRY(count_unsorted(head, m, &m2));
        if (far_round) s.far_pairs = (m - m2) / 2;
        if (m2 == 0) break;
        if (!can_far && !can_list) fused = false;
        hipLaunchKernelGGL(k_seed, dim3(mb), dim3(TB), 0, q, (const uint8_t *)head, (const u32 *)P, m, seed);
        SA_HIP(hipGetLastError());
        SA_TRY(rv_inclusive_max_u32(ws, seed, grp, m));
        if (isa_built) {
            hipLaunchKernelGGL(k_round_isa, dim3(mb), dim3(TB), 0, q, (const sav_t *)S, (const u32 *)grp, m, ISA, (const u32 *)G);
            SA_HIP(hipGetLastError());
        }
        if (!Pn) {
            SA_TRY(bP1.reserve((size_t)std::max<int64_t>(m_list0, 1) * 4)); SA_TRY(bG1.reserve((size_t)std::max<int64_t>(m_list0, 1) * 4));
            Pn = bP1.as<u32>(); Gn = bG1.as<u32>();
        }
        const bool want_cls = (text_round && text_big && !ws.opt.no_slow_class && n > 2 * TEXT_LIM) || cls != nullptr;
        if (want_cls) {
            SA_TRY(bcls0.reserve((size_t)m2 + 64)); SA_TRY(bcls1.reserve((size_t)m2 + 64));
            cls_next = (cls == bcls0.as<uint8_t>()) ? bcls1.as<uint8_t>() : bcls0.as<uint8_t>();
            SA_TRY(emit_unsorted(head, m, P, S, grp, Pn, Sfree, Gn, text_round ? (const uint8_t *)bigflag : (const uint8_t *)cls, cls_next, text_round ? 1 : 0));
            cls = cls_next;
        } else
        SA_TRY(emit_unsorted(head, m, P, S, grp, Pn, Sfree, Gn));
        { u32 *t = P; P = Pn; Pn = t; t = G; G = Gn; Gn = t; }
        { sav_t *t = S; S = Sfree; Sfree = t; }
        m = m2;
        if (text_round && !text_big && !ws.opt.no_text_jump && h < TEXT_LIM && n > 2 * TEXT_LIM) h = TEXT_LIM;
        else if (!far_round) h *= 2;
    }
    if (fused && partial) {
        DBuf &bov = ws.sa[29];
        SA_TRY(bov.reserve(64));
        SA_HIP(hipMemsetAsync(bov.p, 0, 4, q));
        hipLaunchKernelGGL(k_lcp_list, dim3((unsigned)ceil_div(ntodo * 64, TB)), dim3(TB), 0, q, T, n, (const sa_t *)SA, (const u32 *)btodo.as<u32>(), ntodo, LCP, BWT, side_sep,
                           d_maxlcp, bov.as<u32>());
        SA_HIP(hipGetLastError());
        u32 ov = 0;
        SA_TRY(rv_read_back(ws, &ov, bov.p, 4));
        if (ov) fused = false;
        s.lcp_list = ntodo;
    }
#undef SA_TRY
#undef SA_HIP
    freeall();
    if (st) *st = s;
    if (fused_done) *fused_done = fused;
    return 0;
}
```

Measured before the change: 24940.

## Fuse histogram, 2-bit packing and diagonal bit computation into one front pass

Adds a k_front kernel that reads the text once and computes the byte histogram, the 2-bit packed text with exception-block flags, and the stop/exc/lt/gt diagonal bitmaps using SWAR compares and an 8x8 bit transpose. The mirrored half of the diagonal bitmaps is derived from the gt bits by a shift-copy kernel instead of being recomputed from text. This replaces separate k_hist256, k_pack2 and k_diag_bits launches for the two-sequence case, so the text is streamed fewer times. It adds complexity, atomic-based histogramming for non-ACGT bytes, serial tail handling in one thread, and a test entry point with a toggle to disable it.

```diff
diff --git a/include/reveal_amd.h b/include/reveal_amd.h
--- a/include/reveal_amd.h
+++ b/include/reveal_amd.h
@@ -215,10 +215,13 @@
 int rv_sa_stats(rv_index *h, int *sigma, int *bits, int *k0, int *rounds, int64_t *sorted_elems, int *radix_passes);
 int rv_sa_diag_table(rv_index *h);
 int rv_sa_tail(rv_index *h, int64_t *out);
+int rv_sa_passes(rv_index *h, int64_t *out);
 
 int rv_test_exclusive_sum_u32(const uint32_t *in, uint32_t *out, int64_t n);
 int rv_test_inclusive_max_u32(const uint32_t *in, uint32_t *out, int64_t n);
 int rv_test_radix_sort(uint64_t *keys, uint32_t *vals, int64_t n, int bit_lo, int bit_hi);
+int rv_test_front_pass(const uint8_t *T, int64_t n, const int64_t *seps, int nseps, int which, uint32_t *hist, uint64_t *stop, uint64_t *exc, uint64_t *lt,
+                       uint64_t *Tp, uint8_t *blk);
 int rv_test_radix_time(int64_t n, int bits, int dist, int flags, int iters, double *ms, int64_t *bad);
 
 #ifdef __cplusplus
diff --git a/reveal_amd/_index.py b/reveal_amd/_index.py
--- a/reveal_amd/_index.py
+++ b/reveal_amd/_index.py
@@ -171,6 +171,11 @@
             self._dll.rv_sa_tail(self._h, tail)
             return dict(sigma=v[0].value, bits=v[1].value, k0=v[2].value, rounds=v[3].value, sorted_elems=se.value, radix_passes=rp.value,
                         diag_table=int(self._dll.rv_sa_diag_table(self._h)), far_pairs=int(tail[0]), lcp_list=int(tail[1]))
+
+        def sa_passes(self):
+            out = (ctypes.c_int64 * 3)()
+            self._dll.rv_sa_passes(self._h, out)
+            return tuple(int(x) for x in out)
 
         def construct(self, rc=0):
             if self._sx:
diff --git a/reveal_amd/_lib.py b/reveal_amd/_lib.py
--- a/reveal_amd/_lib.py
+++ b/reveal_amd/_lib.py
@@ -127,6 +127,7 @@
     "rv_sa_stats": (_I, [V] + [ctypes.POINTER(_I)] * 4 + [c_i64p, ctypes.POINTER(_I)]),
     "rv_sa_diag_table": (_I, [V]),
     "rv_sa_tail": (_I, [V, c_i64p]),
+    "rv_sa_passes": (_I, [V, c_i64p]),
     "rv_set_picker": (_I, [V, _I, V]),
     "rv_picker_info": (_I, [V, c_i64p]),
     "rv_pick_chain": (_I, [V, _I, _L, V, V, V, V, V, _I, V, V, V, _I, V]),
@@ -171,6 +172,7 @@
     "rv_test_exclusive_sum_u32": (_I, [V, V, _L]),
     "rv_test_inclusive_max_u32": (_I, [V, V, _L]),
     "rv_test_radix_sort": (_I, [V, V, _L, _I, _I]),
+    "rv_test_front_pass": (_I, [V, _L, V, _I, _I, V, V, V, V, V, V]),
     "rv_test_radix_time": (_I, [_L, _I, _I, _I, _I, ctypes.POINTER(_D), c_i64p]),
 }
 
diff --git a/reveal_amd/csrc/rv_api.hip b/reveal_amd/csrc/rv_api.hip
--- a/reveal_amd/csrc/rv_api.hip
+++ b/reveal_amd/csrc/rv_api.hip
@@ -964,6 +964,7 @@
 }
 int rv_sa_diag_table(rv_index *h) { return h->sa_stats.diag_table; }
 int rv_sa_tail(rv_index *h, int64_t *out) { if (!h || !out) return -1; out[0] = h->sa_stats.far_pairs; out[1] = h->sa_stats.lcp_list; return 0; }
+int rv_sa_passes(rv_index *h, int64_t *out) { if (!h || !out) return -1; out[0] = h->sa_stats.front_pass; out[1] = h->sa_stats.front_diag; out[2] = 0; return 0; }
 
 }
 namespace {
@@ -1160,6 +1161,28 @@
     if (!r && hipMemcpy(keys, in1 ? k1.p : k0.p, (size_t)n * 8, hipMemcpyDeviceToHost) != hipSuccess) r = -1;
     if (!r && hipMemcpy(vals, in1 ? v1.p : v0.p, (size_t)n * 4, hipMemcpyDeviceToHost) != hipSuccess) r = -1;
     k0.release(); k1.release(); v0.release(); v1.release();
+    test_ws_done(ws);
+    return r;
+}
+
+int rv_test_front_pass(const uint8_t *T, int64_t n, const int64_t *seps, int nseps, int which, uint32_t *hist, uint64_t *stop, uint64_t *exc, uint64_t *lt,
+                       uint64_t *Tp, uint8_t *blk) {
+    if (n <= 0 || nseps < 0 || (nseps > 0 && !seps)) { rv_set_error("rv_test_front_pass: bad arguments"); return -1; }
+    Workspace ws;
+    RV_TRY(test_ws(ws));
+    const int64_t nw = (n + 63) / 64, pkw = n / 32 + 4, pkb = n / 128 + 8;
+    DBuf dT, dh, ds, de, dl, dTp, db;
+    int r = 0;
+    if (dT.reserve((size_t)n + 64) || dh.reserve(264 * 4) || ds.reserve((size_t)nw * 8) || de.reserve((size_t)nw * 8) || dl.reserve((size_t)nw * 8) ||
+        dTp.reserve((size_t)(pkw + 8) * 8) || db.reserve((size_t)pkb + 16)) r = -1;
+    if (!r && hipMemset(dT.p, 0, (size_t)n + 64) != hipSuccess) r = -1;
+    if (!r && hipMemcpy(dT.p, T, (size_t)n, hipMemcpyHostToDevice) != hipSuccess) r = -1;
+    if (!r) r = rv_front_pass_run(ws, dT.as<uint8_t>(), n, seps, nseps, which, dh.as<u32>(), ds.as<u64>(), de.as<u64>(), dl.as<u64>(), dTp.as<u64>(), db.as<uint8_t>());
+    if (!r && hipStreamSynchronize(ws.stream) != hipSuccess) { rv_set_error("sync failed: %s", hipGetErrorString(hipGetLastError())); r = -1; }
+    if (!r && (hipMemcpy(hist, dh.p, 258 * 4, hipMemcpyDeviceToHost) != hipSuccess || hipMemcpy(stop, ds.p, (size_t)nw * 8, hipMemcpyDeviceToHost) != hipSuccess ||
+               hipMemcpy(exc, de.p, (size_t)nw * 8, hipMemcpyDeviceToHost) != hipSuccess || hipMemcpy(lt, dl.p, (size_t)nw * 8, hipMemcpyDeviceToHost) != hipSuccess ||
+               hipMemcpy(Tp, dTp.p, (size_t)pkw * 8, hipMemcpyDeviceToHost) != hipSuccess || hipMemcpy(blk, db.p, (size_t)pkb, hipMemcpyDeviceToHost) != hipSuccess)) r = -1;
+    dT.release(); dh.release(); ds.release(); de.release(); dl.release(); dTp.release(); db.release();
     test_ws_done(ws);
     return r;
 }
diff --git a/reveal_amd/csrc/rv_common.h b/reveal_amd/csrc/rv_common.h
--- a/reveal_amd/csrc/rv_common.h
+++ b/reveal_amd/csrc/rv_common.h
@@ -71,6 +71,7 @@
     X(no_fused_lcp, "RV_NO_FUSED_LCP", 0) \
     X(no_diag, "RV_NO_DIAG", 0) \
     X(no_packed_text, "RV_NO_PACKED_TEXT", 0) \
+    X(no_front_pass, "RV_NO_FRONT_PASS", 0) \
     X(no_heads_fusion, "RV_NO_HEADS_FUSION", 0) \
     X(no_twin_collapse, "RV_NO_TWIN_COLLAPSE", 0) \
     X(no_far_twins, "RV_NO_FAR_TWINS", 0) \
@@ -308,7 +309,7 @@
     DBuf rs_hist;
     DBuf rs_digits;
     DBuf misc[20];
-    DBuf sa[32];
+    DBuf sa[33];
     HBuf hpin;
     hipEvent_t ev_rb = nullptr;
     void *prof_ctx = nullptr;
@@ -363,10 +364,12 @@
     int    diag_table;
     int64_t far_pairs;
     int64_t lcp_list;
+    int    front_pass, front_diag;
 };
 int rv_build_sa(Workspace &ws, const uint8_t *T, int64_t n, sa_t *SA, RvSaStats *st,
                 lcp_t *LCP = nullptr, uint8_t *BWT = nullptr, sa_t side_sep = 0, u32 *d_maxlcp = nullptr, bool *fused_done = nullptr,
                 const int64_t *seps = nullptr, int nseps = 0);
+int rv_front_pass_run(Workspace &ws, const uint8_t *T, int64_t n, const int64_t *seps, int nseps, int which, u32 *hist, u64 *stop, u64 *exc, u64 *lt, u64 *Tp, uint8_t *blk);
 int rv_build_inverse(Workspace &ws, const sa_t *SA, sa_t *SAi, int64_t n);
 int rv_build_inverse_checked(Workspace &ws, const sa_t *SA, sa_t *SAi, int64_t n);
 int rv_build_lcp(Workspace &ws, const uint8_t *T, const sa_t *SA, bool by_rank, lcp_t *LCP, int64_t n, u32 *d_maxlcp, uint8_t *BWT, sa_t side_sep);
diff --git a/reveal_amd/csrc/rv_construct.hip b/reveal_amd/csrc/rv_construct.hip
--- a/reveal_amd/csrc/rv_construct.hip
+++ b/reveal_amd/csrc/rv_construct.hip
@@ -25,6 +25,21 @@
     y = (y | (y >> 12)) & 0x000000ff000000ffull;
     y = (y | (y >> 24)) & 0xffffull;
     return (u32)y;
+}
+__device__ inline u64 swar_ne(u64 a, u64 b) {
+    const u64 t = a ^ b;
+    return (((t & 0x7f7f7f7f7f7f7f7full) + 0x7f7f7f7f7f7f7f7full) | t) & 0x8080808080808080ull;
+}
+__device__ inline u64 swar_ltu(u64 a, u64 b) {
+    const u64 H = 0x8080808080808080ull;
+    const u64 t = (a | H) - (b & ~H);
+    return ((~a & b) | (~(a ^ b) & ~t)) & H;
+}
+__device__ inline u64 swar_transpose8(u64 x) {
+    u64 t = (x ^ (x >> 7)) & 0x00AA00AA00AA00AAull; x ^= t ^ (t << 7);
+    t = (x ^ (x >> 14)) & 0x0000CCCC0000CCCCull; x ^= t ^ (t << 14);
+    t = (x ^ (x >> 28)) & 0x00000000F0F0F0F0ull; x ^= t ^ (t << 28);
+    return x;
 }
 
 __global__ __launch_bounds__(TB) void k_hist256(const uint8_t *__restrict__ T, int64_t n, u32 *__restrict__ hist) {
@@ -76,11 +91,12 @@
     return s == 0 ? y + ds.Ds[1] : (s < 16 ? y - ds.Ds[s] : -1);
 }
 __global__ __launch_bounds__(TB) void k_diag_bits(const uint8_t *__restrict__ T, int64_t n, DiagSamples ds, u64 *__restrict__ stop, u64 *__restrict__ exc,
-                                                  u64 *__restrict__ lt, int64_t nwords) {
-    const int64_t w = (int64_t)blockIdx.x * TB + threadIdx.x;
-    if (w >= nwords) return;
+                                                  u64 *__restrict__ lt, int64_t nwords, int64_t w0 = 0, u64 *__restrict__ gt = nullptr, int64_t gt_words = 0,
+                                                  int64_t v0 = 0, int64_t v1 = 0) {
+    int64_t w = w0 + (int64_t)blockIdx.x * TB + threadIdx.x;
+    if (w >= nwords) { w = v0 + (w - std::max(nwords, w0)); if (w >= v1) return; }
     const int64_t y0 = w * 64;
-    u64 ws = 0, we = 0, wl = 0;
+    u64 ws = 0, we = 0, wl = 0, wg = 0;
     const int64_t p0 = diag_partner(ds, y0), p63 = y0 + 63 < n ? diag_partner(ds, y0 + 63) : -1;
     if (y0 + 64 <= n && p0 >= 0 && p63 == p0 + 63 && p0 + 64 <= n) {
         u64 a[8], b[8];
@@ -93,7 +109,7 @@
                 const u32 ca = (u32)(a[k] >> (8 * j)) & 0xffu, cb = (u32)(b[k] >> (8 * j)) & 0xffu;
                 const bool ea = !((ca == 'A') | (ca == 'C') | (ca == 'G') | (ca == 'T')), eb = !((cb == 'A') | (cb == 'C') | (cb == 'G') | (cb == 'T'));
                 const int bit = 8 * k + j;
-                we |= (u64)(ea | eb) << bit; ws |= (u64)((ca != cb) | ea | eb) << bit; wl |= (u64)(ca < cb) << bit;
+                we |= (u64)(ea | eb) << bit; ws |= (u64)((ca != cb) | ea | eb) << bit; wl |= (u64)(ca < cb) << bit; wg |= (u64)(ca > cb) << bit;
             }
     } else {
         for (int bit = 0; bit < 64; bit++) {
@@ -102,10 +118,11 @@
             if (p < 0 || p >= n) { we |= 1ull << bit; ws |= 1ull << bit; continue; }
             const u32 ca = T[y], cb = T[p];
             const bool ea = !((ca == 'A') | (ca == 'C') | (ca == 'G') | (ca == 'T')), eb = !((cb == 'A') | (cb == 'C') | (cb == 'G') | (cb == 'T'));
-            we |= (u64)(ea | eb) << bit; ws |= (u64)((ca != cb) | ea | eb) << bit; wl |= (u64)(ca < cb) << bit;
+            we |= (u64)(ea | eb) << bit; ws |= (u64)((ca != cb) | ea | eb) << bit; wl |= (u64)(ca < cb) << bit; wg |= (u64)(ca > cb) << bit;
         }
     }
     stop[w] = ws; exc[w] = we; lt[w] = wl;
+    if (gt && w < gt_words) gt[w] = wg;
 }
 constexpr int32_t DT_NONE = 0x7fffffff;
 constexpr int DT_SHIFT = 4, DT_TILE = 1 << DT_SHIFT;
@@ -1149,23 +1166,23 @@
 
 constexpr int TEXT_LIM = 4096;
 constexpr int PK_BLOCK = 128;
-__global__ __launch_bounds__(TB) void k_pack2(const uint8_t *__restrict__ T, int64_t n, u64 *__restrict__ Tp, uint8_t *__restrict__ blk, int64_t nwords) {
-    const int64_t w = (int64_t)blockIdx.x * TB + threadIdx.x;
-    if (w >= nwords) return;
+__device__ inline u64 pack2_bytes(const u64 (&v)[4], const u64 (&m)[4] ) {
+    u64 word = 0;
+#pragma unroll
+    for (int k = 0; k < 4; k++)
+        word |= (u64)swar_code2(v[k] & (m[k] | (m[k] >> 1) | (m[k] >> 2) | (m[k] >> 3) | (m[k] >> 4) | (m[k] >> 5) | (m[k] >> 6) | (m[k] >> 7))) << (16 * k);
+    return word;
+}
+__device__ inline u64 pack2_word(const uint8_t *__restrict__ T, int64_t n, int64_t w, bool *exc_out) {
     const int64_t p0 = w * 32;
     u64 word = 0; bool exc = false;
     if (p0 + 32 <= n) {
         const uint4 *q4 = reinterpret_cast<const uint4 *>(T + p0);
         const uint4 lo = q4[0], hi = q4[1];
         const u64 v[4] = {(u64)lo.x | ((u64)lo.y << 32), (u64)lo.z | ((u64)lo.w << 32), (u64)hi.x | ((u64)hi.y << 32), (u64)hi.z | ((u64)hi.w << 32)};
-        u64 ok = 0x8080808080808080ull;
-#pragma unroll
-        for (int k = 0; k < 4; k++) {
-            const u64 m = swar_acgt(v[k]);
-            ok &= m;
-            word |= (u64)swar_code2(v[k] & (m | (m >> 1) | (m >> 2) | (m >> 3) | (m >> 4) | (m >> 5) | (m >> 6) | (m >> 7))) << (16 * k);
-        }
-        exc = ok != 0x8080808080808080ull;
+        const u64 m[4] = {swar_acgt(v[0]), swar_acgt(v[1]), swar_acgt(v[2]), swar_acgt(v[3])};
+        word = pack2_bytes(v, m);
+        exc = (m[0] & m[1] & m[2] & m[3]) != 0x8080808080808080ull;
     } else {
         exc = true;
         for (int j = 0; j < 32 && p0 + j < n; j++) {
@@ -1174,8 +1191,127 @@
             word |= (u64)code << (2 * j);
         }
     }
-    Tp[w] = word;
-    if (exc) blk[p0 / PK_BLOCK] = 1;
+    *exc_out = exc;
+    return word;
+}
+__global__ __launch_bounds__(TB) void k_pack2(const uint8_t *__restrict__ T, int64_t n, u64 *__restrict__ Tp, uint8_t *__restrict__ blk, int64_t nwords) {
+    const int64_t w = (int64_t)blockIdx.x * TB + threadIdx.x;
+    if (w >= nwords) return;
+    bool exc;
+    Tp[w] = pack2_word(T, n, w, &exc);
+    if (exc) blk[w * 32 / PK_BLOCK] = 1;
+}
+
+struct FrontOut { u32 *hist; u64 *Tp; uint8_t *blk; int64_t npk; u64 *stop, *exc, *lt, *gt; int64_t D, F; };
+__global__ __launch_bounds__(TB) void k_front(const uint8_t *__restrict__ T, int64_t n, FrontOut fo) {
+    __shared__ u32 hh[256];
+    hh[threadIdx.x] = 0;
+    __syncthreads();
+    u32 cA = 0, cC = 0, cG = 0, cT = 0, cS = 0;
+    const int64_t nfull = n / 64;
+    for (int64_t w = (int64_t)blockIdx.x * TB + threadIdx.x; w < nfull; w += (int64_t)gridDim.x * TB) {
+        const int64_t y0 = w * 64;
+        u64 a[8], ma[8];
+        {
+            const uint4 *q4 = reinterpret_cast<const uint4 *>(T + y0);
+#pragma unroll
+            for (int k = 0; k < 4; k++) { const uint4 v = q4[k]; a[2 * k] = (u64)v.x | ((u64)v.y << 32); a[2 * k + 1] = (u64)v.z | ((u64)v.w << 32); }
+        }
+        u64 anysep = 0;
+#pragma unroll
+        for (int k = 0; k < 8; k++) {
+            const u64 eA = swar_eq(a[k], 'A'), eC = swar_eq(a[k], 'C'), eG = swar_eq(a[k], 'G'), eT = swar_eq(a[k], 'T'), eS = swar_eq(a[k], '$');
+            cA += (u32)__popcll(eA); cC += (u32)__popcll(eC); cG += (u32)__popcll(eG); cT += (u32)__popcll(eT); cS += (u32)__popcll(eS);
+            ma[k] = eA | eC | eG | eT;
+            anysep |= eS;
+            u64 other = ~(ma[k] | eS) & 0x8080808080808080ull;
+            while (other) {
+                const int b = __builtin_ctzll(other) >> 3;
+                atomicAdd(&hh[(a[k] >> (8 * b)) & 255u], 1u);
+                other &= other - 1;
+            }
+        }
+        if (anysep) for (int64_t i = y0; i < y0 + 64; i++) if (T[i] == '$' && i + 1 < n && T[i + 1] == '$') atomicAdd(&fo.hist[256], 1u);
+        if (fo.Tp) {
+#pragma unroll
+            for (int h = 0; h < 2; h++) {
+                const u64 v[4] = {a[4 * h], a[4 * h + 1], a[4 * h + 2], a[4 * h + 3]}, m[4] = {ma[4 * h], ma[4 * h + 1], ma[4 * h + 2], ma[4 * h + 3]};
+                fo.Tp[2 * w + h] = pack2_bytes(v, m);
+            }
+            u64 ok = 0x8080808080808080ull;
+#pragma unroll
+            for (int k = 0; k < 8; k++) ok &= ma[k];
+            if (ok != 0x8080808080808080ull) fo.blk[y0 / PK_BLOCK] = 1;
+        }
+        if (w < fo.F) {
+            u64 b[8];
+            __builtin_memcpy(b, T + y0 + fo.D, 64);
+            u64 ws = 0, we = 0, wl = 0, wg = 0;
+#pragma unroll
+            for (int k = 0; k < 8; k++) {
+                const u64 e = ~(ma[k] & swar_acgt(b[k])) & 0x8080808080808080ull, ne = swar_ne(a[k], b[k]), l = swar_ltu(a[k], b[k]);
+                we |= e >> (7 - k); ws |= (ne | e) >> (7 - k); wl |= l >> (7 - k); wg |= (ne & ~l) >> (7 - k);
+            }
+            fo.stop[w] = swar_transpose8(ws); fo.exc[w] = swar_transpose8(we); fo.lt[w] = swar_transpose8(wl); fo.gt[w] = swar_transpose8(wg);
+        }
+    }
+    if (cA) atomicAdd(&hh[(uint8_t)'A'], cA);
+    if (cC) atomicAdd(&hh[(uint8_t)'C'], cC);
+    if (cG) atomicAdd(&hh[(uint8_t)'G'], cG);
+    if (cT) atomicAdd(&hh[(uint8_t)'T'], cT);
+    if (cS) atomicAdd(&hh[(uint8_t)'$'], cS);
+    __syncthreads();
+    const u32 tot = hh[threadIdx.x];
+    if (tot) atomicAdd(&fo.hist[threadIdx.x], tot);
+    if (blockIdx.x == 0 && threadIdx.x == 0) {
+        fo.hist[257] = T[n - 1];
+        for (int64_t i = nfull * 64; i < n; i++) { atomicAdd(&fo.hist[T[i]], 1u); if (T[i] == '$' && i + 1 < n && T[i + 1] == '$') atomicAdd(&fo.hist[256], 1u); }
+        if (fo.Tp)
+            for (int64_t w2 = nfull * 2; w2 < fo.npk; w2++) {
+                bool exc;
+                fo.Tp[w2] = pack2_word(T, n, w2, &exc);
+                if (exc) fo.blk[w2 * 32 / PK_BLOCK] = 1;
+            }
+    }
+}
+__global__ __launch_bounds__(TB) void k_front_mirror(u64 *__restrict__ stop, u64 *__restrict__ exc, u64 *__restrict__ lt, const u64 *__restrict__ gt, int64_t D, int64_t w0, int64_t w1) {
+    const int64_t w = w0 + (int64_t)blockIdx.x * TB + threadIdx.x;
+    if (w >= w1) return;
+    const int64_t x0 = w * 64 - D, xw = x0 >> 6;
+    const int sh = (int)(x0 & 63);
+    auto take = [&](const u64 *A) { return sh ? (A[xw] >> sh) | (A[xw + 1] << (64 - sh)) : A[xw]; };
+    const u64 s2 = take(stop), e2 = take(exc), l2 = take(gt);
+    stop[w] = s2; exc[w] = e2; lt[w] = l2;
+}
+struct FrontPlan { int64_t F, M0, M1; };
+static FrontPlan front_plan(int64_t n, int64_t D) {
+    FrontPlan fp;
+    fp.F = std::max<int64_t>(0, std::min(D / 64, (n - D) / 64));
+    fp.M0 = (D + 63) / 64;
+    fp.M1 = std::max(fp.M0, std::min(2 * D / 64, n / 64));
+    return fp;
+}
+static int front_pass(hipStream_t q, const uint8_t *T, int64_t n, u32 *hist, u64 *Tp, uint8_t *blk, int64_t npk, const DiagSamples *ds, u64 *stop, u64 *exc, u64 *lt,
+                      u64 *gt, int64_t nw) {
+    FrontOut fo;
+    fo.hist = hist; fo.Tp = Tp; fo.blk = blk; fo.npk = npk; fo.stop = stop; fo.exc = exc; fo.lt = lt; fo.gt = gt; fo.D = 0; fo.F = 0;
+    FrontPlan fp; fp.F = fp.M0 = fp.M1 = 0;
+    if (ds) { fo.D = ds->Ds[1]; fp = front_plan(n, fo.D); fo.F = fp.F; }
+    int64_t blocks = ceil_div(std::max<int64_t>(n / 64, 1), TB);
+    if (blocks > 2048) blocks = 2048;
+    hipLaunchKernelGGL(k_front, dim3((unsigned)blocks), dim3(TB), 0, q, T, n, fo);
+    RV_LAUNCH_CHECK();
+    if (!ds) return 0;
+    const int64_t b0 = std::min(fp.M0, nw);
+    if ((b0 - fp.F) + (nw - fp.M1) > 0) {
+        hipLaunchKernelGGL(k_diag_bits, dim3((unsigned)ceil_div((b0 - fp.F) + (nw - fp.M1), TB)), dim3(TB), 0, q, T, n, *ds, stop, exc, lt, b0, fp.F, gt, b0, fp.M1, nw);
+        RV_LAUNCH_CHECK();
+    }
+    if (fp.M1 > fp.M0) {
+        hipLaunchKernelGGL(k_front_mirror, dim3((unsigned)ceil_div(fp.M1 - fp.M0, TB)), dim3(TB), 0, q, stop, exc, lt, (const u64 *)gt, fo.D, fp.M0, fp.M1);
+        RV_LAUNCH_CHECK();
+    }
+    return 0;
 }
 struct Packed { const u64 *Tp; const uint8_t *blk; };
 
@@ -2175,7 +2311,34 @@
     RV_TRY(d_hist.reserve(264 * sizeof(u32)));
     RV_TRY(d_lut.reserve(256));
     RV_HIP(hipMemsetAsync(d_hist.p, 0, 264 * sizeof(u32), q));
-    {
+    const int64_t nw = (n + 63) / 64;
+    const int64_t pk_words = n / 32 + 4, pk_blocks = n / PK_BLOCK + 8;
+    const bool front = !ws.opt.no_front_pass;
+    const bool front_pack = front && !ws.opt.no_packed_text;
+    const bool front_diag = front_pack && seps && nseps == 1 && side_sep > 0 && (int64_t)side_sep < n - 1 && seps[0] == (int64_t)side_sep && LCP && BWT && d_maxlcp
+                            && !ws.opt.no_fused_lcp && !ws.opt.no_diag;
+    if (front) {
+        u64 *fTp = nullptr; uint8_t *fBlk = nullptr;
+        if (front_pack) {
+            DBuf &bTp = ws.sa[18], &bBlk = ws.sa[19];
+            RV_TRY(bTp.reserve((size_t)(pk_words + 8) * 8)); RV_TRY(bBlk.reserve((size_t)pk_blocks + 16));
+            RV_HIP(hipMemsetAsync(bBlk.p, 0, (size_t)pk_blocks + 16, q));
+            RV_HIP(hipMemsetAsync(bTp.as<u64>() + pk_words, 0, 64, q));
+            fTp = bTp.as<u64>(); fBlk = bBlk.as<uint8_t>();
+        }
+        DiagSamples fds;
+        if (front_diag) {
+            fds.ns = 2;
+            for (int q2 = 0; q2 < HINT_K - 1; q2++) fds.sep[q2] = std::numeric_limits<int64_t>::max();
+            for (int q2 = 0; q2 < HINT_K; q2++) fds.Ds[q2] = 0;
+            fds.sep[0] = seps[0]; fds.Ds[1] = seps[0] + 1;
+            RV_TRY(ws.sa[20].reserve((size_t)nw * 8)); RV_TRY(ws.sa[21].reserve((size_t)nw * 8)); RV_TRY(ws.sa[22].reserve((size_t)nw * 8));
+            RV_TRY(ws.sa[32].reserve((size_t)(ceil_div(fds.Ds[1], 64) + 2) * 8));
+        }
+        RV_TRY(front_pass(q, T, n, d_hist.as<u32>(), fTp, fBlk, pk_words, front_diag ? &fds : nullptr, ws.sa[20].as<u64>(), ws.sa[21].as<u64>(), ws.sa[22].as<u64>(),
+                          ws.sa[32].as<u64>(), nw));
+        s.front_pass = 1; s.front_diag = front_diag ? 1 : 0;
+    } else {
         int64_t blocks = ceil_div(n, (int64_t)TB * 16);
         if (blocks > 2048) blocks = 2048;
         hipLaunchKernelGGL(k_hist256, dim3((unsigned)blocks), dim3(TB), 0, q, T, n, d_hist.as<u32>());
@@ -2275,15 +2438,16 @@
 
     DiagBits dg; dg.stop = dg.exc = dg.lt = nullptr; dg.D = kd.D; dg.tab = 0;
     kd.dtab = nullptr;
-    const int64_t nw = (n + 63) / 64;
     DiagSamples dsm; dsm.ns = kd.ns;
     for (int q2 = 0; q2 < HINT_K - 1; q2++) dsm.sep[q2] = kd.sep[q2];
     for (int q2 = 0; q2 < HINT_K; q2++) dsm.Ds[q2] = kd.Ds[q2];
     if (kd.ly.nd_bits > 0) {
         DBuf &bds = ws.sa[20], &bde = ws.sa[21], &bdl = ws.sa[22];
         SA_TRY(bds.reserve((size_t)nw * 8)); SA_TRY(bde.reserve((size_t)nw * 8)); SA_TRY(bdl.reserve((size_t)nw * 8));
-        hipLaunchKernelGGL(k_diag_bits, dim3((unsigned)ceil_div(nw, TB)), dim3(TB), 0, q, T, n, dsm, bds.as<u64>(), bde.as<u64>(), bdl.as<u64>(), nw);
-        SA_HIP(hipGetLastError());
+        if (!(front_diag && kd.ns == 2)) {
+            hipLaunchKernelGGL(k_diag_bits, dim3((unsigned)ceil_div(nw, TB)), dim3(TB), 0, q, T, n, dsm, bds.as<u64>(), bde.as<u64>(), bdl.as<u64>(), nw);
+            SA_HIP(hipGetLastError());
+        }
         dg.stop = bds.as<u64>(); dg.exc = bde.as<u64>(); dg.lt = bdl.as<u64>();
     }
     const bool collapse = fused && kd.ly.nd_bits > 0 && kd.ns == 2 && K < 64 && kd.D > 1 && n > kd.D + 1 && !ws.opt.no_heads_fusion && !ws.opt.no_twin_collapse
@@ -2523,12 +2687,14 @@
             fo.pk.Tp = nullptr; fo.pk.blk = nullptr;
             if (!ws.opt.no_packed_text) {
                 DBuf &bTp = ws.sa[18], &bBlk = ws.sa[19];
-                const int64_t nwords = n / 32 + 4, nblk = n / PK_BLOCK + 8;
-                SA_TRY(bTp.reserve((size_t)(nwords + 8) * 8)); SA_TRY(bBlk.reserve((size_t)nblk + 16));
-                SA_HIP(hipMemsetAsync(bBlk.p, 0, (size_t)nblk + 16, q));
-                SA_HIP(hipMemsetAsync(bTp.as<u64>() + nwords, 0, 64, q));
-                hipLaunchKernelGGL(k_pack2, dim3((unsigned)ceil_div(nwords, TB)), dim3(TB), 0, q, T, n, bTp.as<u64>(), bBlk.as<uint8_t>(), nwords);
-                SA_HIP(hipGetLastError());
+                if (!front_pack) {
+                    const int64_t nwords = pk_words, nblk = pk_blocks;
+                    SA_TRY(bTp.reserve((size_t)(nwords + 8) * 8)); SA_TRY(bBlk.reserve((size_t)nblk + 16));
+                    SA_HIP(hipMemsetAsync(bBlk.p, 0, (size_t)nblk + 16, q));
+                    SA_HIP(hipMemsetAsync(bTp.as<u64>() + nwords, 0, 64, q));
+                    hipLaunchKernelGGL(k_pack2, dim3((unsigned)ceil_div(nwords, TB)), dim3(TB), 0, q, T, n, bTp.as<u64>(), bBlk.as<uint8_t>(), nwords);
+                    SA_HIP(hipGetLastError());
+                }
                 fo.pk.Tp = bTp.as<u64>(); fo.pk.blk = bBlk.as<uint8_t>();
             }
             fo.LCP = fused ? LCP : (lcp_t *)nullptr; fo.BWT = BWT; fo.keys = keys_by_rank; fo.maxlcp = d_maxlcp; fo.side_sep = side_sep; fo.kd = kd;
@@ -2643,3 +2809,33 @@
     if (fused_done) *fused_done = fused;
     return 0;
 }
+
+int rv_front_pass_run(Workspace &ws, const uint8_t *T, int64_t n, const int64_t *seps, int nseps, int which, u32 *hist, u64 *stop, u64 *exc, u64 *lt, u64 *Tp, uint8_t *blk) {
+    hipStream_t q = ws.stream;
+    const int64_t nw = (n + 63) / 64, pk_words = n / 32 + 4, pk_blocks = n / PK_BLOCK + 8;
+    DiagSamples ds;
+    ds.ns = nseps + 1 < HINT_K ? nseps + 1 : HINT_K;
+    for (int k = 0; k < HINT_K - 1; k++) ds.sep[k] = std::numeric_limits<int64_t>::max();
+    for (int k = 0; k < HINT_K; k++) ds.Ds[k] = 0;
+    for (int k = 0; k < ds.ns - 1; k++) { ds.sep[k] = seps[k]; ds.Ds[k + 1] = seps[k] + 1; }
+    RV_HIP(hipMemsetAsync(hist, 0, 264 * sizeof(u32), q));
+    RV_HIP(hipMemsetAsync(blk, 0, (size_t)pk_blocks + 16, q));
+    RV_HIP(hipMemsetAsync(Tp + pk_words, 0, 64, q));
+    const bool two = nseps == 1 && seps[0] > 0 && seps[0] < n - 1;
+    if (which == 1) {
+        if (two) RV_TRY(ws.sa[32].reserve((size_t)(ceil_div(ds.Ds[1], 64) + 2) * 8));
+        RV_TRY(front_pass(q, T, n, hist, Tp, blk, pk_words, two ? &ds : nullptr, stop, exc, lt, ws.sa[32].as<u64>(), nw));
+    } else {
+        int64_t blocks = ceil_div(n, (int64_t)TB * 16);
+        if (blocks > 2048) blocks = 2048;
+        hipLaunchKernelGGL(k_hist256, dim3((unsigned)blocks), dim3(TB), 0, q, T, n, hist);
+        RV_LAUNCH_CHECK();
+        hipLaunchKernelGGL(k_pack2, dim3((unsigned)ceil_div(pk_words, TB)), dim3(TB), 0, q, T, n, Tp, blk, pk_words);
+        RV_LAUNCH_CHECK();
+    }
+    if (which != 1 || !two) {
+        hipLaunchKernelGGL(k_diag_bits, dim3((unsigned)ceil_div(nw, TB)), dim3(TB), 0, q, T, n, ds, stop, exc, lt, nw);
+        RV_LAUNCH_CHECK();
+    }
+    return 0;
+}
```

Result: no change. 25020, median of 5 (+0.3%).
